# CIawevy/FreeFine

Hardware: AMD Instinct MI355X
Metric: edited images/sec/GPU @512px 50-step DDIM (higher is better)
Workload: dtype bf16x3

## Files before the change

freefine_amd/_lib.py:

```python
import ctypes as C
import os

_HERE = os.path.dirname(os.path.abspath(__file__))
LIB_PATH = os.environ.get("FREEFINE_HIP_LIB") or os.path.join(_HERE, "libfreefine_hip.so")

FFN_F32, FFN_BF16, FFN_BF16X3, FFN_FP8 = 0, 1, 2, 3
IG_OUT_SILU, IG_OUT_F32, IG_GEGLU, IG_OUT_TRANSPOSED, IG_OUT_PAIR, IG_OUT_GELU, IG_OUT_RELU, IG_OUT_KV64 = 1, 2, 4, 8, 16, 32, 64, 128
IG_OUT_QGELU = 256
ELT_RELU, ELT_ADD, ELT_GELU = 0, 1, 2
ATT_MAXP, ATT_MAXB = 4, 16
ATT_HEAD_RULE, ATT_UNIFORM_SEL1, ATT_UNIFORM_SEL0, ATT_CAUSAL = 1, 2, 4, 8
NORM_SILU, NORM_OUT_PAIR = 1, 2
IMGPREP_MAX_SIDE = 4096
IMGPREP_MAX_TAPS = 2 * 3 * IMGPREP_MAX_SIDE + 1
BOX_NMS_MAX = 16384
KEEP_NONE, KEEP_SUM_LT128, KEEP_GT128 = 0, 1, 2


class IgemmDesc(C.Structure):
    _fields_ = [
        ("A", C.c_void_p), ("W", C.c_void_p), ("out", C.c_void_p),
        ("bias", C.c_void_p), ("rowbias", C.c_void_p), ("residual", C.c_void_p),
        ("M", C.c_int), ("N", C.c_int), ("K", C.c_int), ("Kpad", C.c_int),
        ("lda", C.c_int), ("ldo", C.c_int), ("ldr", C.c_int), ("ldrb", C.c_int),
        ("rows_per_batch", C.c_int),
        ("Hin", C.c_int), ("Win", C.c_int), ("Cin", C.c_int), ("Hout", C.c_int), ("Wout", C.c_int),
        ("stride", C.c_int), ("pad", C.c_int), ("upsample", C.c_int),
        ("flags", C.c_int), ("alpha", C.c_float), ("conv", C.c_int),
        ("splitk", C.c_int), ("ws", C.c_void_p), ("ws_bytes", C.c_long),
        ("a_lo", C.c_int), ("x3", C.c_int), ("f8", C.c_int), ("kv64_from", C.c_int),
    ]


class AttnEntry(C.Structure):
    _fields_ = [
        ("q_row", C.c_int), ("kv_row", C.c_int),
        ("w_const", C.c_float), ("w_slope", C.c_float),
        ("wq", C.c_void_p), ("kmask", C.c_void_p), ("qsel", C.c_void_p),
        ("flags", C.c_int), ("hr_row", C.c_int),
    ]


class AttnDesc(C.Structure):
    _fields_ = [
        ("q", C.c_void_p), ("k", C.c_void_p), ("vt", C.c_void_p), ("out", C.c_void_p), ("w_dev", C.c_void_p),
        ("Bo", C.c_int), ("S", C.c_int), ("Sk", C.c_int), ("heads", C.c_int), ("D", C.c_int),
        ("ldq", C.c_int), ("ldk", C.c_int), ("ldvt", C.c_int), ("ldo", C.c_int),
        ("scale", C.c_float), ("npass", C.c_int), ("out_pair", C.c_int), ("kv_pair", C.c_int),
        ("e", AttnEntry * (ATT_MAXP * ATT_MAXB)),
    ]


class CtrlStepDesc(C.Structure):
    _fields_ = [
        ("eps", C.c_void_p), ("x", C.c_void_p), ("noise", C.c_void_p), ("m", C.c_void_p), ("om", C.c_void_p),
        ("x_prev", C.c_void_p), ("pred_x0", C.c_void_p),
        ("c_bt", C.c_float), ("c_at", C.c_float), ("c_ap", C.c_float), ("c_dir", C.c_float),
        ("c_dirm", C.c_float * 8), ("stdv", C.c_float * 8), ("row_masked", C.c_int * 8),
        ("rows", C.c_int), ("CHW", C.c_int), ("HW", C.c_int),
    ]


class SplatXform(C.Structure):
    _fields_ = [("center", C.c_float * 3), ("translate", C.c_float * 3), ("rotate", C.c_float * 9), ("scale", C.c_float * 3),
                ("tan_half_fov", C.c_float)]


class PackDesc(C.Structure):
    _fields_ = [
        ("src", C.c_void_p), ("dst", C.c_void_p), ("src_row", C.c_int * 16),
        ("B", C.c_int), ("Cl", C.c_int), ("CP", C.c_int), ("HW", C.c_int),
    ]


class DiftDesc(C.Structure):
    _fields_ = [
        ("src", C.c_void_p), ("tgt", C.c_void_p), ("kps", C.c_void_p), ("ws", C.c_void_p), ("out_rc", C.c_void_p), ("out_cos", C.c_void_p),
        ("ws_bytes", C.c_long), ("es", C.c_long),
        ("dtype", C.c_int), ("E", C.c_int), ("C", C.c_int), ("ld", C.c_int), ("h", C.c_int), ("w", C.c_int), ("H", C.c_int), ("W", C.c_int), ("K", C.c_int),
    ]


class ResizePilDesc(C.Structure):
    _fields_ = [
        ("src", C.c_void_p), ("dst", C.c_void_p), ("scratch", C.c_void_p), ("m1", C.c_void_p), ("m2", C.c_void_p),
        ("hbounds", C.c_void_p), ("hcoef", C.c_void_p), ("vbounds", C.c_void_p), ("vcoef", C.c_void_p),
        ("B", C.c_int), ("H", C.c_int), ("W", C.c_int), ("C", C.c_int), ("oh", C.c_int), ("ow", C.c_int), ("hksize", C.c_int), ("vksize", C.c_int),
        ("y0", C.c_int), ("x0", C.c_int), ("ch", C.c_int), ("cw", C.c_int), ("rule", C.c_int),
    ]


class CoarseEditDesc(C.Structure):
    _fields_ = [
        ("src_img", C.c_void_p), ("src_mask", C.c_void_p), ("bg", C.c_void_p), ("hole_img", C.c_void_p), ("hole_mask", C.c_void_p), ("inv", C.c_void_p),
        ("final_img", C.c_void_p), ("tmask", C.c_void_p), ("trans_hole", C.c_void_p),
        ("B", C.c_int), ("H", C.c_int), ("W", C.c_int), ("mask_c", C.c_int), ("hole_mask_c", C.c_int),
    ]


_vp, _i, _f, _l = C.c_void_p, C.c_int, C.c_float, C.c_long
SYMBOLS = {
    "ffn_version": (_i, []),
    "ffn_last_error": (C.c_char_p, []),
    "ffn_device_info": (_i, [_i, C.c_char_p, _i]),
    "ffn_graph_launch": (_i, [_vp, _vp]),
    "ffn_igemm": (_i, [_vp, _i, C.POINTER(IgemmDesc)]),
    "ffn_conv3x3_n4": (_i, [_vp, _i, _vp, _vp, _vp, _vp, _i, _i, _i, _i]),
    "ffn_split_pair": (_i, [_vp, _vp, _vp, _l, _i, _i]),
    "ffn_groupnorm_f8": (_i, [_vp, _vp, _vp, _vp, _vp, _i, _i, _i, _i, _i, _f, _i, _f, _vp, _vp, _vp]),
    "ffn_attn": (_i, [_vp, _i, C.POINTER(AttnDesc)]),
    "ffn_attn_kernel_name": (_i, [_i, C.POINTER(AttnDesc), C.c_char_p, _i]),
    "ffn_igemm_tune": (_i, [_vp, _i, C.POINTER(IgemmDesc)]),
    "ffn_igemm_tune_entry_ints": (_i, []),
    "ffn_igemm_tune_export": (_i, [C.POINTER(C.c_int), _i]),
    "ffn_igemm_tune_import": (_i, [C.POINTER(C.c_int), _i]),
    "ffn_igemm_tune_stamp": (_i, []),
    "ffn_igemm_tune_clear": (_i, []),
    "ffn_igemm_tune_enable": (_i, [_i]),
    "ffn_igemm_num_configs": (_i, []),
    "ffn_igemm_force_config": (_i, [_i]),
    "ffn_igemm_kernel_name": (_i, [_i, C.POINTER(IgemmDesc), C.c_char_p, _i]),
    "ffn_attn_presplit": (_i, [_vp, _vp, _vp, _vp, _vp, _i, _i, _i, _i, _i]),
    "ffn_attn_variant": (_i, [_i, _i, C.POINTER(C.c_int), C.POINTER(C.c_int)]),
    "ffn_gn_nchunk": (_i, [_i]),
    "ffn_gn_fused": (_i, [_i, _i, _i, _i]),
    "ffn_gn_stats": (_i, [_vp, _i, _vp, _vp, _vp, _i, _i, _i, _i, _f, _vp, _vp, _vp]),
    "ffn_gn_apply": (_i, [_vp, _i, _vp, _vp, _vp, _vp, _i, _i, _i, _i]),
    "ffn_groupnorm": (_i, [_vp, _i, _vp, _vp, _vp, _vp, _i, _i, _i, _i, _f, _i, _vp, _vp, _vp]),
    "ffn_groupnorm_pair_raw": (_i, [_vp, _vp, _vp, _vp, _vp, _vp, _i, _i, _i, _i, _f, _i, _vp, _vp, _vp]),
    "ffn_layernorm": (_i, [_vp, _i, _vp, _vp, _vp, _vp, _i, _i, _f]),
    "ffn_layernorm_pair": (_i, [_vp, _vp, _vp, _vp, _vp, _i, _i, _f]),
    "ffn_softmax_rows": (_i, [_vp, _i, _vp, _vp, _l, _i, _f]),
    "ffn_pool_layernorm": (_i, [_vp, _i, _vp, _vp, _vp, _vp, _vp, _i, _i, _i, _f, _i]),
    "ffn_cosine_rows": (_i, [_vp, _vp, _vp, _vp, _i, _i, _i]),
    "ffn_cfg_masked": (_i, [_vp, _vp, _vp, _vp, _f, _vp, _l, _i]),
    "ffn_ddim_inv_step": (_i, [_vp, _vp, _vp, _f, _f, _f, _f, _vp, _vp, _l]),
    "ffn_ddim_ctrl_step": (_i, [_vp, C.POINTER(CtrlStepDesc)]),
    "ffn_pack_nchw": (_i, [_vp, _i, C.POINTER(PackDesc)]),
    "ffn_nhwc_to_nchw_f32": (_i, [_vp, _vp, _vp, _i, _i, _i, _i]),
    "ffn_concat": (_i, [_vp, _i, _vp, _vp, _vp, _l, _i, _i]),
    "ffn_timestep_embed": (_i, [_vp, _i, _vp, _vp, _vp, _i, _i, _i]),
    "ffn_transpose": (_i, [_vp, _i, _vp, _vp, _i, _i, _i, _i, _i]),
    "ffn_cast": (_i, [_vp, _i, _i, _vp, _vp, _l]),
    "ffn_eltwise": (_i, [_vp, _i, _i, _vp, _vp, _vp, _l]),
    "ffn_resize_bilinear": (_i, [_vp, _i, _vp, _vp, _i, _i, _i, _i, _i, _i, _i]),
    "ffn_splat_lift": (_i, [_vp, _vp, _vp, _vp, _i, _i, _i, _f, _f]),
    "ffn_splat_project": (_i, [_vp, _vp, _vp, _i, C.POINTER(SplatXform)]),
    "ffn_splat_bin": (_i, [_vp, _i, _vp, _i, _f, _i, _i, _vp, _vp, _vp]),
    "ffn_splat_render": (_i, [_vp, _vp, _vp, _vp, _vp, _f, _i, _i, _i, _vp, _vp, _vp]),
    "ffn_splat_ids": (_i, [_vp, _vp, _vp, _vp, _f, _i, _i, _i, _vp]),
    "ffn_splat_correspond": (_i, [_vp, _vp, _vp, _i, _i, _i, _vp, _i, _vp, _vp]),
    "ffn_geo_project": (_i, [_vp, _vp, C.POINTER(C.c_float), _f, _i, _i, _vp, _vp]),
    "ffn_splat_composite": (_i, [_vp, _vp, _vp, _vp, _vp, _f, _f, _i, _i, _i, _i, _i, _vp]),
    "ffn_mesh_cover": (_i, [_vp, _vp, _vp, _i, _i, _vp]),
    "ffn_embed_tokens": (_i, [_vp, _i, _vp, _vp, _vp, _vp, _l, _i, _i, _i]),
    "ffn_dift_match": (_i, [_vp, C.POINTER(DiftDesc)]),
    "ffn_dift_workspace_bytes": (_l, [_i, _i, _i, _i]),
    "ffn_sift_base": (_i, [_vp, _vp, _vp, _i, _i, _i]),
    "ffn_gauss_blur_f32": (_i, [_vp, _vp, _vp, _vp, _i, _i, _vp, _i]),
    "ffn_decimate2_f32": (_i, [_vp, _vp, _vp, _i, _i]),
    "ffn_sift_extrema": (_i, [_vp, _vp, _vp, _i, _i, _vp, _i, _vp, C.POINTER(C.c_int)]),
    "ffn_sift_refine_orient": (_i, [_vp, _vp, _vp, _i, _i, _i, _vp, _i, _vp]),
    "ffn_sift_describe": (_i, [_vp, _vp, _i, _i, _i, _vp, _i, _vp, _vp]),
    "ffn_knn2_u8": (_i, [_vp, _vp, _i, _vp, _i, _vp, _vp]),
    "ffn_resize_pil_bilinear_u8": (_i, [_vp, _vp, _vp, _vp, _i, _i, _i, _i, _i, _vp, _vp, _i, _vp, _vp, _i]),
    "ffn_resize_pil_u8": (_i, [_vp, C.POINTER(ResizePilDesc)]),
    "ffn_resize_taps8_u8": (_i, [_vp, _vp, _vp, _i, _i, _i, _i, _i, _i, _vp, _vp, _vp, _vp]),
    "ffn_resize_gather_u8": (_i, [_vp, _vp, _vp, _i, _i, _i, _i, _i, _i, _vp, _vp, _i]),
    "ffn_dilate_u8": (_i, [_vp, _vp, _vp, _vp, _i, _i, _i, _i, _i]),
    "ffn_mask_bbox_u8": (_i, [_vp, _vp, _vp, _i, _i, _i, _i]),
    "ffn_coarse_edit_2d": (_i, [_vp, C.POINTER(CoarseEditDesc)]),
    "ffn_vit_patch_rows": (_i, [_vp, _i, _vp, _vp, _vp, _i, _i, _i, _i, _i]),
    "ffn_vit_patch_rows_pair": (_i, [_vp, _vp, _vp, _vp, _i, _i, _i, _i, _i]),
    "ffn_sam_patch_rows": (_i, [_vp, _i, _vp, _vp, _i, _i, _i, _i, _i, _i, C.POINTER(C.c_float), C.POINTER(C.c_float)]),
    "ffn_sam_patch_rows_pair": (_i, [_vp, _vp, _vp, _i, _i, _i, _i, _i, _i, C.POINTER(C.c_float), C.POINTER(C.c_float)]),
    "ffn_hyper_masks": (_i, [_vp, _vp, _vp, _vp, _i, _i, _i, _i]),
    "ffn_upsample_bicubic": (_i, [_vp, _vp, _vp, _vp, _i, _i, _i, _i, _i]),
    "ffn_upsample_bicubic_stats": (_i, [_vp, _vp, _vp, _vp, _i, _i, _i, _i, _i, _f]),
    "ffn_box_nms": (_i, [_vp, _vp, _vp, _i, _f]),
    "ffn_image_to_nhwc": (_i, [_vp, _i, _vp, _vp, _l, _i]),
    "ffn_nhwc_to_image": (_i, [_vp, _i, _vp, _vp, _i, _i, _i]),
}

# ... 29 lines not shown
```

freefine_amd/csrc/capi.hip:

```cpp
#include <stdlib.h>
#include <string.h>

#include "capi_common.h"
#include "conv_small.h"
#include "elementwise.h"
#include "norms.h"

__thread char g_err[512] = "";

extern "C" int ffn_version(void) { return 14; }
extern "C" const char* ffn_last_error(void) { return g_err; }
extern "C" int ffn_device_info(int device, char* name, int name_len) {
    hipDeviceProp_t prop;
    hipError_t e = hipGetDeviceProperties(&prop, device);
    if (e != hipSuccess) return fail(FFN_EHIP, "hipGetDeviceProperties: %s", hipGetErrorString(e));
    if (name && name_len > 0) {
        strncpy(name, prop.gcnArchName, name_len - 1);
        name[name_len - 1] = 0;
    }
    return prop.multiProcessorCount;
}

extern "C" int ffn_graph_launch(void* stream, void* graph_exec) {
    REQUIRE(graph_exec, "graph_launch: null graph");
    hipError_t e = hipGraphLaunch(reinterpret_cast<hipGraphExec_t>(graph_exec), reinterpret_cast<hipStream_t>(stream));
    if (e != hipSuccess) return fail(FFN_EHIP, "hipGraphLaunch: %s", hipGetErrorString(e));
    return FFN_OK;
}

extern "C" int ffn_split_pair(void* stream, const float* src, void* dst, long rows, int C, int ld_src) {
    REQUIRE(src && dst && rows > 0 && C > 0 && C % 4 == 0 && ld_src >= C && ld_src % 4 == 0, "split_pair: bad arguments (C=%d, ld_src=%d)", C, ld_src);
    REQUIRE(aligned16(src) && aligned16(dst), "split_pair: pointers must be 16-byte aligned");
    static const int wide = [] { const char* e = getenv("FFN_PAIR8"); return e ? atoi(e) : 1; }();
    if (wide && C % 8 == 0 && ld_src % 4 == 0) LAUNCH(split_pair8_kernel, dim3(grid_for(rows * (C / 8))), dim3(256), 0, reinterpret_cast<hipStream_t>(stream), src, (bf16*)dst, rows, C, ld_src);
    else LAUNCH(split_pair_kernel, dim3(grid_for(rows * (C / 4))), dim3(256), 0, reinterpret_cast<hipStream_t>(stream), src, (bf16*)dst, rows, C, ld_src);
    return check_launch("split_pair");
}
extern "C" int ffn_conv3x3_n4(void* stream, int dtype, const void* x, const float* w, const float* bias, float* out, int B, int H, int W, int Cin) {
    REQUIRE(dtype == FFN_F32 || dtype == FFN_BF16, "conv3x3_n4: fp32 or bf16 activations");
    REQUIRE(x && w && out && aligned16(x) && aligned16(w) && aligned16(out) && (!bias || aligned16(bias)), "conv3x3_n4: null / unaligned pointer");
    REQUIRE(B > 0 && H > 0 && W > 0 && Cin > 0 && Cin % 16 == 0 && Cin <= 448, "conv3x3_n4: B=%d H=%d W=%d Cin=%d (Cin %% 16 == 0, <= 448)", B, H, W, Cin);
    hipStream_t s = reinterpret_cast<hipStream_t>(stream);
    const long npix = (long)B * H * W;
    const int lds = 36 * Cin * 4;
    dim3 grid((unsigned)((npix + 63) / 64));
    int rc;
    if (dtype == FFN_F32) {
        if ((rc = set_lds(conv3x3_n4_kernel<float>, lds))) return rc;
        LAUNCH(conv3x3_n4_kernel<float>, grid, dim3(256), lds, s, (const float*)x, w, bias, out, B, H, W, Cin);
    } else {
        if ((rc = set_lds(conv3x3_n4_kernel<bf16>, lds))) return rc;
        LAUNCH(conv3x3_n4_kernel<bf16>, grid, dim3(256), lds, s, (const bf16*)x, w, bias, out, B, H, W, Cin);
    }
    return check_launch("conv3x3_n4");
}

extern "C" int ffn_eltwise(void* stream, int dtype, int op, const void* a, const void* b, void* y, long n) {
    REQUIRE(dtype == FFN_F32 || dtype == FFN_BF16, "eltwise: bad dtype %d", dtype);
    REQUIRE(op == FFN_ELT_RELU || op == FFN_ELT_ADD || op == FFN_ELT_GELU, "eltwise: bad op %d", op);
    REQUIRE(a && y && (op != FFN_ELT_ADD || b), "eltwise: null operand");
    REQUIRE(n > 0 && n % 4 == 0, "eltwise: n=%ld must be a positive multiple of 4", n);
    hipStream_t s = reinterpret_cast<hipStream_t>(stream);
    const long n4 = n / 4;
    const int grid = grid_for(n4);
    if (dtype == FFN_F32) {
        if (op == FFN_ELT_RELU) LAUNCH((eltwise_kernel<float, FFN_ELT_RELU>), dim3(grid), dim3(256), 0, s, (const float*)a, (const float*)b, (float*)y, n4);
        else if (op == FFN_ELT_GELU) LAUNCH((eltwise_kernel<float, FFN_ELT_GELU>), dim3(grid), dim3(256), 0, s, (const float*)a, (const float*)b, (float*)y, n4);
        else LAUNCH((eltwise_kernel<float, FFN_ELT_ADD>), dim3(grid), dim3(256), 0, s, (const float*)a, (const float*)b, (float*)y, n4);
    } else {
        if (op == FFN_ELT_RELU) LAUNCH((eltwise_kernel<bf16, FFN_ELT_RELU>), dim3(grid), dim3(256), 0, s, (const bf16*)a, (const bf16*)b, (bf16*)y, n4);
        else if (op == FFN_ELT_GELU) LAUNCH((eltwise_kernel<bf16, FFN_ELT_GELU>), dim3(grid), dim3(256), 0, s, (const bf16*)a, (const bf16*)b, (bf16*)y, n4);
        else LAUNCH((eltwise_kernel<bf16, FFN_ELT_ADD>), dim3(grid), dim3(256), 0, s, (const bf16*)a, (const bf16*)b, (bf16*)y, n4);
    }
    return check_launch("eltwise");
}
extern "C" int ffn_resize_bilinear(void* stream, int dtype, const void* x, void* y, int B, int Hin, int Win, int Hout, int Wout, int C, int relu) {
    REQUIRE(dtype == FFN_F32 || dtype == FFN_BF16, "resize_bilinear: bad dtype %d", dtype);
    REQUIRE(x && y, "resize_bilinear: null operand");
    REQUIRE(B > 0 && Hin > 0 && Win > 0 && Hout > 0 && Wout > 0 && C > 0 && C % 4 == 0, "resize_bilinear: bad shape (C=%d must be a multiple of 4)", C);
    REQUIRE((long)B * Hout * Wout * C < (1l << 40) && (long)Hin * Win < (1l << 31), "resize_bilinear: problem too large");
    hipStream_t s = reinterpret_cast<hipStream_t>(stream);
    const long n4 = (long)B * Hout * Wout * (C / 4);
    const int grid = grid_for(n4);
    if (dtype == FFN_F32) {
        if (relu) LAUNCH((resize_bilinear_kernel<float, true>), dim3(grid), dim3(256), 0, s, (const float*)x, (float*)y, n4, Hin, Win, Hout, Wout, C);
        else LAUNCH((resize_bilinear_kernel<float, false>), dim3(grid), dim3(256), 0, s, (const float*)x, (float*)y, n4, Hin, Win, Hout, Wout, C);
    } else {
        if (relu) LAUNCH((resize_bilinear_kernel<bf16, true>), dim3(grid), dim3(256), 0, s, (const bf16*)x, (bf16*)y, n4, Hin, Win, Hout, Wout, C);
        else LAUNCH((resize_bilinear_kernel<bf16, false>), dim3(grid), dim3(256), 0, s, (const bf16*)x, (bf16*)y, n4, Hin, Win, Hout, Wout, C);
    }
    return check_launch("resize_bilinear");
}

extern "C" int ffn_gn_nchunk(int HW) {
    int n = HW / 128;
    if (n < 1) n = 1;
    if (n > 256) n = 256;
    return n;
}
extern "C" int ffn_gn_fused(int B, int HW, int C, int G) {
    const long slice = (long)HW * (C / (G > 0 ? G : 1));
    if (slice > 131072) return 0;
    if (HW <= 64) return 1;
    if (HW <= 256) return B <= 32 ? 1 : 0;
    return (HW <= 1024 && (long)B * HW * C <= 3000000l) ? 1 : 0;
}
extern "C" int ffn_groupnorm(void* stream, int dtype, const void* x, void* y, const float* gamma, const float* beta, int B, int HW, int C,
                             int G, float eps, int silu, float* partial_ws, float* scale, float* shift) {
    REQUIRE(dtype == FFN_F32 || dtype == FFN_BF16, "groupnorm: bad dtype");
    REQUIRE(x && y && gamma && beta && C % G == 0 && (C / G) % 2 == 0, "groupnorm: bad arguments (C=%d, G=%d)", C, G);
    hipStream_t s = reinterpret_cast<hipStream_t>(stream);
    const long slice = (long)HW * (C / G);
    (void)slice;
    const bool fused = ffn_gn_fused(B, HW, C, G) != 0;
    const bool pair = silu & FFN_NORM_OUT_PAIR;
    REQUIRE(!pair || (dtype == FFN_F32 && C % 4 == 0), "groupnorm: pair output needs fp32 input and C %% 4 == 0");
    silu &= FFN_NORM_SILU;
    if (fused && pair) {
        dim3 grid(G, B);
        if (silu) LAUNCH((gn_fused_kernel<float, true, true>), grid, dim3(1024), 0, s, (const float*)x, (float*)y, gamma, beta, HW, C, G, eps);
        else LAUNCH((gn_fused_kernel<float, false, true>), grid, dim3(1024), 0, s, (const float*)x, (float*)y, gamma, beta, HW, C, G, eps);
        return check_launch("gn_fused(pair)");
    }
    if (fused) {
        dim3 grid(G, B);
        if (dtype == FFN_F32) {
            if (silu) LAUNCH((gn_fused_kernel<float, true>), grid, dim3(1024), 0, s, (const float*)x, (float*)y, gamma, beta, HW, C, G, eps);
            else LAUNCH((gn_fused_kernel<float, false>), grid, dim3(1024), 0, s, (const float*)x, (float*)y, gamma, beta, HW, C, G, eps);
        } else {
            if (silu) LAUNCH((gn_fused_kernel<bf16, true>), grid, dim3(1024), 0, s, (const bf16*)x, (bf16*)y, gamma, beta, HW, C, G, eps);
            else LAUNCH((gn_fused_kernel<bf16, false>), grid, dim3(1024), 0, s, (const bf16*)x, (bf16*)y, gamma, beta, HW, C, G, eps);
        }
        return check_launch("gn_fused");
    }
    REQUIRE(partial_ws && scale && shift, "groupnorm: workspace required beyond 32x32 positions");
    int rc = ffn_gn_stats(stream, dtype, x, gamma, beta, B, HW, C, G, eps, partial_ws, scale, shift);
    if (rc) return rc;
    return ffn_gn_apply(stream, dtype, x, y, scale, shift, B, HW, C, silu | (pair ? FFN_NORM_OUT_PAIR : 0));
}
extern "C" int ffn_groupnorm_pair_raw(void* stream, const void* x, void* y, void* yraw, const float* gamma, const float* beta, int B, int HW, int C, int G,
                                      float eps, int silu, float* partial_ws, float* scale, float* shift) {
    REQUIRE(x && y && yraw && gamma && beta && partial_ws && scale && shift, "groupnorm_pair_raw: null pointer (the workspace is always needed)");
    REQUIRE(C % 8 == 0 && C % G == 0 && (C / G) % 2 == 0 && aligned16(x) && aligned16(y) && aligned16(yraw), "groupnorm_pair_raw: bad arguments (C=%d, G=%d)", C, G);
    REQUIRE(y != yraw && yraw != x && y != x, "groupnorm_pair_raw: x, y and yraw must be distinct buffers");
    int rc = ffn_gn_stats(stream, FFN_F32, x, gamma, beta, B, HW, C, G, eps, partial_ws, scale, shift);
    if (rc) return rc;
    hipStream_t s = reinterpret_cast<hipStream_t>(stream);
    const long n8 = (long)B * HW * (C / 8);
    if (silu & FFN_NORM_SILU) LAUNCH((gn_apply_pair8_kernel<true, true>), dim3(grid_for(n8)), dim3(256), 0, s, (const float*)x, (bf16*)y, scale, shift, n8, HW, C, (bf16*)yraw);
    else LAUNCH((gn_apply_pair8_kernel<false, true>), dim3(grid_for(n8)), dim3(256), 0, s, (const float*)x, (bf16*)y, scale, shift, n8, HW, C, (bf16*)yraw);
    return check_launch("gn_apply(pair + raw pair)");
}
extern "C" int ffn_groupnorm_f8(void* stream, const void* x, void* y, const float* gamma, const float* beta, int B, int HW, int C, int Cp, int G,
                                float eps, int silu, float qscale, float* partial_ws, float* scale, float* shift) {
    REQUIRE(x && y && gamma && beta && partial_ws && scale && shift, "groupnorm_f8: null pointer (the workspace is always needed)");
    REQUIRE(C % 16 == 0 && C % G == 0 && Cp >= C && Cp % 16 == 0 && aligned16(x) && aligned16(y) && qscale > 0.f, "groupnorm_f8: bad arguments (C=%d, Cp=%d)", C, Cp);
    int rc = ffn_gn_stats(stream, FFN_BF16, x, gamma, beta, B, HW, C, G, eps, partial_ws, scale, shift);
    if (rc) return rc;
    hipStream_t s = reinterpret_cast<hipStream_t>(stream);
    const long nch = (long)B * HW * (Cp / 16);
    if (silu & FFN_NORM_SILU) LAUNCH(gn_apply_f8_kernel<true>, dim3(grid_for(nch)), dim3(256), 0, s, (const bf16*)x, (uint8_t*)y, scale, shift, nch, HW, C, Cp, qscale);
    else LAUNCH(gn_apply_f8_kernel<false>, dim3(grid_for(nch)), dim3(256), 0, s, (const bf16*)x, (uint8_t*)y, scale, shift, nch, HW, C, Cp, qscale);
    return check_launch("gn_apply_f8");
// ... 179 lines not shown
```

freefine_amd/csrc/capi_igemm.hip:

```cpp
#include <math.h>
#include <stdlib.h>
#include <string.h>
#include <initializer_list>

#include "capi_common.h"
#include "igemm.h"
#include "igemm_p8.h"

static bool can_split(const ffn_igemm_desc& d) {
    return d.ws && d.splitk != 1 && !(d.flags & (FFN_IG_GEGLU | FFN_IG_OUT_TRANSPOSED | FFN_IG_OUT_KV64));
}
static void igemm_rule_for(int dtype, const ffn_igemm_desc& d, int* bm, int* bn, int* splitk) {
    const long t128 = (long)((d.M + 127) / 128) * ((d.N + 127) / 128);
    const long t12864 = (long)((d.M + 127) / 128) * ((d.N + 63) / 64);
    *splitk = 1;
    if (!d.conv && !(d.flags & FFN_IG_GEGLU) && d.M >= 128 && (!can_split(d) || t12864 >= 128)) {
        *bm = 128; *bn = 64;
    } else if (d.N > 64 && (t128 >= 256 || (can_split(d) && d.M > 512 && d.N >= 128))) {
        *bm = 128; *bn = 128;
    } else if (t12864 >= 256 || d.M >= 4096 || (can_split(d) && d.M >= 96 && d.N >= 64)) {
        *bm = 128; *bn = 64;
    } else { *bm = 64; *bn = 64; }
    if (can_split(d)) {
        const int kstage = dtype == FFN_F32 ? 32 : 64;
        const int nk = (d.K + kstage - 1) / kstage;
        const long tiles = (long)((d.M + *bm - 1) / *bm) * ((d.N + *bn - 1) / *bn);
        int s = d.splitk > 1 ? d.splitk : (tiles >= 224 ? 1 : (int)((448 + tiles - 1) / tiles));
        if (d.splitk <= 1 && s > nk / 6) s = nk / 6;
        const long per = (long)d.M * d.N * 4;
        if ((long)s * per > d.ws_bytes) s = (int)(d.ws_bytes / per);
        if (s > nk) s = nk;
        if (s < 1) s = 1;
        *splitk = s;
    }
}

enum { CFG_64x64, CFG_128x64, CFG_128x128_8, CFG_128x128_16, CFG_256x128, CFG_256x256, CFG_128x320, CFG_128x160, CFG_192x320, CFG_H_128x320, CFG_H_256x128, CFG_H_256x256, CFG_H_128x128, CFG_PP_256x320, CFG_PP_256x256, CFG_PP_192x320, CFG_PP_192x256, CFG_PP_256x128, CFG_COUNT };
struct IgCfgInfo { int bm, bn, nwm, nwn; };
static const IgCfgInfo kCfg[CFG_COUNT] = {{64, 64, 2, 2}, {128, 64, 4, 2}, {128, 128, 2, 4}, {128, 128, 4, 4},
                                          {256, 128, 4, 4}, {256, 256, 4, 4}, {128, 320, 4, 4}, {128, 160, 4, 2}, {192, 320, 3, 4},
                                          {128, 320, 4, 4}, {256, 128, 4, 4}, {256, 256, 4, 4}, {128, 128, 4, 4},
                                          {256, 320, 2, 4}, {256, 256, 2, 4}, {192, 320, 2, 4}, {192, 256, 2, 4},
                                          {256, 128, 2, 4}};
struct IgChoice { int cfg, splitk; };
struct TunedEntry { IgChoice ch; bool validated; };

static bool is_halo_cfg(int cfg) { return cfg == CFG_H_128x320 || cfg == CFG_H_256x128 || cfg == CFG_H_256x256 || cfg == CFG_H_128x128; }
static bool is_pp_cfg(int cfg) { return cfg >= CFG_PP_256x320 && cfg <= CFG_PP_256x128; }
static bool pp_ok(const ffn_igemm_desc& d, int bm, int bn, int splitk = 1) {
    const long lim = (1l << 31) - 4096;
    const int nkt = d.x3 ? d.K / 96 : d.K / 64;
    if (bn == 128 && (bm != 256 || !d.x3 || d.conv != 1 || splitk > 1 || d.N % 256 == 0 || d.N % 320 == 0 || (d.flags & (FFN_IG_GEGLU | FFN_IG_OUT_PAIR | FFN_IG_OUT_KV64 | FFN_IG_OUT_TRANSPOSED)))) return false;
    if (d.x3) {
        if (d.x3 != 2 || d.K % 96 != 0 || d.a_lo != 32) return false;
    } else if (d.K % 64 != 0) return false;
    if (nkt < 2 || d.N % bn != 0 || d.M < bm) return false;
    const int osz = d.x3 ? 4 : 2;
    if (splitk > 1) {
        if (!can_split(d) || nkt % splitk != 0 || nkt / splitk < 2 || (long)splitk * d.M * d.N * 4 > d.ws_bytes || (long)splitk * d.M * d.N * 4 >= lim) return false;
    } else {
        const int act_ok = (!d.residual && !d.x3 && !d.f8 && !(d.flags & FFN_IG_GEGLU)) ? (FFN_IG_OUT_GELU | FFN_IG_OUT_RELU) : 0;
        if ((d.alpha != 1.0f && !d.f8) || (d.flags & ~(FFN_IG_GEGLU | act_ok | (d.x3 ? (FFN_IG_OUT_F32 | FFN_IG_OUT_PAIR | FFN_IG_OUT_KV64) : 0)))) return false;
        if (d.f8 && (!d.conv || (d.flags & FFN_IG_GEGLU))) return false;
        if (d.x3 && (d.flags & FFN_IG_GEGLU) && !(d.flags & FFN_IG_OUT_PAIR)) return false;
        if ((d.flags & FFN_IG_OUT_PAIR) && !(d.flags & FFN_IG_GEGLU) && (d.N % 32 != 0 || (d.ldo / 2) % 32 != 0 || (d.flags & FFN_IG_OUT_TRANSPOSED))) return false;
        if ((d.flags & FFN_IG_GEGLU) && bn != 256) return false;
        if (d.rowbias && d.rows_per_batch < 128) return false;
    }
    long a_bytes;
    if (d.conv) {
        const int pix = d.x3 ? d.lda : d.Cin;
        const int cpt = d.x3 ? d.Cin / 32 : d.Cin / 64;
        if (d.Cin % (d.x3 ? 32 : 64) != 0 || d.K != (d.conv == 2 ? 4 : 9) * (d.x3 ? 3 : 1) * d.Cin) return false;
        if (d.x3 && d.lda != 2 * d.Cin) return false;
        if (d.conv == 2 && (d.f8 || d.stride != 1 || d.upsample)) return false;
        if ((long)cpt * 9 * cpt >= 65536) return false;
        a_bytes = (long)(d.M / (d.Hout * d.Wout)) * d.Hin * d.Win * pix * 2;
        if (2 * d.Hin + 2 >= 32768 || 2 * d.Win + 2 >= 32768) return false;
        if (a_bytes + 256l * pix * 2 >= lim) return false;
    } else {
        a_bytes = (long)d.M * d.lda * 2;
        if (a_bytes + 256l * d.lda * 2 >= lim) return false;
    }
    if ((long)d.N * d.Kpad * 2 >= lim || (long)(d.M + 256) * d.ldo * ((d.flags & FFN_IG_OUT_PAIR) ? 2 : osz) >= lim) return false;
    if (d.residual && (long)(d.M + 256) * d.ldr * osz >= lim) return false;
    return true;
}
static int halo_bytes_for(const ffn_igemm_desc& d, int bm) {
    if (!d.conv || d.stride != 1 || d.upsample || d.pad != 1 || d.Hin != d.Hout || d.Win != d.Wout) return 0;
    if (d.Cin % 64 != 0 || d.Cin > 30000 || d.K != 9 * d.Cin || d.M % bm != 0) return 0;
    const int H = d.Hin, W = d.Win;
    int tw, tr;
    if (W <= bm) {
        if (bm % W != 0 || (H * W) % bm != 0) return 0;
        tw = W; tr = bm / W;
    } else {
        if (W % bm != 0) return 0;
        tw = bm; tr = 1;
    }
    const int nq = ((tr + 2) * (tw + 2) + 7) / 8;
    if (nq > 4 * 16) return 0;
    return nq * 8 * 128;
}
static bool x3_cfg(int cfg) { return cfg == CFG_64x64 || cfg == CFG_128x64 || cfg == CFG_128x128_8 || is_pp_cfg(cfg); }
static ffn_igemm_desc x3_view(const ffn_igemm_desc& d) {
    ffn_igemm_desc v = d;
    v.x3 = d.x3 == 2 ? 2 : 1;
    v.f8 = 0;
    v.K = 3 * d.K;
    v.flags |= FFN_IG_OUT_F32;
    return v;
}
static ffn_igemm_desc f8_view(const ffn_igemm_desc& d) {
    ffn_igemm_desc v = d;
    v.f8 = 1;
    v.x3 = 0;
    v.K = d.K / 2;
    v.Cin = d.Cin / 2;
    v.Kpad = d.Kpad / 2;
    v.lda = d.lda / 2;
    return v;
}
static ffn_igemm_desc igemm_view(int dtype, const ffn_igemm_desc& d) {
    if (dtype == FFN_BF16X3) return x3_view(d);
    if (dtype == FFN_FP8) return f8_view(d);
    ffn_igemm_desc v = d;
    v.x3 = v.f8 = 0;
    return v;
}
static int pp_tile_height(const ffn_igemm_desc& d, int bn, std::initializer_list<int> heights, int min_fill4, bool trans = false) {
    long best = -1;
    int bh = 0;
    for (int h : heights) {
        if (trans ? d.M < h : !pp_ok(d, h, bn)) continue;
        const long tiles = (long)((d.M + h - 1) / h) * (d.N / bn);
        if (tiles * 4 < (long)device_cus() * min_fill4) continue;
        const long cost = ((tiles + device_cus() - 1) / device_cus()) * h;
        if (best < 0 || cost < best) { best = cost; bh = h; }
    }
    return bh;
}
static int pp_cfg(int bm, int bn) {
    for (int cfg = CFG_PP_256x320; cfg <= CFG_PP_256x128; ++cfg)
        if (kCfg[cfg].bm == bm && kCfg[cfg].bn == bn) return cfg;
    return -1;
}
static bool conv2_tile(const ffn_igemm_desc& d, int* bm, int* bn) {
    for (int n : {320, 256})
        for (int h : {256, 192})
            if (pp_tile_height(d, n, {h}, 0)) { *bm = h; *bn = n; return true; }
    return false;
}
static bool pp_trans_tile(const ffn_igemm_desc& d, int* bm, int* bn) {
    const long lim = (1l << 31) - 4096;
    *bn = d.N % 320 == 0 ? 320 : (d.N % 256 == 0 ? 256 : 0);
    if (!*bn || d.alpha != 1.0f || d.rows_per_batch % 16 != 0 || d.M % 4 != 0) return false;
    if (d.x3) {
        if (d.x3 != 2 || d.K % 96 != 0 || d.K < 192 || d.a_lo != 32) return false;
    } else if (d.K % 64 != 0 || d.K < 128) return false;
    if ((long)(d.M + 256) * d.lda * 2 >= lim || (long)d.N * d.Kpad * 2 >= lim) return false;
    if ((long)((d.M + d.rows_per_batch - 1) / d.rows_per_batch) * d.N * d.ldo * (d.x3 ? 4 : 2) >= lim) return false;
    return (*bm = pp_tile_height(d, *bn, {256, 192}, 0, true)) != 0;
}
static IgChoice rule_choice(int dtype, const ffn_igemm_desc& d) {
    int bm, bn, sk;
    igemm_rule_for(dtype, d, &bm, &bn, &sk);
    const int kstage = dtype == FFN_F32 ? 32 : 64;
    const int nk = ((d.K + kstage - 1) / kstage + sk - 1) / sk;
    int cfg = CFG_64x64;
    if (bm == 128 && bn == 64) cfg = CFG_128x64;
    if (bm == 128 && bn == 128) cfg = (!d.conv && nk <= 24 && !d.x3 && !d.f8) ? CFG_128x128_16 : CFG_128x128_8;
    return IgChoice{cfg, sk};
}
static IgChoice heuristic_choice(const ffn_igemm_desc& d) {
    int bm, bn;
    if (d.conv == 2 && conv2_tile(d, &bm, &bn)) return IgChoice{pp_cfg(bm, bn), 1};
    if (d.splitk <= 1) {
        for (int n : {320, 256})
            if ((bm = pp_tile_height(d, n, {256, 192}, 3))) return IgChoice{pp_cfg(bm, n), 1};
        if (pp_tile_height(d, 128, {256}, 3)) return IgChoice{CFG_PP_256x128, 1};
    }
    return rule_choice(FFN_BF16, d);
}

struct TuneKey {
    int M, N, K, conv, Cin, Hin, Win, stride, upsample, flags, lda, splitk, ptrs, wslabs, rpb, alpha1, ldo, pad, Hout, Wout, Kpad, ldr, dtype;
    bool operator==(const TuneKey& o) const { return memcmp(this, &o, sizeof(TuneKey)) == 0; }
};
struct TuneKeyHash {
    size_t operator()(const TuneKey& k) const {
        const int* p = reinterpret_cast<const int*>(&k);
        size_t h = 1469598103934665603ull;
        for (size_t i = 0; i < sizeof(TuneKey) / sizeof(int); ++i) h = (h ^ (size_t)(unsigned)p[i]) * 1099511628211ull;
        return h;
    }
};
static TuneKey tune_key(const ffn_igemm_desc& d) {
    TuneKey k;
    memset(&k, 0, sizeof(k));
    k.M = d.M; k.N = d.N; k.K = d.K; k.conv = d.conv; k.flags = d.flags; k.lda = d.lda; k.splitk = d.splitk;
    if (d.conv) { k.Cin = d.Cin; k.Hin = d.Hin; k.Win = d.Win; k.stride = d.stride; k.upsample = d.upsample; k.pad = d.pad; k.Hout = d.Hout; k.Wout = d.Wout; }
    k.Kpad = d.Kpad;
    k.ldr = d.residual ? d.ldr : 0;
    k.dtype = d.x3 ? (FFN_BF16X3 | (d.x3 << 8)) : (d.f8 ? FFN_FP8 : FFN_BF16);
    k.ptrs = (d.bias ? 1 : 0) | (d.rowbias ? 2 : 0) | (d.residual ? 4 : 0) | (d.ws && d.ws_bytes > 0 ? 8 : 0);
    const long per = (long)d.M * d.N * 4;
    k.wslabs = d.ws ? (int)(d.ws_bytes / per > 1024 ? 1024 : d.ws_bytes / per) : 0;
    k.rpb = d.rows_per_batch;
    k.alpha1 = d.alpha == 1.0f;
    k.ldo = d.ldo;
    return k;
}
static std::mutex g_tune_mu;
static std::unordered_map<TuneKey, TunedEntry, TuneKeyHash> g_tuned;
static int g_tune_runtime = 1;
static bool tune_enabled() {
    static const bool on = [] { const char* e = getenv("FFN_IGEMM_TUNE"); return !(e && atoi(e) == 0); }();
    return on && g_tune_runtime;
}
static constexpr int kPpSplitBelow = 160;
static int candidates_for(const ffn_igemm_desc& d, IgChoice* out, int cap) {
    int n = 0;
    const IgChoice h = heuristic_choice(d);
    out[n++] = h;
    const int nk = (d.K + 63) / 64;
    const long per = (long)d.M * d.N * 4;
    for (int cfg = 0; cfg < CFG_COUNT; ++cfg) {
        const IgCfgInfo& c = kCfg[cfg];
        if ((d.x3 || d.f8) && !x3_cfg(cfg)) continue;
        if (d.conv == 2 && !is_pp_cfg(cfg)) continue;
        if ((cfg == CFG_128x320 || cfg == CFG_128x160 || cfg == CFG_192x320) && (d.flags & FFN_IG_GEGLU)) continue;
        if (is_halo_cfg(cfg)) {
            const int hb = halo_bytes_for(d, c.bm);
            if (hb <= 0 || d.splitk > 1 || 2 * hb + 2 * c.bn * 128 > 160 * 1024) continue;
            if ((cfg == CFG_H_128x320) && (d.flags & FFN_IG_GEGLU)) continue;
        }
        const bool halo = is_halo_cfg(cfg) || is_pp_cfg(cfg);
        if (is_pp_cfg(cfg)) {
            const long pt = (long)((d.M + c.bm - 1) / c.bm) * (d.N / (c.bn > 0 ? c.bn : 1));
            if (d.splitk <= 1 && pp_ok(d, c.bm, c.bn) && n < cap) out[n++] = IgChoice{cfg, 1};
            if (cfg != CFG_PP_256x128 && d.splitk != 1 && pt > 0 && pt < kPpSplitBelow && d.N % c.bn == 0) {
                const int nkt = d.x3 ? d.K / 96 : d.K / 64;
                int added = 0;
                for (int sgo = (int)((384 + pt - 1) / pt); sgo >= 2 && added < 2; --sgo) {
                    if (d.splitk > 1 && sgo != d.splitk) continue;
                    if (nkt % sgo != 0 || nkt / sgo < 2 || !pp_ok(d, c.bm, c.bn, sgo)) continue;
                    if (n < cap) out[n++] = IgChoice{cfg, sgo};
                    ++added;
                }
            }
            continue;
        }
        if (c.bm > 64 && c.bm >= 2 * d.M) continue;
        if (c.bn > 64 && c.bn >= 2 * d.N) continue;
        if (cfg == CFG_64x64 && (long)d.M * d.N > (1l << 22)) continue;
        const long tiles = (long)((d.M + c.bm - 1) / c.bm) * ((d.N + c.bn - 1) / c.bn);
        int splits[3] = {1, 0, 0};
        if (d.splitk > 1) {
            int sf = (can_split(d) && !halo) ? d.splitk : 1;
            if ((long)sf * per > d.ws_bytes) sf = (int)(d.ws_bytes / per);
            if (sf > nk) sf = nk;
            splits[0] = sf >= 2 ? sf : 1;
        } else if (can_split(d) && !halo) {
            for (int t = 0; t < 2; ++t) {
                int sgo = (int)(((t ? 512 : 256) + tiles / 2) / tiles);
                if (sgo > nk / 4) sgo = nk / 4;
                if ((long)sgo * per > d.ws_bytes) sgo = (int)(d.ws_bytes / per);
                if (sgo >= 2) splits[1 + t] = sgo;
            }
            if (splits[2] == splits[1]) splits[2] = 0;
        }
        for (int t = 0; t < 3 && n < cap; ++t) {
            if (!splits[t]) continue;
            bool dup = false;
            for (int j = 0; j < n; ++j) dup |= out[j].cfg == cfg && out[j].splitk == splits[t];
            if (!dup) out[n++] = IgChoice{cfg, splits[t]};
        }
    }
    return n;
}
static int g_force_cfg = -1;
extern "C" int ffn_igemm_num_configs(void) { return CFG_COUNT; }
extern "C" int ffn_igemm_force_config(int cfg) {
    const int prev = g_force_cfg;
    g_force_cfg = (cfg >= 0 && cfg < CFG_COUNT) ? cfg : -1;
    return prev;
}
static bool known_choice(const ffn_igemm_desc& d, IgChoice* ch) {
    IgChoice cand[40];
    if (g_force_cfg >= 0) {
        *ch = heuristic_choice(d);
        for (int i = candidates_for(d, cand, 40) - 1; i >= 0; --i)
            if (cand[i].cfg == g_force_cfg) *ch = cand[i];
        return true;
    }
    std::lock_guard<std::mutex> lk(g_tune_mu);
    auto it = g_tuned.find(tune_key(d));
    if (it == g_tuned.end()) return false;
    if (!it->second.validated) {
        const int nc = candidates_for(d, cand, 40);
        bool ok = false;
        for (int i = 0; i < nc; ++i) ok |= cand[i].cfg == it->second.ch.cfg && cand[i].splitk == it->second.ch.splitk;
        if (!ok) return g_tuned.erase(it), false;
        it->second.validated = true;
    }
    *ch = it->second.ch;
    return true;
}

enum IgKind { IG_RING, IG_HALO, IG_PP, IG_PP_TRANS };
struct IgemmPlan {
    IgKind kind;
    bool f32;
    int bm, bn, amode, nwm, nwn;
    bool swap, fastk, x3, f8;
    bool res, geglu, split;
    int splitk, halo_bytes, lds;
    bool reduce_f32;
    dim3 grid, block;
};
static int igemm_plan(int dtype, const ffn_igemm_desc& d, const IgChoice* ch, IgemmPlan* p) {
    *p = IgemmPlan{};
    p->f32 = dtype == FFN_F32;
    p->x3 = d.x3 != 0;
    p->f8 = d.f8 != 0;
    p->amode = d.conv ? AMODE_CONV3 : AMODE_DENSE;
    p->swap = !(d.flags & FFN_IG_OUT_TRANSPOSED);
    p->reduce_f32 = p->f32 || p->x3;
    p->splitk = 1;
    p->block = dim3(512);
    const bool tuned = ch != nullptr;
    IgChoice rule;
    if (!tuned && !p->f32 && pp_trans_tile(d, &p->bm, &p->bn)) {
        p->kind = IG_PP_TRANS;
    } else {
        if (!tuned) ch = &(rule = rule_choice(p->f32 ? FFN_F32 : FFN_BF16, d));
        REQUIRE(ch->cfg >= 0 && ch->cfg < CFG_COUNT, "igemm: bad configuration %d", ch->cfg);
        REQUIRE(!(p->x3 || p->f8) || x3_cfg(ch->cfg), "igemm: configuration %d is not built for split-bf16 / fp8 problems", ch->cfg);
        const IgCfgInfo& c = kCfg[ch->cfg];
        p->kind = is_halo_cfg(ch->cfg) ? IG_HALO : (is_pp_cfg(ch->cfg) ? IG_PP : IG_RING);
        p->bm = c.bm; p->bn = c.bn; p->nwm = c.nwm; p->nwn = c.nwn;
        p->splitk = ch->splitk;
        p->block = dim3(64 * c.nwm * c.nwn);
        if (!tuned && p->x3) p->nwm = p->nwn = 2, p->block = dim3(256);
    }
    const int ntm = (d.M + p->bm - 1) / p->bm, ntn = (d.N + p->bn - 1) / p->bn;
    switch (p->kind) {
    case IG_RING: {
        p->fastk = tuned && !p->x3 && !p->f8 && (d.conv ? d.Cin % 64 == 0 : d.K % 64 == 0) && (long)d.K * 2 + 256 <= (long)sizeof(g_zero_page);
        p->lds = 2 * (p->bm + p->bn) * 128;
        int gx = ntm * ntn;
        if (tuned || p->x3) {
            int per_cu = (160 * 1024) / p->lds;
            if (per_cu > 2048 / (int)p->block.x) per_cu = 2048 / (int)p->block.x;
            const int cap = (device_cus() * per_cu) / p->splitk;
            if (gx > cap && cap >= 8) gx = cap;
        }
        p->grid = dim3(gx, p->splitk);
        break;
    }
    case IG_HALO:
        p->halo_bytes = halo_bytes_for(d, p->bm);
        REQUIRE(p->halo_bytes > 0 && p->splitk == 1 && !p->x3 && !p->f8, "igemm: halo kernel not applicable");
        p->lds = 2 * p->halo_bytes + 2 * p->bn * 128;
        p->grid = dim3((d.M / p->bm) * ntn);
        break;
    case IG_PP:
        REQUIRE(pp_ok(d, p->bm, p->bn, p->splitk), "igemm: ping-pong kernel not applicable");
        p->split = p->splitk > 1;
        p->res = !p->split && d.residual;
        p->geglu = !p->split && !d.conv && (d.flags & FFN_IG_GEGLU);
        [[fallthrough]];
    case IG_PP_TRANS: {
        p->lds = 2 * (p->bm + p->bn) * 128 + 12288;
        const int nt = ntm * (d.N / p->bn) * p->splitk;
        p->grid = dim3(nt < device_cus() ? nt : device_cus());
        break;
    }
    }
    return FFN_OK;
}
template <typename K, typename... A>
static int igemm_launch(const IgemmPlan& p, K kern, hipStream_t s, A... args) {
    static const char* const what[] = {"igemm", "igemm(halo)", "igemm(ping-pong)", "igemm(ping-pong, transposed)"};
    if (int rc = set_lds(kern, p.lds)) return rc;
    LAUNCH(kern, p.grid, p.block, p.lds, s, args...);
    return check_launch(what[p.kind]);
}
template <typename T, int AMODE, bool SWAP, bool FASTK = false, bool X3 = false, bool F8 = false>
static int launch_ring(const IgemmPlan& p, hipStream_t s, const ffn_igemm_desc& d) {
#define FFN_RING(BM_, BN_, WM_, WN_) \
    if (p.bm == BM_ && p.bn == BN_ && p.nwm == WM_ && p.nwn == WN_) return igemm_launch(p, igemm_glds_kernel<T, BM_, BN_, AMODE, SWAP, 2, WM_, WN_, FASTK, X3, F8>, s, d)
    if constexpr (X3 && !SWAP) {
        FFN_RING(64, 64, 2, 2);
        FFN_RING(128, 64, 2, 2);
        FFN_RING(128, 128, 2, 2);
    } else {
        FFN_RING(64, 64, 2, 2);
        FFN_RING(128, 64, 4, 2);
        FFN_RING(128, 128, 2, 4);
        if constexpr (!X3 && !F8) FFN_RING(128, 128, 4, 4);
        if constexpr (sizeof(T) == 2 && SWAP && !X3 && !F8) {
            FFN_RING(256, 128, 4, 4);
            FFN_RING(256, 256, 4, 4);
            FFN_RING(128, 320, 4, 4);
            FFN_RING(128, 160, 4, 2);
            FFN_RING(192, 320, 3, 4);
        }
    }
#undef FFN_RING
    return fail(FFN_EINVAL, "igemm: no %d x %d tile on %d x %d waves for this problem", p.bm, p.bn, p.nwm, p.nwn);
}
template <int AMODE, bool X3 = false, bool F8 = false>
static int launch_pp(const IgemmPlan& p, hipStream_t s, const ffn_igemm_desc& d) {
    const bool trans = p.kind == IG_PP_TRANS;
#define FFN_PP(BM_, BN_, RES_, GEGLU_, SPLIT_, TRANS_)                                                                       \
    if (p.bm == BM_ && p.bn == BN_ && p.res == RES_ && p.geglu == GEGLU_ && p.split == SPLIT_ && trans == TRANS_) \
        return igemm_launch(p, igemm_pp_kernel<BM_, BN_, AMODE, RES_, GEGLU_, SPLIT_, TRANS_, X3, F8>, s, d, p.splitk)
#define FFN_PP_TILE(BM_, BN_)                                                                   \
    FFN_PP(BM_, BN_, false, false, false, false);                                               \
    FFN_PP(BM_, BN_, true, false, false, false);                                                \
    FFN_PP(BM_, BN_, false, false, true, false);                                                \
    if constexpr (AMODE == AMODE_DENSE && !F8) {                                                \
        FFN_PP(BM_, BN_, false, false, false, true);                                            \
        if constexpr (BN_ == 256) FFN_PP(BM_, BN_, false, true, false, false);                  \
    }
    FFN_PP_TILE(256, 320)
    FFN_PP_TILE(256, 256)
    FFN_PP_TILE(192, 320)
    FFN_PP_TILE(192, 256)
    if constexpr (X3 && AMODE == AMODE_CONV3) {
        FFN_PP(256, 128, false, false, false, false);
        FFN_PP(256, 128, true, false, false, false);
    }
#undef FFN_PP_TILE
#undef FFN_PP
    return fail(FFN_EINVAL, "igemm: no %d x %d ping-pong tile of this form", p.bm, p.bn);
}
static int igemm_run(hipStream_t s, int dtype, const ffn_igemm_desc& d, const IgChoice* ch) {
    IgemmPlan p;
    int rc = igemm_plan(dtype, d, ch, &p);
    if (rc) return rc;
    const bool conv = p.amode == AMODE_CONV3;
    switch (p.kind) {
    case IG_RING:
        if (p.f32) rc = conv ? launch_ring<float, AMODE_CONV3, true>(p, s, d) : (p.swap ? launch_ring<float, AMODE_DENSE, true>(p, s, d) : launch_ring<float, AMODE_DENSE, false>(p, s, d));
        else if (!p.swap) rc = p.x3 ? launch_ring<bf16, AMODE_DENSE, false, false, true>(p, s, d) : launch_ring<bf16, AMODE_DENSE, false>(p, s, d);
        else if (p.x3) rc = conv ? launch_ring<bf16, AMODE_CONV3, true, false, true>(p, s, d) : launch_ring<bf16, AMODE_DENSE, true, false, true>(p, s, d);
        else if (p.f8) rc = launch_ring<bf16, AMODE_CONV3, true, false, false, true>(p, s, d);
        else if (p.fastk) rc = conv ? launch_ring<bf16, AMODE_CONV3, true, true>(p, s, d) : launch_ring<bf16, AMODE_DENSE, true, true>(p, s, d);
        else rc = conv ? launch_ring<bf16, AMODE_CONV3, true>(p, s, d) : launch_ring<bf16, AMODE_DENSE, true>(p, s, d);
        break;
    case IG_HALO:
#define FFN_HALO(BM_, BN_) \
    if (p.bm == BM_ && p.bn == BN_) rc = igemm_launch(p, igemm_halo_kernel<bf16, BM_, BN_, 4, 4>, s, d, p.halo_bytes)
        FFN_HALO(128, 320);
        FFN_HALO(256, 128);
        FFN_HALO(256, 256);
        FFN_HALO(128, 128);
#undef FFN_HALO
        break;
    case IG_PP:
    case IG_PP_TRANS:
        if (p.x3) rc = conv ? launch_pp<AMODE_CONV3, true>(p, s, d) : launch_pp<AMODE_DENSE, true>(p, s, d);
        else if (p.f8) rc = launch_pp<AMODE_CONV3, false, true>(p, s, d);
        else rc = conv ? launch_pp<AMODE_CONV3>(p, s, d) : launch_pp<AMODE_DENSE>(p, s, d);
        break;
    }
    if (rc || p.splitk == 1) return rc;
    const dim3 grid(grid_for((long)d.M * (d.N / 4)));
    if (p.reduce_f32) LAUNCH(igemm_splitk_reduce_kernel<float>, grid, dim3(256), 0, s, d, p.splitk);
    else LAUNCH(igemm_splitk_reduce_kernel<bf16>, grid, dim3(256), 0, s, d, p.splitk);
    return check_launch("igemm_splitk_reduce");
}
static int igemm_tune_now(hipStream_t s, int dtype, const ffn_igemm_desc& d) {
    std::lock_guard<std::mutex> lk(g_tune_mu);
    IgChoice cand[40];
    const int nc = candidates_for(d, cand, 40);
    hipEvent_t e0, e1;
    if (hipEventCreate(&e0) != hipSuccess || hipEventCreate(&e1) != hipSuccess) return igemm_run(s, dtype, d, &cand[0]);
    IgChoice best = cand[0];
    float best_ms = 1e30f;
    const int reps = 3;
    for (int i = 0; i < nc; ++i) {
        int rc = igemm_run(s, dtype, d, &cand[i]);
        if (rc) continue;
        float ms = 1e30f;
        for (int round = 0; round < 2 && !rc; ++round) {
            (void)hipEventRecord(e0, s);
            for (int r = 0; r < reps && !rc; ++r) rc = igemm_run(s, dtype, d, &cand[i]);
            (void)hipEventRecord(e1, s);
            if (rc || hipEventSynchronize(e1) != hipSuccess) { rc = rc ? rc : FFN_EHIP; break; }
            float t = 0.f;
            (void)hipEventElapsedTime(&t, e0, e1);
            if (t < ms) ms = t;
        }
        if (rc) continue;
        if (ms < best_ms) { best_ms = ms; best = cand[i]; }
    }
    (void)hipEventDestroy(e0);
    (void)hipEventDestroy(e1);
    g_tuned[tune_key(d)] = TunedEntry{best, true};
    static const bool verbose = getenv("FFN_IGEMM_TUNE_VERBOSE") != nullptr;
    if (verbose)
        fprintf(stderr, "[ffn tune] %s M=%d N=%d K=%d flags=%d -> %dx%d split %d (%.1f us, %d candidates)\n", d.conv ? "conv" : "dense", d.M, d.N,
                d.K, d.flags, kCfg[best.cfg].bm, kCfg[best.cfg].bn, best.splitk, best_ms * 1e3f / reps, nc);
    return igemm_run(s, dtype, d, &best);
}
static constexpr int kTuneEntryInts = (int)(sizeof(TuneKey) / sizeof(int)) + 3;
static constexpr int kTuneStamp = 0x67780000 ^ (950 << 4) ^ ((int)sizeof(TuneKey) << 8) ^ CFG_COUNT ^ (4 << 24);
extern "C" int ffn_igemm_tune_entry_ints(void) { return kTuneEntryInts; }
extern "C" int ffn_igemm_tune_stamp(void) { return kTuneStamp; }
extern "C" int ffn_igemm_tune_clear(void) {
    std::lock_guard<std::mutex> lk(g_tune_mu);
    const int n = (int)g_tuned.size();
    g_tuned.clear();
    return n;
}
extern "C" int ffn_igemm_tune_enable(int on) {
    std::lock_guard<std::mutex> lk(g_tune_mu);
    const int prev = g_tune_runtime;
    g_tune_runtime = on ? 1 : 0;
    return prev;
}
extern "C" int ffn_igemm_tune_export(int* buf, int max_entries) {
    std::lock_guard<std::mutex> lk(g_tune_mu);
    int n = 0;
    for (const auto& kv : g_tuned) {
        if (buf && n < max_entries) {
            int* e = buf + (long)n * kTuneEntryInts;
            e[0] = kTuneStamp;
            memcpy(e + 1, &kv.first, sizeof(TuneKey));
            e[kTuneEntryInts - 2] = kv.second.ch.cfg;
            e[kTuneEntryInts - 1] = kv.second.ch.splitk;
        }
        ++n;
    }
    return n;
}
extern "C" int ffn_igemm_tune_import(const int* buf, int n_entries) {
    REQUIRE(buf || n_entries == 0, "igemm_tune_import: null buffer");
    std::lock_guard<std::mutex> lk(g_tune_mu);
    int n = 0;
    for (int i = 0; i < n_entries; ++i) {
        const int* e = buf + (long)i * kTuneEntryInts;
        if (e[0] != kTuneStamp) continue;
        TuneKey k;
        memcpy(&k, e + 1, sizeof(TuneKey));
        const IgChoice ch{e[kTuneEntryInts - 2], e[kTuneEntryInts - 1]};
        if (ch.cfg < 0 || ch.cfg >= CFG_COUNT || ch.splitk < 1) continue;
        g_tuned[k] = TunedEntry{ch, false};
        ++n;
    }
    return n;
}
static int igemm_validate(int dtype, const ffn_igemm_desc& d) {
    REQUIRE(dtype == FFN_F32 || dtype == FFN_BF16 || dtype == FFN_BF16X3 || dtype == FFN_FP8, "igemm: bad dtype %d", dtype);
    if (dtype == FFN_FP8) {
        REQUIRE(d.conv && d.Cin > 0 && d.Cin % 16 == 0 && d.K == 9 * d.Cin && d.Kpad >= d.K && d.Kpad % 16 == 0 && d.lda == d.Cin,
                "igemm(fp8): 3x3 convolutions with Cin %% 16 == 0 only (Cin=%d, K=%d, Kpad=%d, lda=%d)", d.Cin, d.K, d.Kpad, d.lda);
        REQUIRE(d.M > 0 && d.N > 0 && d.N % 4 == 0 && d.ldo % 4 == 0 && d.rows_per_batch > 0 && d.M % (d.Hout * d.Wout) == 0, "igemm(fp8): bad shape");
        REQUIRE(!(d.flags & (FFN_IG_GEGLU | FFN_IG_OUT_TRANSPOSED | FFN_IG_OUT_PAIR | FFN_IG_OUT_F32)), "igemm(fp8): plain / SiLU / residual epilogues only");
        REQUIRE(d.stride == 1 || d.stride == 2, "igemm(fp8): stride %d", d.stride);
        int ex = 0;
        REQUIRE(d.alpha > 0.f && frexpf(d.alpha, &ex) == 0.5f, "igemm(fp8): alpha must be a power of two (the un-scaling of two power-of-two operand scales)");
        if (d.residual) REQUIRE(d.ldr % 4 == 0 && d.ldr >= d.N, "igemm(fp8): ldr=%d must be a multiple of 4 and >= N=%d", d.ldr, d.N);
        REQUIRE(d.ldo >= d.N, "igemm(fp8): ldo=%d must be >= N=%d", d.ldo, d.N);
        return FFN_OK;
    }
    const int epc = dtype == FFN_F32 ? 4 : 8;
    const int kmul = dtype == FFN_BF16X3 ? (d.x3 == 2 ? 2 : 3) : 1;
    REQUIRE(d.M > 0 && d.N > 0 && d.K > 0, "igemm: empty problem M=%d N=%d K=%d", d.M, d.N, d.K);
    REQUIRE(d.Kpad >= kmul * d.K && d.Kpad % epc == 0, "igemm: Kpad=%d (row stride of W) must be >= %d x K=%d and a multiple of %d", d.Kpad, kmul, d.K, epc);
    if (dtype == FFN_BF16X3) {
        const int plane = d.conv ? d.Cin : d.K;
        if (d.x3 == 2) {
            REQUIRE(plane % 32 == 0 && d.a_lo == 32 && d.lda >= 2 * plane, "igemm: blocked split-bf16 operands need K (conv: Cin) %% 32 == 0, a_lo = 32, lda >= 2 x that (%d, a_lo=%d, lda=%d)", plane, d.a_lo, d.lda);
        } else {
            REQUIRE(d.a_lo % 8 == 0 && d.a_lo >= plane && d.a_lo + plane <= d.lda, "igemm: split-bf16 A needs planes of %d elements: a_lo=%d, lda=%d", plane, d.a_lo, d.lda);
        }
        REQUIRE(d.lda % 8 == 0, "igemm: lda=%d must be a multiple of 8", d.lda);
        REQUIRE(d.alpha == 1.0f, "igemm: split-bf16 problems take alpha = 1");
    }
    REQUIRE(d.K % epc == 0, "igemm: K=%d must be a multiple of %d", d.K, epc);
    REQUIRE(d.rows_per_batch > 0, "igemm: rows_per_batch must be > 0");
    if (d.conv) {
        REQUIRE(d.Cin % epc == 0, "igemm: Cin=%d must be a multiple of %d", d.Cin, epc);
        if (d.conv == 2) {
            REQUIRE((dtype == FFN_BF16 || dtype == FFN_BF16X3) && d.K == 4 * d.Cin && d.stride == 1 && d.upsample == 0 && d.pad >= 0 && d.pad <= 3 && d.splitk <= 1,
                    "igemm: 2x2 convolution needs FFN_BF16 / FFN_BF16X3, K = 4*Cin, stride 1, no upsample, pad in 0..3, no forced split");
            int bm, bn;
            REQUIRE(conv2_tile(igemm_view(dtype, d), &bm, &bn), "igemm: 2x2 convolution M=%d N=%d Cin=%d fits no ping-pong tile (Cin %% 64 (split-bf16: 32), N %% 256 / 320, M >= 192)", d.M, d.N, d.Cin);
        } else {
            REQUIRE(d.conv == 1, "igemm: conv=%d", d.conv);
            REQUIRE(d.K == 9 * d.Cin, "igemm: conv K=%d != 9*Cin=%d", d.K, 9 * d.Cin);
        }
        REQUIRE(d.stride == 1 || d.stride == 2, "igemm: stride %d", d.stride);
        REQUIRE(d.upsample == 0 || d.upsample == 1, "igemm: upsample %d", d.upsample);
        REQUIRE(d.M % (d.Hout * d.Wout) == 0, "igemm: M=%d not a multiple of Hout*Wout", d.M);
    } else {
        REQUIRE(d.lda % epc == 0, "igemm: lda=%d must be a multiple of %d", d.lda, epc);
    }
    if (d.flags & FFN_IG_OUT_KV64) {
        REQUIRE(dtype == FFN_BF16X3 && !d.conv && !d.residual && !d.rowbias && d.splitk <= 1 &&
                    !(d.flags & (FFN_IG_GEGLU | FFN_IG_OUT_PAIR | FFN_IG_OUT_SILU | FFN_IG_OUT_GELU | FFN_IG_OUT_RELU | FFN_IG_OUT_QGELU)),
                "igemm: FFN_IG_OUT_KV64 needs FFN_BF16X3, dense A, the plain epilogue and no forced split-K");
        if (d.flags & FFN_IG_OUT_TRANSPOSED) REQUIRE(d.rows_per_batch % 64 == 0 && d.M % d.rows_per_batch == 0 && d.ldo >= d.rows_per_batch && d.ldo % 64 == 0,
                                                     "igemm: KV64 transposed output needs rows_per_batch %% 64 == 0, whole batches, ldo %% 64 == 0 (rows_per_batch=%d, ldo=%d)", d.rows_per_batch, d.ldo);
        else REQUIRE(d.kv64_from >= 0 && d.kv64_from < d.N && d.kv64_from % 64 == 0 && d.N % 64 == 0 && d.ldo % 4 == 0,
                     "igemm: KV64 output needs kv64_from and N %% 64 == 0 (kv64_from=%d, N=%d)", d.kv64_from, d.N);
    }
    if (d.flags & FFN_IG_OUT_TRANSPOSED) {
        REQUIRE(!d.conv, "igemm: transposed output is only supported for dense A");
        REQUIRE(d.ldo % 4 == 0, "igemm: transposed ldo=%d must be a multiple of 4", d.ldo);
        REQUIRE(!(d.flags & (FFN_IG_GEGLU | FFN_IG_OUT_F32 | FFN_IG_OUT_SILU | FFN_IG_OUT_GELU | FFN_IG_OUT_RELU | FFN_IG_OUT_QGELU)) && !d.residual && !d.rowbias,
                "igemm: transposed output supports bias only");
    } else {
        REQUIRE(d.N % 4 == 0 && d.ldo % 4 == 0, "igemm: N=%d and ldo=%d must be multiples of 4", d.N, d.ldo);
        if (d.residual) REQUIRE(d.ldr % 4 == 0, "igemm: ldr=%d must be a multiple of 4", d.ldr);
        if (d.flags & FFN_IG_OUT_PAIR) {
            const int nout = (d.flags & FFN_IG_GEGLU) ? d.N / 2 : d.N;
            REQUIRE(dtype == FFN_BF16X3 && d.ldo % 16 == 0 && d.ldo / 2 >= nout, "igemm: pair output needs FFN_BF16X3, ldo %% 16 == 0, ldo/2 >= columns");
            REQUIRE(d.residual != d.out, "igemm: pair output cannot overwrite its fp32 residual");
            REQUIRE((d.ldo / 2) % 32 != 0 || nout % 32 == 0 || nout == d.ldo / 2, "igemm: blocked pair output (ldo/2 %% 32 == 0) needs whole 32-column blocks");
            REQUIRE(nout == d.ldo / 2 || (d.ldo / 2) % 32 == 0, "igemm: pair output into a wider row needs ldo/2 %% 32 == 0 (ldo=%d, columns=%d)", d.ldo, nout);
        }
        if (d.flags & FFN_IG_GEGLU) {
            REQUIRE(d.N % 64 == 0, "igemm: GEGLU needs N %% 64 == 0 (N=%d)", d.N);
            REQUIRE(!d.residual && !d.rowbias && !(d.flags & (FFN_IG_OUT_F32 | FFN_IG_OUT_SILU | FFN_IG_OUT_GELU | FFN_IG_OUT_RELU | FFN_IG_OUT_QGELU)), "igemm: GEGLU epilogue is exclusive");
        }
    }
    const int act = d.flags & (FFN_IG_OUT_SILU | FFN_IG_OUT_GELU | FFN_IG_OUT_RELU | FFN_IG_OUT_QGELU);
    REQUIRE((act & (act - 1)) == 0, "igemm: SILU / GELU / QGELU / RELU are mutually exclusive");
    REQUIRE(d.splitk >= 0, "igemm: splitk must be >= 0");
    if (!d.conv && dtype != FFN_BF16X3) REQUIRE(d.lda >= d.K, "igemm: lda=%d must be >= K=%d", d.lda, d.K);
    if (d.flags & FFN_IG_OUT_TRANSPOSED) {
        const int cols = d.rows_per_batch < d.M ? d.rows_per_batch : d.M;
        REQUIRE(d.ldo >= cols, "igemm: transposed ldo=%d must be >= the %d rows of a batch", d.ldo, cols);
    } else if (!(d.flags & FFN_IG_OUT_PAIR)) {
        const int nout = (d.flags & FFN_IG_GEGLU) ? d.N / 2 : d.N;
        REQUIRE(d.ldo >= nout, "igemm: ldo=%d must be >= the %d output columns", d.ldo, nout);
    }
    if (d.residual) REQUIRE(d.ldr >= d.N, "igemm: ldr=%d must be >= N=%d", d.ldr, d.N);
    return FFN_OK;
}
static bool tuned_family(int dtype, const ffn_igemm_desc& d) { return dtype != FFN_F32 && !(d.flags & FFN_IG_OUT_TRANSPOSED); }
extern "C" int ffn_igemm_kernel_name(int dtype, const ffn_igemm_desc* d0, char* buf, int len) {
    REQUIRE(d0 && buf && len > 0, "igemm_kernel_name: null argument");
    if (int rc = igemm_validate(dtype, *d0)) return rc;
    const ffn_igemm_desc d = igemm_view(dtype, *d0);
    const bool tuned = tuned_family(dtype, d);
    IgChoice ch;
    if (tuned && !known_choice(d, &ch)) ch = heuristic_choice(d);
    IgemmPlan p;
    if (int rc = igemm_plan(dtype, d, tuned ? &ch : nullptr, &p)) return rc;
    auto b = [](bool v) { return v ? "true" : "false"; };
    switch (p.kind) {
    case IG_RING:
        snprintf(buf, len, "void igemm_glds_kernel<%s, %d, %d, %d, %s, 2, %d, %d, %s, %s, %s>(ffn_igemm_desc)", p.f32 ? "float" : "bf16", p.bm, p.bn, p.amode,
                 b(p.swap), p.nwm, p.nwn, b(p.fastk), b(p.x3), b(p.f8));
        break;
    case IG_HALO: snprintf(buf, len, "void igemm_halo_kernel<bf16, %d, %d, %d, %d>(ffn_igemm_desc, int)", p.bm, p.bn, p.nwm, p.nwn); break;
    case IG_PP:
    case IG_PP_TRANS:
        snprintf(buf, len, "void igemm_pp_kernel<%d, %d, %d, %s, %s, %s, %s, %s, %s>(ffn_igemm_desc, int)", p.bm, p.bn, p.amode, b(p.res), b(p.geglu), b(p.split),
                 b(p.kind == IG_PP_TRANS), b(p.x3), b(p.f8));
        break;
    }
    return FFN_OK;
}
extern "C" int ffn_igemm(void* stream, int dtype, const ffn_igemm_desc* d0) {
    REQUIRE(d0, "igemm: null descriptor");
    if (int rc = igemm_validate(dtype, *d0)) return rc;
    if (dtype == FFN_FP8) {
        REQUIRE(d0->A && d0->W && d0->out && aligned16(d0->A) && aligned16(d0->W) && aligned16(d0->out), "igemm(fp8): A/W/out must be non-null and 16-byte aligned");
    } else {
        REQUIRE(d0->A && d0->W && d0->out, "igemm: null A/W/out");
        REQUIRE(aligned16(d0->A) && aligned16(d0->W) && aligned16(d0->out), "igemm: A/W/out must be 16-byte aligned");
    }
    if ((dtype == FFN_BF16X3 || dtype == FFN_F32) && d0->residual) REQUIRE(aligned16(d0->residual), "igemm: fp32 residual must be 16-byte aligned");
    if ((dtype == FFN_BF16 || dtype == FFN_FP8) && d0->residual)
        REQUIRE((reinterpret_cast<uintptr_t>(d0->residual) & 7) == 0, "igemm%s: bf16 residual must be 8-byte aligned", dtype == FFN_FP8 ? "(fp8)" : "");
    if (d0->ws) REQUIRE(aligned16(d0->ws) && d0->ws_bytes >= 0, "igemm%s: workspace must be 16-byte aligned", dtype == FFN_FP8 ? "(fp8)" : "");
    hipStream_t s = reinterpret_cast<hipStream_t>(stream);
    const ffn_igemm_desc d = igemm_view(dtype, *d0);
    if (!tuned_family(dtype, d)) return igemm_run(s, dtype, d, nullptr);
    IgChoice ch;
    if (!known_choice(d, &ch)) {
        hipStreamCaptureStatus cap = hipStreamCaptureStatusNone;
        (void)hipStreamIsCapturing(s, &cap);
        if (tune_enabled() && cap == hipStreamCaptureStatusNone && d.residual != d.out) return igemm_tune_now(s, dtype, d);
        ch = heuristic_choice(d);
    }
    return igemm_run(s, dtype, d, &ch);
}

extern "C" int ffn_igemm_tune(void* stream, int dtype, const ffn_igemm_desc* d) { return ffn_igemm(stream, dtype, d); }
```

freefine_amd/csrc/igemm.h:

```cpp
#pragma once
#include <type_traits>
#include "common.h"
#include "../../include/freefine_hip.h"

enum { AMODE_DENSE = 0, AMODE_CONV3 = 1 };
enum { IG_OUT_SILU = FFN_IG_OUT_SILU, IG_OUT_F32 = FFN_IG_OUT_F32, IG_GEGLU = FFN_IG_GEGLU, IG_OUT_TRANSPOSED = FFN_IG_OUT_TRANSPOSED, IG_OUT_PAIR = FFN_IG_OUT_PAIR,
       IG_OUT_GELU = FFN_IG_OUT_GELU, IG_OUT_RELU = FFN_IG_OUT_RELU, IG_OUT_KV64 = FFN_IG_OUT_KV64, IG_OUT_QGELU = FFN_IG_OUT_QGELU };
__device__ __forceinline__ float ig_activation(float x, int flags) {
    if (flags & IG_OUT_SILU) return silu_exact(x);
    if (flags & IG_OUT_GELU) return gelu_erf(x);
    if (flags & IG_OUT_RELU) return fmaxf(x, 0.f);
    if (flags & IG_OUT_QGELU) return x / (1.0f + expf(-1.702f * x));
    return x;
}
__device__ __forceinline__ void store_pair_row4(bf16* row, int c, int C, const float* v) {
    bf16* p = row + pair_pos(c, C);
    const int lo_off = pair_lo(C);
    u32x2 hi, lo;
    hi[0] = pack_bf16x2(v[0], v[1]);
    hi[1] = pack_bf16x2(v[2], v[3]);
    lo[0] = pack_bf16x2(v[0] - __uint_as_float(hi[0] << 16), v[1] - __uint_as_float(hi[0] & 0xffff0000u));
    lo[1] = pack_bf16x2(v[2] - __uint_as_float(hi[1] << 16), v[3] - __uint_as_float(hi[1] & 0xffff0000u));
    *reinterpret_cast<u32x2*>(p) = hi;
    *reinterpret_cast<u32x2*>(p + lo_off) = lo;
}
__device__ __forceinline__ void store_kv64_4(float* blk, int d, const float* v) {
    bf16* p = reinterpret_cast<bf16*>(blk) + d;
    u32x2 hi, lo;
    hi[0] = pack_bf16x2(v[0], v[1]);
    hi[1] = pack_bf16x2(v[2], v[3]);
    lo[0] = pack_bf16x2(v[0] - __uint_as_float(hi[0] << 16), v[1] - __uint_as_float(hi[0] & 0xffff0000u));
    lo[1] = pack_bf16x2(v[2] - __uint_as_float(hi[1] << 16), v[3] - __uint_as_float(hi[1] & 0xffff0000u));
    *reinterpret_cast<u32x2*>(p) = hi;
    *reinterpret_cast<u32x2*>(p + 64) = lo;
}
typedef ffn_igemm_desc IgemmParams;

template <typename T, int FM, int FN, bool SWAP>
__device__ __forceinline__ void igemm_epilogue(const IgemmParams& p, f32x4 (&acc)[FM][FN], int mbase, int nbase, int l15, int g) {
    T* __restrict__ outT = reinterpret_cast<T*>(p.out);
    float* __restrict__ outF = reinterpret_cast<float*>(p.out);
    const T* __restrict__ res = reinterpret_cast<const T*>(p.residual);
    const bool out_f32 = p.flags & IG_OUT_F32;
    const bool out_act = p.flags & (IG_OUT_SILU | IG_OUT_GELU | IG_OUT_RELU | IG_OUT_QGELU);

    if (SWAP && gridDim.y > 1) {
        float* __restrict__ slab = reinterpret_cast<float*>(p.ws) + (long)blockIdx.y * p.M * p.N;
#pragma unroll
        for (int i = 0; i < FM; ++i) {
            const int m = mbase + i * 16 + l15;
#pragma unroll
            for (int j = 0; j < FN; ++j) {
                const int n = nbase + j * 16 + 4 * g;
                if (m < p.M && n < p.N) {
                    float v[4] = {acc[i][j][0], acc[i][j][1], acc[i][j][2], acc[i][j][3]};
                    store4(slab + (long)m * p.N + n, v);
                }
            }
        }
        return;
    }
    if (SWAP) {
        if ((FN % 2 == 0) && (p.flags & IG_GEGLU)) {
#pragma unroll
            for (int i = 0; i < FM; ++i) {
                const int m = mbase + i * 16 + l15;
#pragma unroll
                for (int j = 0; j + 1 < FN; j += 2) {
                    const int nh = nbase + j * 16 + 4 * g;
                    if (m < p.M && nh < p.N) {
                        float v[4];
#pragma unroll
                        for (int r = 0; r < 4; ++r) {
                            float h = acc[i][j][r] * p.alpha, gt = acc[i][j + 1][r] * p.alpha;
                            if (p.bias) {
                                h += p.bias[nh + r];
                                gt += p.bias[nh + 16 + r];
                            }
                            v[r] = h * gelu_for<T>(gt);
                        }
                        const int no = (nbase) / 2 + (j / 2) * 16 + 4 * g;
                        if (p.flags & IG_OUT_PAIR) store_pair_row4(reinterpret_cast<bf16*>(p.out) + (long)m * p.ldo, no, p.ldo / 2, v);
                        else store4(outT + (long)m * p.ldo + no, v);
                    }
                }
            }
        } else {
#pragma unroll
            for (int i = 0; i < FM; ++i) {
                const int m = mbase + i * 16 + l15;
                const int bb = m / p.rows_per_batch;
#pragma unroll
                for (int j = 0; j < FN; ++j) {
                    const int n = nbase + j * 16 + 4 * g;
                    if (m < p.M && n < p.N) {
                        float v[4];
#pragma unroll
                        for (int r = 0; r < 4; ++r) {
                            float x = acc[i][j][r] * p.alpha;
                            if (p.bias) x += p.bias[n + r];
                            if (p.rowbias) x += p.rowbias[(long)bb * p.ldrb + n + r];
                            if (out_act) x = ig_activation(x, p.flags);
                            v[r] = x;
                        }
                        if (res) {
                            float rr[4];
                            load4(res + (long)m * p.ldr + n, rr);
#pragma unroll
                            for (int r = 0; r < 4; ++r) v[r] += rr[r];
                        }
                        if (p.flags & IG_OUT_PAIR)
                            store_pair_row4(reinterpret_cast<bf16*>(p.out) + (long)m * p.ldo, n, p.ldo / 2, v);
                        else if ((p.flags & IG_OUT_KV64) && n >= p.kv64_from)
                            store_kv64_4(outF + (long)m * p.ldo + p.kv64_from + ((n - p.kv64_from) & ~63), (n - p.kv64_from) & 63, v);
                        else if (out_f32)
                            store4(outF + (long)m * p.ldo + n, v);
                        else
                            store4(outT + (long)m * p.ldo + n, v);
                    }
                }
            }
        }
    } else {
#pragma unroll
        for (int i = 0; i < FM; ++i) {
            const int mb = mbase + i * 16 + 4 * g;
#pragma unroll
            for (int j = 0; j < FN; ++j) {
                const int n = nbase + j * 16 + l15;
                if (n >= p.N) continue;
                float v[4];
#pragma unroll
                for (int r = 0; r < 4; ++r) {
                    float x = acc[i][j][r] * p.alpha;
                    if (p.bias) x += p.bias[n];
                    v[r] = x;
                }
                if (p.flags & IG_OUT_TRANSPOSED) {
                    const int bb = mb / p.rows_per_batch, s = mb - bb * p.rows_per_batch;
                    if ((p.flags & IG_OUT_KV64) && mb < p.M) {
                        store_kv64_4(outF + ((long)bb * p.N + n) * p.ldo + (s & ~63), s & 63, v);
                    } else if ((p.rows_per_batch & 3) == 0 && mb + 3 < p.M) {
                        store4(outT + ((long)bb * p.N + n) * p.ldo + s, v);
                    } else {
#pragma unroll
                        for (int r = 0; r < 4; ++r) {
                            const int m = mb + r;
                            if (m < p.M) {
                                const int b2 = m / p.rows_per_batch, s2 = m - b2 * p.rows_per_batch;
                                DT<T>::st(outT + ((long)b2 * p.N + n) * p.ldo + s2, v[r]);
                            }
                        }
                    }
                } else {
#pragma unroll
                    for (int r = 0; r < 4; ++r) {
                        const int m = mb + r;
                        if (m < p.M) DT<T>::st(outT + (long)m * p.ldo + n, v[r]);
// ... 462 lines not shown
```

freefine_amd/csrc/igemm_p8.h:

```cpp
#pragma once
#include <type_traits>
#include "igemm.h"

#ifndef PP_PRIO
#define PP_PRIO 1
#endif
#ifndef PP_ABL
#define PP_ABL 0
#endif
#ifndef PP_TAPINNER
#define PP_TAPINNER 1
#endif
#ifdef PP_STAMP
__device__ unsigned long long pp_stamp_out[8 * 64];
#define PP_STAMP_AT(k_) do { if (blockIdx.x == 7 && s >= 24 && s < 28) { const unsigned long long t_ = __builtin_amdgcn_s_memtime(); \
    if (lane == 0) *reinterpret_cast<unsigned long long*>(smem + CV + 12288 + (wave * 64 + (s - 24) * 16 + (k_)) * 8) = t_; } } while (0)
#else
#define PP_STAMP_AT(k_) do {} while (0)
#endif
#ifdef PP_NBE
#define X3_NBE(FN_, NA_) (PP_NBE)
#else
#define X3_NBE(FN_, NA_) ((FN_) + 2 - ((FN_) + (NA_) + 1) / 2)
#endif
template <int N>
__device__ __forceinline__ void pp_wait_vmcnt() {
    if (PP_ABL != 2) asm volatile("s_waitcnt vmcnt(%0)" ::"n"(N) : "memory");
}
__device__ __forceinline__ void pp_barrier() {
    asm volatile("" ::: "memory");
    __builtin_amdgcn_s_barrier();
    asm volatile("" ::: "memory");
}

#ifdef PP_TRACE
__device__ unsigned long long pp_trace[256 * 64];
#endif
template <int BM, int BN, int AMODE, bool RES, bool GEGLU, bool SPLIT = false, bool TRANS = false, bool X3 = false, bool F8 = false>
__global__ __launch_bounds__(512) void igemm_pp_kernel(const IgemmParams p, int splitk = 1) {
    typedef bf16 T;
    constexpr int HM = BM / 2;
    constexpr int FM = HM / 16;
    constexpr int FH = FM / 2;
    constexpr int NA = BM / 64;
    constexpr int FN = BN / 64;
    constexpr int WN = BN / 4;
    constexpr int ABYTES = BM * 128, BBYTES = BN * 128, BUF = ABYTES + BBYTES;
    constexpr int CV = 2 * BUF;
    constexpr int NB1 = (FN + 1) / 2;
    constexpr int NST = (SPLIT || TRANS || X3) ? FH * FN : (GEGLU ? FH * FN / 2 : FH * ((FN + 1) / 2));
    constexpr int OSZ = (X3 && !GEGLU) ? 4 : 2;
    constexpr int OOB = (int)0x80000000;
    static_assert((BM == 256 || BM == 192) && (BN == 256 || BN == 320 || (BN == 128 && BM == 256 && X3 && AMODE == AMODE_CONV3 && !GEGLU && !SPLIT && !TRANS)), "tiles built for this kernel");
    static_assert(!GEGLU || FN % 2 == 0, "GEGLU pairs hidden / gate column blocks inside a wave");

    extern __shared__ __attribute__((aligned(16))) char smem[];

    const int tid = threadIdx.x;
    const int lane = tid & 63, wave = __builtin_amdgcn_readfirstlane(tid >> 6);
    const int wr = wave >> 2, wc = wave & 3;
    const int l15 = lane & 15, g = lane >> 4;
    const int lrow = lane >> 3, csrc = (lane & 7) ^ lrow;

    static_assert(!SPLIT || (!RES && !GEGLU), "split-K slabs carry raw accumulators: the epilogue runs in the reduce kernel");
    static_assert(!TRANS || (!RES && !GEGLU && !SPLIT && AMODE == AMODE_DENSE), "transposed output: dense A, bias only");
    static_assert(!F8 || (!X3 && !TRANS && !GEGLU), "fp8 operands: plain / residual / split-K epilogues");
    const int ntn = p.N / BN;
    const int ntm = (p.M + BM - 1) / BM;
    const int nsl = SPLIT ? splitk : 1;
    const int ntiles = ntm * ntn * nsl;
    const int G = gridDim.x;
    const int nk = (X3 ? p.K / 96 : p.K / 64) / nsl;
    const int first = __builtin_amdgcn_readfirstlane(xcd_remap(blockIdx.x, G));
    const int my_tiles = (ntiles - first + G - 1) / G;
    const int S = my_tiles * nk;

    const int PIX = X3 ? p.lda * 2 : p.Cin * 2;
    const long a_bytes = AMODE == AMODE_DENSE ? (long)p.M * p.lda * 2 : (long)(p.M / (p.Hout * p.Wout)) * p.Hin * p.Win * PIX;
    const __amdgpu_buffer_rsrc_t rsrcA = __builtin_amdgcn_make_buffer_rsrc(const_cast<void*>(p.A), 0, (int)a_bytes, 0x00020000);
    const __amdgpu_buffer_rsrc_t rsrcB = __builtin_amdgcn_make_buffer_rsrc(const_cast<void*>(p.W), 0, (int)((long)p.N * p.Kpad * 2), 0x00020000);
    const __amdgpu_buffer_rsrc_t rsrcBias = __builtin_amdgcn_make_buffer_rsrc(const_cast<float*>(p.bias), 0, p.bias ? p.N * 4 : 0, 0x00020000);
    const int nbatch = (p.M + p.rows_per_batch - 1) / p.rows_per_batch;
    const __amdgpu_buffer_rsrc_t rsrcRb =
        __builtin_amdgcn_make_buffer_rsrc(const_cast<float*>(p.rowbias), 0, p.rowbias ? ((nbatch - 1) * p.ldrb + p.N) * 4 : 0, 0x00020000);
    const long o_bytes = TRANS ? (long)((p.M + p.rows_per_batch - 1) / p.rows_per_batch) * p.N * p.ldo * OSZ : (long)p.M * p.ldo * OSZ;
    const __amdgpu_buffer_rsrc_t rsrcO = __builtin_amdgcn_make_buffer_rsrc(p.out, 0, (int)o_bytes, 0x00020000);
    const __amdgpu_buffer_rsrc_t rsrcR = __builtin_amdgcn_make_buffer_rsrc(const_cast<void*>(p.residual), 0, RES ? (int)((long)p.M * p.ldr * OSZ) : 0, 0x00020000);

    int l_tile = first, l_kt = 0;
    int l_k0 = 0;
    int a_off[NA];
    int a_yx[NA];
    int b_voff;
    const int b_step = 64 * p.Kpad * 2;
    int apiece[NA];
    if constexpr (BM == 256) {
        apiece[0] = wave; apiece[1] = 16 + wave; apiece[2] = 8 + wave; apiece[3] = 24 + wave;
    } else {
        apiece[0] = wave < 6 ? wave : wave + 6;
        apiece[1] = wave < 4 ? 14 + wave : 2 + wave;
        apiece[2] = wave < 2 ? 10 + wave : 16 + wave;
    }
    const int cpt = AMODE == AMODE_DENSE ? 1 : (X3 ? p.Cin / 32 : p.Cin / 64);
    const int cpt_rcp = (65536 + cpt - 1) / cpt;
    constexpr bool TAPIN = X3 && AMODE != AMODE_DENSE && PP_TAPINNER;
    const int ntap = p.conv == 2 ? 4 : 9;
    auto kt_split = [&](int kt, int& tap, int& c) {
        if (TAPIN) {
            c = p.conv == 2 ? (kt >> 2) : ((kt * 7282) >> 16);
            tap = kt - c * ntap;
        } else {
            tap = (kt * cpt_rcp) >> 16;
            c = kt - tap * cpt;
        }
    };
    int ka = 0, tap_ky = 0, tap_kx = 0, tap_off = 0;
    auto k_position = [&]() {
        const int kt = l_k0 + l_kt;
        if (AMODE == AMODE_DENSE) {
            ka = kt * 128;
        } else {
            int tap, c;
            kt_split(kt, tap, c);
            ka = c * 128;
            tap_ky = p.conv == 2 ? (tap >> 1) : ((tap * 21846) >> 16);
            tap_kx = tap - (p.conv == 2 ? 2 : 3) * tap_ky;
            tap_off = (tap_ky * p.Win + tap_kx) * PIX;
        }
    };
    auto w_position = [&]() {
        const int kt = l_k0 + l_kt;
        if (!TAPIN) return kt * 128;
        int tap, c;
        kt_split(kt, tap, c);
        return (tap * cpt + c) * 128;
    };
    auto prep = [&](int wtile) {
        const int tile = wtile / nsl;
        l_k0 = (wtile - tile * nsl) * nk;
        const int mt = (tile / ntn) * BM, nt = (tile % ntn) * BN;
#pragma unroll
        for (int i = 0; i < NA; ++i) {
            const int m = mt + 8 * apiece[i] + lrow;
            if (AMODE == AMODE_DENSE) {
                a_off[i] = m < p.M ? (PP_ABL == 10 ? m & 255 : m) * (p.lda * 2) + csrc * 16 : OOB;
            } else {
                const int hw = p.Hout * p.Wout;
                const int ma = PP_ABL == 10 ? (m & 255) : m;
                const int b = ma / hw, rem = ma - b * hw;
                const int yo = rem / p.Wout, xo = rem - yo * p.Wout;
                const int y0 = yo * p.stride - (p.conv == 2 ? (p.pad >> 1) : p.pad), x0 = xo * p.stride - (p.conv == 2 ? (p.pad & 1) : p.pad);
                a_off[i] = ((b * p.Hin + (y0 >> p.upsample)) * p.Win + (x0 >> p.upsample)) * PIX + csrc * 16;
                a_yx[i] = m < p.M ? ((y0 << 16) | (x0 & 0xffff)) : (int)0x80008000;
            }
        }
        b_voff = (nt + 8 * wave + lrow) * (p.Kpad * 2) + csrc * 16;
    };
    auto issue_a = [&](int i, int buf) {
        int voff = a_off[i];
        if (AMODE != AMODE_DENSE) {
            const int y0 = a_yx[i] >> 16, x0 = (int)(short)(a_yx[i] & 0xffff);
            const int yy = y0 + tap_ky, xx = x0 + tap_kx;
            const bool inb = (unsigned)yy < (unsigned)(p.Hin << p.upsample) && (unsigned)xx < (unsigned)(p.Win << p.upsample);
            int toff = tap_off;
            if (p.upsample) {
                const int dy = (tap_ky + (y0 & 1)) >> 1, dx = (tap_kx + (x0 & 1)) >> 1;
                toff = (dy * p.Win + dx) * PIX;
            }
            voff = inb ? voff + toff : OOB;
        }
        if (PP_ABL != 1) __builtin_amdgcn_raw_ptr_buffer_load_lds(rsrcA, (lptr_t)(smem + buf * BUF + apiece[i] * 1024), 16, voff, ka, 0, 0);
    };
    auto issue_b = [&](int i, int buf) {
        const int so = w_position() + i * b_step;
        if (PP_ABL != 1) __builtin_amdgcn_raw_ptr_buffer_load_lds(rsrcB, (lptr_t)(smem + buf * BUF + ABYTES + (wave + 8 * i) * 1024), 16, b_voff, so, 0, 0);
    };
    auto issue_colvec = [&](int tile) {
        if (SPLIT) return;
        const int mt = (tile / ntn) * BM + wr * HM, nt = (tile % ntn) * BN + wc * WN;
        const int bb = mt / p.rows_per_batch;
        char* slot = smem + CV + wave * 1536;
#pragma unroll
        for (int h = 0; h < 2; ++h) {
            const int c = h * 64 + lane;
            const int vb = c < WN ? (nt + c) * 4 : OOB;
            __builtin_amdgcn_raw_ptr_buffer_load_lds(rsrcBias, (lptr_t)(slot + h * 256), 4, vb, 0, 0, 0);
            __builtin_amdgcn_raw_ptr_buffer_load_lds(rsrcRb, (lptr_t)(slot + 512 + h * 256), 4, vb, bb * p.ldrb * 4, 0, 0);
            __builtin_amdgcn_raw_ptr_buffer_load_lds(rsrcRb, (lptr_t)(slot + 1024 + h * 256), 4, vb, (bb + 1) * p.ldrb * 4, 0, 0);
        }
    };
    int switched = 0;
    auto advance = [&]() {
        ++l_kt;
        switched = 0;
        if (l_kt == nk) {
            l_kt = 0;
            l_tile += G;
            if (l_tile < ntiles) {
                prep(l_tile);
                issue_colvec(l_tile);
                switched = 1;
            }
        }
    };

    const int swz = l15 & 7;
    const int a_rd0 = (wr * HM + l15) * 128 + ((g ^ swz) << 4);
    const int a_rd1 = (wr * HM + l15) * 128 + (((4 + g) ^ swz) << 4);
    const int b_rd0 = ABYTES + (wc * WN + l15) * 128 + ((g ^ swz) << 4);
    const int b_rd1 = ABYTES + (wc * WN + l15) * 128 + (((4 + g) ^ swz) << 4);

    f32x4 acc[FM][FN];
    u32x4 fa[FH], fb[FN];

    auto read_a = [&](int buf, int rd, int i0) {
#pragma unroll
        for (int i = 0; i < FH; ++i) fa[i] = *reinterpret_cast<const u32x4*>(smem + buf * BUF + rd + (i0 + i) * 2048);
    };
    auto read_b = [&](int buf, int rd) {
#pragma unroll
        for (int j = 0; j < FN; ++j) fb[j] = *reinterpret_cast<const u32x4*>(smem + buf * BUF + rd + j * 2048);
    };
    auto mfma_rows = [&](auto I0) {
        constexpr int i0 = decltype(I0)::value;
        if (PP_PRIO == 1) __builtin_amdgcn_s_setprio(1);
        if (PP_PRIO == 2) __builtin_amdgcn_s_setprio(0);
#pragma unroll
        for (int i = 0; i < FH; ++i)
#pragma unroll
            for (int j = 0; j < FN; ++j) {
                if constexpr (F8) mma_fp8(fb[j], fa[i], acc[i0 + i][j]);
                else if constexpr (TRANS) DT<T>::mma(fa[i], fb[j], acc[i0 + i][j]);
                else DT<T>::mma(fb[j], fa[i], acc[i0 + i][j]);
            }
        if (PP_PRIO == 1) __builtin_amdgcn_s_setprio(0);
        if (PP_PRIO == 2) __builtin_amdgcn_s_setprio(1);
    };
    typedef std::integral_constant<int, 0> I0_t;
    typedef std::integral_constant<int, FH> I4_t;

    const float f8_inv = F8 ? 1.0f / p.alpha : 1.0f;
    auto init_rows = [&](int tile, auto I0) {
        constexpr int i0 = decltype(I0)::value;
        if constexpr (SPLIT) {
#pragma unroll
            for (int i = i0; i < i0 + FH; ++i)
#pragma unroll
                for (int j = 0; j < FN; ++j) acc[i][j] = f32x4{0.f, 0.f, 0.f, 0.f};
            return;
        }
        const char* slot = smem + CV + wave * 1536;
        if constexpr (TRANS) {
#pragma unroll
            for (int j = 0; j < FN; ++j) {
                const float bv = *reinterpret_cast<const float*>(slot + (j * 16 + l15) * 4);
#pragma unroll
                for (int i = i0; i < i0 + FH; ++i) acc[i][j] = f32x4{bv, bv, bv, bv};
            }
            return;
        }
        const int m0 = (tile / ntn) * BM + wr * HM, n0 = (tile % ntn) * BN + wc * WN;
        const int E = (m0 / p.rows_per_batch + 1) * p.rows_per_batch - m0;
        if constexpr (RES && X3) {
            const int voff = (l15 * p.ldr + 4 * g) * 4;
#pragma unroll
            for (int i = i0; i < i0 + FH; ++i)
#pragma unroll
                for (int j = 0; j < FN; ++j)
                    acc[i][j] = __builtin_bit_cast(f32x4, __builtin_amdgcn_raw_buffer_load_b128(rsrcR, voff, ((m0 + i * 16) * p.ldr + n0 + j * 16) * 4, 0));
#pragma unroll
            for (int j = 0; j < FN; ++j) {
                const f32x4 bv = *reinterpret_cast<const f32x4*>(slot + (j * 16 + 4 * g) * 4);
                const f32x4 c0 = bv + *reinterpret_cast<const f32x4*>(slot + 512 + (j * 16 + 4 * g) * 4);
                const f32x4 c1 = bv + *reinterpret_cast<const f32x4*>(slot + 1024 + (j * 16 + 4 * g) * 4);
#pragma unroll
                for (int i = i0; i < i0 + FH; ++i) acc[i][j] += (i * 16 + l15 >= E) ? c1 : c0;
                __builtin_amdgcn_sched_barrier(0);
            }
            return;
        }
        constexpr int RB = X3 ? 1 : ((BM == 256 && BN == 320) ? 2 : FH);
#pragma unroll
        for (int ib = i0; ib < i0 + FH; ib += RB) {
            u32x2 w[(RES && !X3) ? RB : 1][(RES && !X3) ? FN : 1];
            u32x4 w4[(RES && X3) ? RB : 1][(RES && X3) ? FN : 1];
            if constexpr (RES && X3) {
                const int voff = (l15 * p.ldr + 4 * g) * 4;
#pragma unroll
                for (int i = 0; i < RB; ++i)
#pragma unroll
                    for (int j = 0; j < FN; ++j)
                        w4[i][j] = __builtin_bit_cast(u32x4, __builtin_amdgcn_raw_buffer_load_b128(rsrcR, voff, ((m0 + (ib + i) * 16) * p.ldr + n0 + j * 16) * 4, 0));
            } else if constexpr (RES) {
                const int voff = (l15 * p.ldr + 4 * g) * 2;
#pragma unroll
                for (int i = 0; i < RB; ++i)
#pragma unroll
                    for (int j = 0; j < FN; ++j)
                        w[i][j] = __builtin_bit_cast(u32x2, __builtin_amdgcn_raw_buffer_load_b64(rsrcR, voff, ((m0 + (ib + i) * 16) * p.ldr + n0 + j * 16) * 2, 0));
            }
#pragma unroll
            for (int i = ib; i < ib + RB && i < i0 + FH; ++i) {
                const int rb_off = (i * 16 + l15 >= E) ? 1024 : 512;
#pragma unroll
                for (int j = 0; j < FN; ++j) {
                    f32x4 c = *reinterpret_cast<const f32x4*>(slot + (j * 16 + 4 * g) * 4) + *reinterpret_cast<const f32x4*>(slot + rb_off + (j * 16 + 4 * g) * 4);
                    if constexpr (F8) c *= f8_inv;
                    if constexpr (RES && X3) {
                        acc[i][j] = c + __builtin_bit_cast(f32x4, w4[i - ib][j]);
                    } else if constexpr (RES) {
                        const unsigned w0 = w[i - ib][j][0], w1 = w[i - ib][j][1];
                        if constexpr (F8) {
                            acc[i][j][0] = fmaf(__uint_as_float(w0 << 16), f8_inv, c[0]);
                            acc[i][j][1] = fmaf(__uint_as_float(w0 & 0xffff0000u), f8_inv, c[1]);
                            acc[i][j][2] = fmaf(__uint_as_float(w1 << 16), f8_inv, c[2]);
                            acc[i][j][3] = fmaf(__uint_as_float(w1 & 0xffff0000u), f8_inv, c[3]);
                        } else {
                        acc[i][j][0] = c[0] + __uint_as_float(w0 << 16);
                        acc[i][j][1] = c[1] + __uint_as_float(w0 & 0xffff0000u);
                        acc[i][j][2] = c[2] + __uint_as_float(w1 << 16);
                        acc[i][j][3] = c[3] + __uint_as_float(w1 & 0xffff0000u);
                        }
// ... 477 lines not shown
```

freefine_amd/ops.py:

```python
import ctypes as CT
import math

import os
import threading

import torch

from . import _lib as L


def _dt(t):
    if t.dtype == torch.float32:
        return L.FFN_F32
    if t.dtype == torch.bfloat16:
        return L.FFN_BF16
    raise TypeError(f"unsupported dtype {t.dtype}")


def epc(dtype):
    return 4 if dtype == torch.float32 else 8


def kstage(dtype):
    return 8 * epc(dtype)


def _stream():
    return torch.cuda.current_stream().cuda_stream


def _p(t):
    return 0 if t is None else t.data_ptr()


_PROF = None


def profile_begin():
    global _PROF
    _PROF = []


def profile_end():
    global _PROF
    rec, _PROF = _PROF, None
    torch.cuda.synchronize()
    out = {}
    for name, flops, nbytes, s, e in rec:
        d = out.setdefault(name, dict(calls=0, total_ms=0.0, flops=0.0, bytes=0.0))
        d["calls"] += 1
        d["total_ms"] += s.elapsed_time(e)
        d["flops"] += flops
        d["bytes"] += nbytes
    return out


def _timed(name, flops, nbytes, fn):
    if _PROF is None:
        return fn()
    s, e = torch.cuda.Event(enable_timing=True), torch.cuda.Event(enable_timing=True)
    s.record()
    rc = fn()
    e.record()
    _PROF.append((name, flops, nbytes, s, e))
    return rc


def _tname(t):
    return "float" if t.dtype == torch.float32 else "bf16"


def _igemm_name(lib, dcode, d):
    buf = CT.create_string_buffer(160)
    lib.ffn_igemm_kernel_name(dcode, CT.byref(d), buf, 160)
    return buf.value.decode()


_GN_CHUNK_MB = float(os.environ.get("FFN_GN_CHUNK_MB", "0"))
_GN_RAW = os.environ.get("FFN_GN_RAW", "1") != "0"
_KV64 = os.environ.get("FFN_KV64", "1") != "0"
_ATTN_PRESPLIT = os.environ.get("FFN_ATTN_PRESPLIT", "1") != "0"


def _mark_x3(t, order=1):
    t._ffn_x3 = order
    return t


def is_x3(w):
    return bool(getattr(w, "_ffn_x3", 0))


def split_hi_lo(w):
    w = w.float()
    hi = w.to(torch.bfloat16)
    return hi, (w - hi.float()).to(torch.bfloat16)


def pack_linear(w, dtype, x3=False):
    n, k = w.shape
    if x3:
        assert k % 8 == 0, f"split-bf16 weights need K % 8 == 0 (K={k})"
        hi, lo = split_hi_lo(w)
        if k % 32 == 0:
            return _mark_x3(torch.stack([hi.reshape(n, k // 32, 32), lo.reshape(n, k // 32, 32)], dim=2).reshape(n, 2 * k).contiguous(), 2)
        return _mark_x3(torch.cat([hi, lo, hi], dim=1).contiguous(), 1)
    ks = kstage(dtype)
    kpad = (k + ks - 1) // ks * ks
    out = torch.zeros(n, kpad, dtype=dtype, device=w.device)
    out[:, :k] = w.to(dtype)
    return out


def pack_conv3x3(w, dtype, cin_pad=None, x3=False):
    cout, cin = w.shape[:2]
    cp = cin_pad or cin
    w2 = torch.zeros(cout, 3, 3, cp, dtype=torch.float32, device=w.device)
    w2[..., :cin] = w.permute(0, 2, 3, 1).float()
    if x3:
        assert cp % 8 == 0, f"split-bf16 conv weights need Cin % 8 == 0 (Cin={cp})"
        hi, lo = split_hi_lo(w2.reshape(cout, 9, cp))
        if cp % 32 == 0:
            return _mark_x3(torch.stack([hi.reshape(cout, 9, cp // 32, 32), lo.reshape(cout, 9, cp // 32, 32)], dim=3).reshape(cout, 18 * cp).contiguous(), 2)
        return _mark_x3(torch.cat([hi, lo, hi], dim=2).reshape(cout, 27 * cp).contiguous(), 1)
    return pack_linear(w2.reshape(cout, 9 * cp), dtype)


def pack_conv3x3_n4(w):
    assert w.shape[0] == 4 and w.shape[2:] == (3, 3)
    return w.float().permute(0, 2, 3, 1).reshape(4, -1).contiguous()


def conv3x3_n4_eligible(cout, cin):
    return cout == 4 and cin % 16 == 0 and cin <= 448 and os.environ.get("FFN_CONV_N4", "1") != "0"


def conv3x3_n4(x, w4, bias, B, H, W, Cin):
    lib = L.load()
    assert x.is_contiguous() and x.shape[-1] == Cin and x.dtype in (torch.float32, torch.bfloat16)
    out = torch.empty(B, H * W, 4, dtype=torch.float32, device=x.device)
    L.check(_timed("conv3x3_n4_kernel", 2.0 * B * H * W * 4 * 9 * Cin, x.element_size() * x.numel() + 16.0 * B * H * W,
                   lambda: lib.ffn_conv3x3_n4(_stream(), _dt(x), x.data_ptr(), w4.data_ptr(), _p(bias), out.data_ptr(), B, H, W, Cin)), "ffn_conv3x3_n4")
    return out


def up2x_eligible(cin, cout, rows):
    return cin % 64 == 0 and (cout % 256 == 0 or cout % 320 == 0) and rows >= 192


def pack_conv3x3_up2x(w, dtype, x3=False):
    assert dtype == torch.bfloat16 or x3
    cout, cin = w.shape[:2]
    wf = w.float()
    groups = {0: ((0,), (1, 2)), 1: ((0, 1), (2,))}
    out = torch.empty(4, cout, 2, 2, cin, dtype=torch.float32, device=w.device)
    for a in (0, 1):
        for b in (0, 1):
            for dy in (0, 1):
                for dx in (0, 1):
                    acc = torch.zeros(cout, cin, dtype=torch.float32, device=w.device)
                    for ky in groups[a][dy]:
                        for kx in groups[b][dx]:
                            acc += wf[:, :, ky, kx]
                    out[2 * a + b, :, dy, dx] = acc
    if x3:
        assert cin % 32 == 0
        hi, lo = split_hi_lo(out.reshape(4 * cout, 4, cin))
        return _mark_x3(torch.stack([hi.reshape(4 * cout, 4, cin // 32, 32), lo.reshape(4 * cout, 4, cin // 32, 32)], dim=3).reshape(4 * cout, 8 * cin).contiguous(), 2)
    return pack_linear(out.reshape(4 * cout, 4 * cin), dtype)


def conv3x3_up2x(x, w4, bias, B, Hin, Win, Cin, *, out=None):
    lib = L.load()
    cout = w4.shape[0] // 4
    x3 = is_x3(w4)
    per_img = Hin * Win * max(4 * cout * (4 if x3 else 2), Cin * (4 if x3 else 2))
    nb = max(1, ((1 << 30) - 1) // per_img)
    if B > nb:
        if out is None:
            out = torch.empty(B, 4 * Hin * Win, cout, dtype=torch.float32 if x3 else x.dtype, device=x.device)
        for b0 in range(0, B, nb):
            b1 = min(B, b0 + nb)
            conv3x3_up2x(x[b0:b1], w4, bias, b1 - b0, Hin, Win, Cin, out=out[b0:b1])
        return out
    if x3:
        xa = x if pair_width(x) is not None else split_pair(x, Cin)
        assert pair_width(xa) == Cin
        odt, dcode = torch.float32, L.FFN_BF16X3
    else:
        assert x.dtype == torch.bfloat16 and x.is_contiguous()
        xa, odt, dcode = x, x.dtype, L.FFN_BF16
    assert w4.shape[1] >= (8 if x3 else 4) * Cin
    y = torch.empty(B, Hin * Win, 4 * cout, dtype=odt, device=x.device)
    for c in range(4):
        a, b = c >> 1, c & 1
        d = L.IgemmDesc()
        d.A, d.W = xa.data_ptr(), w4.data_ptr() + c * cout * w4.stride(0) * w4.element_size()
        d.bias, d.rowbias, d.residual = _p(bias), None, None
        d.M, d.N, d.K, d.Kpad = B * Hin * Win, cout, 4 * Cin, w4.stride(0)
        d.lda, d.a_lo, d.x3 = (2 * Cin, 32, 2) if x3 else (Cin, 0, 0)
        d.rows_per_batch, d.ldrb = Hin * Win, 0
        d.out, d.ldo, d.ldr = y.data_ptr() + c * cout * y.element_size(), 4 * cout, 0
        d.Hin, d.Win, d.Cin, d.Hout, d.Wout = Hin, Win, Cin, Hin, Win
        d.stride, d.pad, d.upsample = 1, 2 * (1 - a) + (1 - b), 0
        d.flags, d.alpha, d.conv = 0, 1.0, 2
        d.splitk, d.ws, d.ws_bytes = 0, _workspace(x.device).data_ptr(), WS_BYTES
        if _PROF is None:
            L.check(lib.ffn_igemm(_stream(), dcode, CT.byref(d)), "ffn_igemm(conv 2x2)")
        else:
            L.check(_timed(_igemm_name(lib, dcode, d), 2.0 * d.M * cout * 4 * Cin, y.element_size() * (x.numel() + cout * 4 * Cin + d.M * cout),
                           lambda: lib.ffn_igemm(_stream(), dcode, CT.byref(d))), "ffn_igemm(conv 2x2)")
    if out is None:
        out = torch.empty(B, 4 * Hin * Win, cout, dtype=odt, device=x.device)
    out.view(B, Hin, 2, Win, 2, cout).copy_(y.view(B, Hin, Win, 2, 2, cout).permute(0, 1, 3, 2, 4, 5))
    return out


F8_ACT_SCALE = 16.0


def pack_conv3x3_f8(w, cin_pad=None):
    cout, cin = w.shape[:2]
    cp = cin_pad or (cin + 127) // 128 * 128
    w2 = torch.zeros(cout, 3, 3, cp, dtype=torch.float32, device=w.device)
    w2[..., :cin] = w.permute(0, 2, 3, 1).float()
    amax = float(w2.abs().max())
    k = math.floor(math.log2(448.0 / amax)) if amax > 0 else 0
    ws = 2.0 ** k
    q = (w2 * ws).clamp(-448.0, 448.0).to(torch.float8_e4m3fn).reshape(cout, 9 * cp).contiguous().view(torch.uint8)
    q._ffn_f8 = (cp, 1.0 / (ws * F8_ACT_SCALE))
    return q


def is_f8(w):
    return getattr(w, "_ffn_f8", None) is not None


def groupnorm_f8(x, gamma, beta, G, eps, Cp, silu=False, ws=None):
    lib = L.load()
    B, HW, Cc = x.shape
    assert x.dtype == torch.bfloat16
    out = torch.empty(B, HW, Cp, dtype=torch.uint8, device=x.device)
    out._ffn_f8_act = Cc
    partial, scale, shift = ws if ws is not None else gn_workspace(B, HW, Cc, x.device)
    call = lambda: lib.ffn_groupnorm_f8(_stream(), x.data_ptr(), out.data_ptr(), gamma.data_ptr(), beta.data_ptr(), B, HW, Cc, Cp, G, eps,
                                        L.NORM_SILU if silu else 0, F8_ACT_SCALE, partial.data_ptr(), scale.data_ptr(), shift.data_ptr())
    L.check(_timed("gn_partial+gn_finalize+gn_apply_f8", 0.0, x.numel() * 2.0 + out.numel(), call), "ffn_groupnorm_f8")
    return out


def pack_geglu(w, b, dtype, x3=False):
    f2, k = w.shape
    f = f2 // 2
    assert f % 16 == 0
    idx = torch.arange(f, device=w.device).reshape(f // 16, 16)
    order = torch.stack([idx, idx + f], dim=1).reshape(-1)
    wp = pack_linear(w[order], dtype, x3)
    bp = None if b is None else b[order].float().contiguous()
    return wp, bp


def _mark_pair(t, C):
    t._ffn_pair = C
    return t


def pair_width(x):
    return getattr(x, "_ffn_pair", None)


def split_pair(x, K=None):
    lib = L.load()
    assert x.dtype == torch.float32 and x.stride(-1) == 1
    K = K if K is not None else x.shape[-1]
    rows = x.numel() // x.shape[-1]
    ld = x.stride(-2) if x.ndim > 1 else x.shape[-1]
    out = torch.empty(*x.shape[:-1], 2 * K, dtype=torch.bfloat16, device=x.device)
    L.check(_timed("split_pair_kernel", 0.0, 8.0 * rows * K, lambda: lib.ffn_split_pair(_stream(), x.data_ptr(), out.data_ptr(), rows, K, ld)),
            "ffn_split_pair")
    return _mark_pair(out, K)


_WS = {}
WS_BYTES = 96 << 20


def _workspace(device):
    key = (device, torch.cuda.current_stream().cuda_stream)
    ws = _WS.get(key)
    if ws is None:
        ws = _WS[key] = torch.empty(WS_BYTES // 4, dtype=torch.float32, device=device)
    return ws

_TLS = threading.local()


def _invariant():
    return getattr(_TLS, "batch_invariant", False)


class batch_invariant:

    def __enter__(self):
        self.prev, _TLS.batch_invariant = _invariant(), True

    def __exit__(self, *exc):
        _TLS.batch_invariant = self.prev


def linear(x, w, bias=None, *, K=None, out=None, residual=None, rowbias=None, rows_per_batch=None, silu=False,
           geglu=False, out_f32=False, transposed_ld=None, alpha=1.0, splitk=0, out_pair=False, gelu=False, relu=False, kv64_from=None, qgelu=False):
    lib = L.load()
    K = K if K is not None else x.shape[-1]
    M = x.numel() // x.shape[-1]
    N = w.shape[0]
    d = L.IgemmDesc()
    x3 = is_x3(w)
    if x3 and pair_width(x) is not None:
        K = pair_width(x)
        M = x.numel() // x.shape[-1]
        xa = x
    else:
        xa = split_pair(x, K) if x3 else x
    dcode = L.FFN_BF16X3 if x3 else _dt(x)
    d.A, d.W = xa.data_ptr(), w.data_ptr()
    d.bias, d.rowbias, d.residual = _p(bias), _p(rowbias), _p(residual)
    d.M, d.N, d.K, d.Kpad = M, N, K, w.stride(0)
    d.lda = xa.stride(-2) if xa.ndim > 1 else xa.shape[-1]
    d.x3 = int(w._ffn_x3) if x3 else 0
    d.a_lo = (32 if d.x3 == 2 else K) if x3 else 0
    odt = torch.float32 if x3 else x.dtype
    d.rows_per_batch = rows_per_batch or M
    d.ldrb = rowbias.stride(0) if rowbias is not None else 0
    flags = 0
    n_out = N
    if silu:
        flags |= L.IG_OUT_SILU
    if gelu:
        flags |= L.IG_OUT_GELU
    if relu:
        flags |= L.IG_OUT_RELU
    if qgelu:
        flags |= L.IG_OUT_QGELU
    if geglu:
        flags |= L.IG_GEGLU
        n_out = N // 2
    if out_f32:
        flags |= L.IG_OUT_F32
    if transposed_ld is not None:
        flags |= L.IG_OUT_TRANSPOSED
        nb = M // d.rows_per_batch
        if out is None:
            alloc = torch.zeros if transposed_ld > d.rows_per_batch else torch.empty
            out = alloc(nb, N, transposed_ld, dtype=odt, device=x.device)
        d.ldo = transposed_ld
    elif out_pair:
        assert x3 and out is None
        flags |= L.IG_OUT_PAIR
        out = _mark_pair(torch.empty(*x.shape[:-1], 2 * n_out, dtype=torch.bfloat16, device=x.device), n_out)
        d.ldo = 2 * n_out
    else:
        if out is None:
            out = torch.empty(*x.shape[:-1], n_out, dtype=torch.float32 if out_f32 else odt, device=x.device)
        d.ldo = out.stride(-2) if out.ndim > 1 else n_out
    assert xa.stride(-1) == 1 and out.stride(-1) == 1 and (residual is None or residual.stride(-1) == 1), "linear: x, out and residual need contiguous columns"
    d.ldr = (residual.stride(-2) if residual.ndim > 1 else residual.shape[-1]) if residual is not None else 0
    d.out = out.data_ptr()
    if kv64_from is not None:
        assert x3 and residual is None and rowbias is None and not (silu or gelu or relu or qgelu or geglu or out_pair)
        flags |= L.IG_OUT_KV64
        d.kv64_from = int(kv64_from)
        splitk = 1
    d.flags, d.alpha, d.conv = flags, alpha, 0
    if splitk == 0 and _invariant():
        splitk = 1
    d.splitk, d.ws, d.ws_bytes = splitk, _workspace(x.device).data_ptr(), WS_BYTES
    if _PROF is None:
        L.check(lib.ffn_igemm(_stream(), dcode, CT.byref(d)), "ffn_igemm")
    else:
        esz = x.element_size()
        L.check(_timed(_igemm_name(lib, dcode, d), 2.0 * M * N * K, esz * (M * K + N * K + M * n_out),
                       lambda: lib.ffn_igemm(_stream(), dcode, CT.byref(d))), "ffn_igemm")
    return out


def conv3x3(x, w, bias, B, Hin, Win, Cin, *, stride=1, pad=1, upsample=False, out=None, residual=None, rowbias=None,
            rowbias_ld=None, out_f32=False, Hout=None, Wout=None, splitk=0, relu=False):
    lib = L.load()
    He, We = (Hin * 2, Win * 2) if upsample else (Hin, Win)
    if Hout is None:
        Hout = (He + 2 * pad - 3) // stride + 1
        Wout = (We + 2 * pad - 3) // stride + 1
    N = w.shape[0]
    d = L.IgemmDesc()
    x3 = is_x3(w)
    f8 = is_f8(w)
    if f8:
        assert x.dtype == torch.uint8 and x.shape[-1] == w._ffn_f8[0] and out_f32 is False
        Cin = x.shape[-1]
        xa = x
    elif x3 and pair_width(x) is not None:
        assert pair_width(x) == Cin
        xa = x
    else:
        xa = split_pair(x, Cin) if x3 else x
    dcode = L.FFN_FP8 if f8 else (L.FFN_BF16X3 if x3 else _dt(x))
    odt = torch.float32 if x3 else (torch.bfloat16 if f8 else x.dtype)
    d.A, d.W = xa.data_ptr(), w.data_ptr()
    d.bias, d.rowbias, d.residual = _p(bias), _p(rowbias), _p(residual)
    d.M, d.N, d.K, d.Kpad = B * Hout * Wout, N, 9 * Cin, w.shape[1]
    d.lda = 2 * Cin if x3 else Cin
    d.x3 = int(w._ffn_x3) if x3 else 0
    d.a_lo = (32 if d.x3 == 2 else Cin) if x3 else 0
    d.rows_per_batch = Hout * Wout
    d.ldrb = (rowbias_ld or rowbias.stride(0)) if rowbias is not None else 0
    if out is None:
        out = torch.empty(B, Hout * Wout, N, dtype=torch.float32 if out_f32 else odt, device=x.device)
    assert xa.is_contiguous(), "conv3x3: x must be contiguous (a column view of a wider buffer has no pixel stride the kernels could follow)"
    assert out.stride(-1) == 1 and (residual is None or residual.stride(-1) == 1), "conv3x3: out and residual need contiguous columns"
    d.out, d.ldo = out.data_ptr(), out.stride(-2)
    d.ldr = residual.stride(-2) if residual is not None else 0
    d.Hin, d.Win, d.Cin, d.Hout, d.Wout = Hin, Win, Cin, Hout, Wout
    d.stride, d.pad, d.upsample = stride, pad, 1 if upsample else 0
    d.flags, d.alpha, d.conv = (L.IG_OUT_F32 if out_f32 else 0) | (L.IG_OUT_RELU if relu else 0), (w._ffn_f8[1] if f8 else 1.0), 1
    if splitk == 0 and _invariant():
        splitk = 1
    d.splitk, d.ws, d.ws_bytes = splitk, _workspace(x.device).data_ptr(), WS_BYTES
    if _PROF is None:
        L.check(lib.ffn_igemm(_stream(), dcode, CT.byref(d)), "ffn_igemm(conv)")
    else:
        esz = x.element_size()
        k_real = 9 * getattr(x, "_ffn_f8_act", Cin)
        L.check(_timed(_igemm_name(lib, dcode, d), 2.0 * d.M * N * k_real, esz * (x.numel() + N * d.K + d.M * N),
                       lambda: lib.ffn_igemm(_stream(), dcode, CT.byref(d))), "ffn_igemm(conv)")
    return out


class AttnEntrySpec:
    __slots__ = ("q_row", "kv_row", "w_const", "w_slope", "wq", "kmask", "qsel", "flags", "hr_row")

    def __init__(self, q_row, kv_row, w_const=1.0, w_slope=0.0, wq=None, kmask=None, qsel=None, flags=0, hr_row=None):
        self.q_row, self.kv_row, self.w_const, self.w_slope = q_row, kv_row, w_const, w_slope
        self.wq, self.kmask, self.qsel, self.flags, self.hr_row = wq, kmask, qsel, flags, hr_row

    def remap(self, row_map, logical_row):
        return AttnEntrySpec(row_map[self.q_row], row_map[self.kv_row], self.w_const, self.w_slope, self.wq, self.kmask, self.qsel,
                             self.flags, logical_row if self.hr_row is None else self.hr_row)

    def pinned(self, logical_row):
        return self if self.hr_row is not None else AttnEntrySpec(self.q_row, self.kv_row, self.w_const, self.w_slope, self.wq, self.kmask, self.qsel,
                                                                  self.flags, logical_row)

    def renumber(self, ren, kv_ren=None):
        kv_ren = ren if kv_ren is None else kv_ren
        if self.q_row not in ren or self.kv_row not in kv_ren:
            raise ValueError(f"attention term (q row {self.q_row}, kv row {self.kv_row}) reaches outside the rows of this phase {sorted(ren)} / {sorted(kv_ren)}")
        return AttnEntrySpec(ren[self.q_row], kv_ren[self.kv_row], self.w_const, self.w_slope, self.wq, self.kmask, self.qsel, self.flags, self.hr_row)

    def shifted(self, base, logical_row, kv_base=None):
        return AttnEntrySpec(self.q_row + base, self.kv_row + (base if kv_base is None else kv_base), self.w_const, self.w_slope, self.wq,
                             self.kmask, self.qsel, self.flags, logical_row if self.hr_row is None else self.hr_row)


def _set_entries(d, passes, b0, nb, ptr=_p):
    for p, rows in enumerate(passes):
        for b in range(nb):
            sp = rows[b0 + b]
            e = d.e[p * L.ATT_MAXB + b]
            if sp is None:
                e.w_const = e.w_slope = 0.0
                continue
            e.q_row, e.kv_row, e.w_const, e.w_slope = sp.q_row, sp.kv_row, sp.w_const, sp.w_slope
            e.wq, e.kmask, e.qsel, e.flags = ptr(sp.wq), ptr(sp.kmask), ptr(sp.qsel), sp.flags
            hr = sp.hr_row if sp.hr_row is not None else (b0 + b if b0 else None)
            e.hr_row = 0 if hr is None else hr + 1


def _takes_kv_images(lib, d):
    probe = L.AttnDesc.from_buffer_copy(d)
    probe.kv_pair = 1
    return lib.ffn_attn_kernel_name(L.FFN_BF16X3, CT.byref(probe), CT.create_string_buffer(160), 160) == 0


def kv_images_ok(Dh, S, Sk, passes=None, nbytes=0):
    if not (_ATTN_PRESPLIT and _KV64 and nbytes < 2 ** 31 - 65536):
        return False
    lib = L.load()
    passes = passes or [[AttnEntrySpec(0, 0)]]
    Bo = len(passes[0])
    for b0 in range(0, Bo, L.ATT_MAXB):
        nb = min(L.ATT_MAXB, Bo - b0)
        d = L.AttnDesc()
        d.Bo, d.S, d.Sk, d.heads, d.D, d.npass = nb, S, Sk, 1, Dh, len(passes)
        d.ldq = d.ldk = d.ldo = Dh
        d.ldvt = Sk
        d.w_dev = 1
        _set_entries(d, passes, b0, nb, lambda t: 0 if t is None else 1)
        if not _takes_kv_images(lib, d):
            return False
    return True


_ROWSPLIT = os.environ.get("FFN_ATT_ROWSPLIT", "1") != "0"
_CUS = {}


def attn_row_split(Bo, wg_per_row, maxb, cus):
    best_n, best = min(maxb, Bo), None
    for n in range(min(maxb, Bo), 0, -1):
        full, rest = divmod(Bo, n)
        rounds = full * -(-n * wg_per_row // cus) + (-(-rest * wg_per_row // cus) if rest else 0)
        if best is None or rounds < best:
            best_n, best = n, rounds
    return best_n


def attention(q, k, vt, heads, scale, passes=None, *, Sk=None, out=None, w_dev=None, Bo=None, C=None, x3=False, out_pair=False, kv_images=False, causal=False):
    lib = L.load()
    Bq, S, _ = q.shape
    Cq = C if C is not None else q.shape[2]
    Sk = Sk if Sk is not None else k.shape[1]
    Dh = Cq // heads
    if passes is None:
        passes = [[AttnEntrySpec(b, b) for b in range(Bq)]]
    if causal:
        passes = [[None if sp is None else AttnEntrySpec(sp.q_row, sp.kv_row, sp.w_const, sp.w_slope, sp.wq, sp.kmask, sp.qsel, sp.flags | L.ATT_CAUSAL, sp.hr_row)
                   for sp in rows] for rows in passes]
    Bo = Bo if Bo is not None else len(passes[0])
    out_pair = bool(out_pair and x3 and q.dtype == torch.float32 and Dh <= 64 and out is None and Cq % 8 == 0)
    if out_pair:
        out = _mark_pair(torch.empty(Bo, S, 2 * Cq, dtype=torch.bfloat16, device=q.device), Cq)
    if out is None:
        out = torch.empty(Bo, S, Cq, dtype=q.dtype, device=q.device)
    for rows in passes:
        assert len(rows) == Bo
    esz = q.element_size()
    dcode = L.FFN_BF16X3 if (x3 and q.dtype == torch.float32) else _dt(q)
    descs = []
    chunk = L.ATT_MAXB
    if _ROWSPLIT and Bo > 1 and Dh == 64 and S >= 128 and Sk % 64 == 0 and q.is_cuda:
        di = q.device.index if q.device.index is not None else torch.cuda.current_device()
        if di not in _CUS:
            _CUS[di] = torch.cuda.get_device_properties(di).multi_processor_count
        chunk = attn_row_split(Bo, heads * -(-S // 256), L.ATT_MAXB, _CUS[di])
    for b0 in range(0, Bo, chunk):
        nb = min(chunk, Bo - b0)
        d = L.AttnDesc()
        d.q, d.k, d.vt, d.w_dev = q.data_ptr(), k.data_ptr(), vt.data_ptr(), _p(w_dev)
        d.out = out.data_ptr() + b0 * S * Cq * esz
        d.Bo, d.S, d.Sk, d.heads, d.D = nb, S, Sk, heads, Dh
        d.ldq, d.ldk, d.ldvt, d.ldo = q.stride(1), k.stride(1), vt.stride(1), (2 * Cq if out_pair else Cq)
        d.out_pair = 1 if out_pair else 0
        d.scale, d.npass = scale, len(passes)
        d.kv_pair = 1 if kv_images else 0
        _set_entries(d, passes, b0, nb)
        descs.append((b0, nb, d))
    if kv_images:
        assert dcode == L.FFN_BF16X3 and kv_images_ok(Dh, S, Sk)
    elif dcode == L.FFN_BF16X3 and _ATTN_PRESPLIT and k.stride(2) == 1 and vt.stride(2) == 1 and k.stride(0) == Sk * k.stride(1) \
            and vt.stride(0) == heads * Dh * vt.stride(1) and k.shape[0] * Sk * heads * Dh * 4 < 2 ** 31 - 65536:
        if all(_takes_kv_images(lib, d) for _, _, d in descs):
            Bk = k.shape[0]
            kp = torch.empty(Bk, Sk, 2 * heads * Dh, dtype=torch.bfloat16, device=q.device)
            vp = torch.empty(Bk, heads * Dh, 2 * Sk, dtype=torch.bfloat16, device=q.device)
            L.check(_timed("attn_presplit_kernel", 0.0, 16.0 * Bk * Sk * heads * Dh,
                           lambda: lib.ffn_attn_presplit(_stream(), k.data_ptr(), vt.data_ptr(), kp.data_ptr(), vp.data_ptr(), Bk, Sk, heads, k.stride(1), vt.stride(1))),
                    "ffn_attn_presplit")
            for _, _, d in descs:
                d.k, d.vt, d.kv_pair = kp.data_ptr(), vp.data_ptr(), 1
                d.ldk, d.ldvt = heads * Dh, Sk
    for b0, nb, d in descs:
        if _PROF is None:
            L.check(lib.ffn_attn(_stream(), dcode, CT.byref(d)), "ffn_attn")
        else:
            nterms = sum(1 for rows in passes for sp in rows[b0:b0 + nb] if sp is not None and (sp.w_const != 0.0 or sp.w_slope != 0.0))
            nbuf = CT.create_string_buffer(160)
            lib.ffn_attn_kernel_name(dcode, CT.byref(d), nbuf, 160)
            L.check(_timed(nbuf.value.decode(), 4.0 * nterms * S * Sk * Cq,
                           esz * nterms * (S * Cq + 2 * Sk * Cq) + esz * nb * S * Cq,
                           lambda: lib.ffn_attn(_stream(), dcode, CT.byref(d))), "ffn_attn")
    return out


def gn_workspace(B, HW, C, device):
    lib = L.load()
    nchunk = lib.ffn_gn_nchunk(HW)
# ... 885 lines not shown
```

freefine_amd/unet.py:

```python
import ctypes as CT
import os
import weakref

import torch

from . import _lib as L
from . import ops
from .config import UNetConfig

_GRAPH_RAW = os.environ.get("FFN_GRAPH_RAW", "1") != "0"


class _Res:
    pass


class HipUNet:
    def __init__(self, cfg: UNetConfig, state, dtype=torch.bfloat16, device="cuda:0", x3=False, fp8_conv=False):
        assert not x3 or dtype == torch.float32, "split-bf16 mode keeps fp32 activations"
        assert not fp8_conv or dtype == torch.bfloat16, "fp8 convolutions are an option of the bf16 fast mode"
        self.x3 = bool(x3)
        self.fp8_conv = bool(fp8_conv)
        self.cfg, self.dtype, self.device = cfg, dtype, torch.device(device)
        self.in_channels = cfg.in_channels
        self.hook, self.controller = "edit", None
        self._graphs = {}
        self._capture_stream = None
        self._text_bufs = {}
        self.use_graph = False
        self._row_map = None
        self._plan_cache = {}
        self._row_idx = {}
        self._reuse, self._reuse_idx, self._enc_a, self.last_boundary = None, {}, {}, None
        self._in_phase_a = False
        self._kv_ext = False
        self.last_kv = None
        self._enc_rows = 0
        self.reuse_replays = 0
        self._pack(state)

    def _f32(self, t):
        return t.detach().float().contiguous().to(self.device)

    def _lin(self, st, name, bias=True):
        w = st[name + ".weight"].to(self.device)
        if w.ndim == 4:
            w = w.reshape(w.shape[0], w.shape[1])
        return ops.pack_linear(w.float(), self.dtype, self.x3), (self._f32(st[name + ".bias"]) if bias else None), w.shape[1]

    def _conv(self, st, name, cin_pad=None):
        w = st[name + ".weight"].to(self.device)
        return ops.pack_conv3x3(w.float(), self.dtype, cin_pad, self.x3), self._f32(st[name + ".bias"]), (cin_pad or w.shape[1])

    def _resnet(self, st, p, temb_list):
        r = _Res()
        r.n1 = (self._f32(st[p + ".norm1.weight"]), self._f32(st[p + ".norm1.bias"]))
        r.n2 = (self._f32(st[p + ".norm2.weight"]), self._f32(st[p + ".norm2.bias"]))
        if self.fp8_conv:
            r.c1 = (ops.pack_conv3x3_f8(st[p + ".conv1.weight"].to(self.device).float()), self._f32(st[p + ".conv1.bias"]), st[p + ".conv1.weight"].shape[1])
            r.c2 = (ops.pack_conv3x3_f8(st[p + ".conv2.weight"].to(self.device).float()), self._f32(st[p + ".conv2.bias"]), st[p + ".conv2.weight"].shape[1])
        else:
            r.c1 = self._conv(st, p + ".conv1")
            r.c2 = self._conv(st, p + ".conv2")
        r.cout = st[p + ".conv1.weight"].shape[0]
        r.sc = self._lin(st, p + ".conv_shortcut") if (p + ".conv_shortcut.weight") in st else None
        r.temb_off = sum(w.shape[0] for w, _ in temb_list)
        temb_list.append((st[p + ".time_emb_proj.weight"].float(), st[p + ".time_emb_proj.bias"].float()))
        return r

    def _transformer(self, st, p, heads):
        t = _Res()
        t.heads = heads
        t.norm = (self._f32(st[p + ".norm.weight"]), self._f32(st[p + ".norm.bias"]))
        t.proj_in = self._lin(st, p + ".proj_in")
        t.proj_out = self._lin(st, p + ".proj_out")
        b = p + ".transformer_blocks.0"
        t.ln = [(self._f32(st[f"{b}.norm{i}.weight"]), self._f32(st[f"{b}.norm{i}.bias"])) for i in (1, 2, 3)]
        wq, wk = st[f"{b}.attn1.to_q.weight"].float(), st[f"{b}.attn1.to_k.weight"].float()
        t.C = wq.shape[0]
        t.w_qk1 = ops.pack_linear(torch.cat([wq, wk], 0).to(self.device), self.dtype, self.x3)
        t.w_v1 = ops.pack_linear(st[f"{b}.attn1.to_v.weight"].float().to(self.device), self.dtype, self.x3)
        t.o1 = self._lin(st, f"{b}.attn1.to_out.0")
        t.w_q2 = ops.pack_linear(st[f"{b}.attn2.to_q.weight"].float().to(self.device), self.dtype, self.x3)
        t.w_k2 = ops.pack_linear(st[f"{b}.attn2.to_k.weight"].float().to(self.device), self.dtype, self.x3)
        t.w_v2 = ops.pack_linear(st[f"{b}.attn2.to_v.weight"].float().to(self.device), self.dtype, self.x3)
        t.o2 = self._lin(st, f"{b}.attn2.to_out.0")
        t.ff1 = ops.pack_geglu(st[f"{b}.ff.net.0.proj.weight"].float().to(self.device), st[f"{b}.ff.net.0.proj.bias"].float().to(self.device), self.dtype, self.x3)
        t.ff2 = self._lin(st, f"{b}.ff.net.2")
        return t

    def _pack(self, st):
        cfg = self.cfg
        ch = cfg.block_out_channels
        n = len(ch)
        e = 8 if self.x3 else ops.epc(self.dtype)
        self.cin_pad = (cfg.in_channels + e - 1) // e * e
        self.conv_in = self._conv(st, "conv_in", self.cin_pad)
        self.te1 = self._lin(st, "time_embedding.linear_1")
        self.te2 = self._lin(st, "time_embedding.linear_2")
        self.freq = ops.timestep_freqs(ch[0], self.device, shift=cfg.freq_shift)
        temb_list = []
        self.down, self.up = [], []
        self.attn_calls = 0
        for i in range(n):
            blk = _Res()
            blk.res = [self._resnet(st, f"down_blocks.{i}.resnets.{j}", temb_list) for j in range(cfg.layers_per_block)]
            blk.attn = [self._transformer(st, f"down_blocks.{i}.attentions.{j}", cfg.heads[i]) for j in range(cfg.layers_per_block)] \
                if cfg.down_has_attn[i] else None
            blk.down = self._conv(st, f"down_blocks.{i}.downsamplers.0.conv") if i < n - 1 else None
            self.down.append(blk)
        self.mid = _Res()
        self.mid.res = [self._resnet(st, "mid_block.resnets.0", temb_list)]
        self.mid.attn = [self._transformer(st, "mid_block.attentions.0", cfg.heads[n - 1])]
        self.mid.res.append(self._resnet(st, "mid_block.resnets.1", temb_list))
        rev_attn = list(reversed(cfg.down_has_attn))
        for i in range(n):
            blk = _Res()
            blk.res = [self._resnet(st, f"up_blocks.{i}.resnets.{j}", temb_list) for j in range(cfg.layers_per_block + 1)]
            blk.attn = [self._transformer(st, f"up_blocks.{i}.attentions.{j}", cfg.heads[n - 1 - i]) for j in range(cfg.layers_per_block + 1)] \
                if rev_attn[i] else None
            blk.up = self._conv(st, f"up_blocks.{i}.upsamplers.0.conv") if i < n - 1 else None
            blk.up2 = None
            if blk.up is not None and (self.dtype == torch.bfloat16 or self.x3) and os.environ.get("FFN_UP2X", "1") != "0":
                wu = st[f"up_blocks.{i}.upsamplers.0.conv.weight"].to(self.device)
                if ops.up2x_eligible(wu.shape[1], wu.shape[0], 192):
                    blk.up2 = ops.pack_conv3x3_up2x(wu, self.dtype, x3=self.x3)
            self.up.append(blk)
        self.norm_out = (self._f32(st["conv_norm_out.weight"]), self._f32(st["conv_norm_out.bias"]))
        self.conv_out = self._conv(st, "conv_out")
        wco = st["conv_out.weight"]
        self.conv_out_n4 = ops.pack_conv3x3_n4(wco.to(self.device)) if ops.conv3x3_n4_eligible(wco.shape[0], wco.shape[1]) else None
        wcat = torch.cat([w for w, _ in temb_list], 0).to(self.device)
        self.temb_w = ops.pack_linear(wcat, self.dtype, self.x3)
        self.temb_b = torch.cat([b for _, b in temb_list], 0).float().to(self.device).contiguous()
        self.transformers = [t for blk in self.down if blk.attn for t in blk.attn] + self.mid.attn + \
                            [t for blk in self.up if blk.attn for t in blk.attn]
        self.num_attention_calls = 2 * len(self.transformers)
        self.t_dev = torch.zeros(1, dtype=torch.float32, device=self.device)
        self.cg_dev = torch.zeros(1, dtype=torch.float32, device=self.device)

    _INSTANCE_STATE = ("hook", "controller", "_graphs", "_capture_stream", "_text_bufs", "use_graph", "_row_map", "_plan_cache", "_row_idx", "t_dev", "cg_dev",
                       "_reuse", "_reuse_idx", "_enc_a", "last_boundary", "last_kv")

    def share(self):
        other = object.__new__(HipUNet)
        other.__dict__.update({k: v for k, v in self.__dict__.items() if k not in self._INSTANCE_STATE})
        other.hook, other.controller = "edit", None
        other._graphs, other._text_bufs, other._plan_cache, other._row_idx = {}, {}, {}, {}
        other._capture_stream = None
        other._reuse, other._reuse_idx, other._enc_a, other.last_boundary, other.last_kv = None, {}, {}, None, None
        other.use_graph, other._row_map = self.use_graph, None
        other.t_dev, other.cg_dev = torch.zeros_like(self.t_dev), torch.zeros_like(self.cg_dev)
        return other

    def set_attention_control(self, hook, controller):
        self.hook, self.controller = hook, controller
        self._graphs.clear()
        self._plan_cache.clear()

    def _ctrls(self):
        c = self.controller
        return [] if c is None else (list(c) if isinstance(c, (list, tuple)) else [c])

    def to(self, *a, **k):
        return self

    def __call__(self, sample, timestep, encoder_hidden_states=None, row_map=None, reuse=None, **kw):
        return self.forward(sample, timestep, encoder_hidden_states, row_map, reuse)

    def prepare_text(self, enc):
        key = tuple(enc.shape)
        ent = self._text_bufs.get(key)
        if ent is not None and ent["ref"]() is enc and ent["version"] == enc._version:
            return ent["kv"]
        Bt, Sk, Dm = enc.shape
        x = enc.to(self.device)
        x = ops.cast(x.float().contiguous(), self.dtype) if x.dtype != self.dtype else x.contiguous()
        ld = (Sk + 7) // 8 * 8
        old = ent["kv"] if ent is not None else [(None, None)] * len(self.transformers)
        kv = []
        for t, (ko, vo) in zip(self.transformers, old):
            k = ops.linear(x, t.w_k2, None, K=Dm, out=ko)
            vt = ops.linear(x, t.w_v2, None, K=Dm, rows_per_batch=Sk, transposed_ld=ld, out=vo)
            kv.append((k, vt))
        self._text_bufs[key] = dict(ref=weakref.ref(enc), version=enc._version, kv=kv)
        return kv

    def join_block(self, min_tca_block=None):
        n = len(self.up)
        tb = len([t for blk in self.down if blk.attn for t in blk.attn]) + 1
        first = []
        for blk in self.up:
            first.append(tb)
            tb += len(blk.attn) if blk.attn else 0
        if min_tca_block is None:
            return n - 1, first[n - 1]
        j = max([i for i in range(n) if first[i] <= min_tca_block], default=0)
        return j, first[j]

    def forward(self, sample, timestep, enc, row_map=None, reuse=None):
        sample = sample.to(self.device, torch.float32).contiguous()
        B = sample.shape[0]
        self._row_map = tuple(row_map) if row_map is not None else None
        self._enc_rows = enc.shape[0]
        self._reuse = self._prepare_reuse(reuse, B, enc)
        self.t_dev.fill_(float(timestep))
        ctrls = self._ctrls()
        assert not ctrls or B % len(ctrls) == 0, f"batch {B} is not a multiple of the {len(ctrls)} batched images"
        if ctrls and ctrls[0].context_guidance is not None:
            assert all(c.context_guidance == ctrls[0].context_guidance for c in ctrls), "batched images share one schedule"
            self.cg_dev.fill_(float(ctrls[0].context_guidance))
        text_kv = self.prepare_text(enc)
        ru = self._reuse
        if ru is not None and ru["mode"] in ("replay", "replay_kv"):
            ru["text_kv_a"] = self.prepare_text(ru["enc_a"])
            self.reuse_replays += 1
        if not self.use_graph:
            return self._expand(self._run(sample, text_kv))
# ... 157 lines not shown
        merged = [[] for _ in range(npass)]
        if is_cross and sel is not None and tsel is not None:
            Bt = len(tsel)
        else:
            Bt = (self._enc_rows // K) if (is_cross and sel is None and self._enc_rows % K == 0) else Bp
        for i, plan in enumerate(plans):
            ps = plan["passes"] if plan["passes"] is not None else [[ops.AttnEntrySpec(b, b) for b in range(Bp)]]
            for p in range(npass):
                rows = ps[p] if p < len(ps) else [None] * Bp
                for pr, e in enumerate(rows):
                    if e is not None:
                        ref_j = e.kv_row - self.REF_KV
                        e = e.shifted(i * Bp, rep[pr], i * Bt)
                        if ref_j >= 0:
                            e.kv_row = K * Bp + i * nr + ref_j
                    merged[p].append(e)
        out = dict(kind=plans[0]["kind"], passes=merged, needs_cg=any(p["needs_cg"] for p in plans),
                   branch="+".join(sorted({p.get("branch", "") for p in plans})))
        if any("ref_rows" in p for p in plans):
            out["ref_rows"] = [i * Bp + r for i, p in enumerate(plans) for r in p.get("ref_rows", list(range(Bp)))]
        return out

    def _call_list(self, H, W):
        cfg = self.cfg
        n = len(cfg.block_out_channels)
        out = []
        h, w = H, W
        for i in range(n):
            if cfg.down_has_attn[i]:
                out += [(x, "down", h * w, cfg.heads[i]) for _ in range(cfg.layers_per_block) for x in (False, True)]
            if i < n - 1:
                h, w = (h + 1) // 2, (w + 1) // 2
        out += [(False, "mid", h * w, cfg.heads[n - 1]), (True, "mid", h * w, cfg.heads[n - 1])]
        rev_attn = list(reversed(cfg.down_has_attn))
        for i in range(n):
            if rev_attn[i]:
                out += [(x, "up", h * w, cfg.heads[n - 1 - i]) for _ in range(cfg.layers_per_block + 1) for x in (False, True)]
            if i < n - 1:
                h, w = 2 * h, 2 * w
        return out

    def _ctrl_key(self, B, H, W):
        ru = self._reuse
        key = [self.hook, B, H, W, self._row_map,
               None if ru is None or ru["mode"] == "record" else (ru["mode"], ru.get("join"), ru.get("kv_from"), ru["ref"], ru.get("text_sel"), bool(ru.get("drop_tail")))]
        for c in self._ctrls():
            mv = tuple((m.data_ptr(), m._version) if torch.is_tensor(m) else None
                       for m in (c.fg_retain_mask, c.fg_ref_mask, c.local_edit_region, c.src_masks, c.tgt_masks))
            key.append((id(c), c.use_tca, c.use_style_align, c.local_edit, c.method, tuple(c.layer_idx), tuple(c.tca_scope),
                        tuple(c.style_align_scope), c.cur_att_layer, c.prompt_length, c._mask_epoch, mv))
        return tuple(key)

    def _plan_all(self, B, H, W):
        ctrls = self._ctrls()
        if not ctrls:
            return None
        key = self._ctrl_key(B, H, W)
        hit = self._plan_cache.get(key)
        if hit is not None:
            for c in ctrls:
                c.cur_step += 1 if c.cur_att_layer == 0 else 0
                if c.cur_att_layer != 0:
                    for _ in range(self.num_attention_calls):
                        c._tick()
            return hit
        fp = self._plan_all_slow(B, H, W)
        if len(self._plan_cache) > 64:
            self._plan_cache.clear()
        self._plan_cache[key] = fp
        return fp

    def _plan_all_slow(self, B, H, W):
        fps = []
        ru = self._reuse
        join_tb = self.join_block_tb(ru["join"]) if (ru is not None and ru["mode"] == "replay") else -1
        kv_from = ru["kv_from"] if (ru is not None and ru["mode"] == "replay_kv") else None
        calls = self._call_list(H, W)
        drop = ru is not None and ru["mode"] == "replay" and bool(ru.get("drop_tail"))
        for ci, (is_cross, place, S, heads) in enumerate(calls):
            self._in_phase_a = ci // 2 < join_tb
            self._kv_ext = kv_from is not None and not is_cross and ci // 2 >= kv_from
            if drop and ci == len(calls) - 1:
                self._in_phase_a = True
            plan = self._plan(is_cross, place, B, S, heads)
            if drop and ci == len(calls) - 2:
                plan = self._without_ref_queries(plan, B)
            if plan["passes"] is None:
                fps.append(0)
                continue
            rows = tuple(tuple(None if e is None else (e.q_row, e.kv_row, e.w_const, e.w_slope, e.flags, e.hr_row,
                                                       0 if e.wq is None else e.wq.data_ptr(),
                                                       0 if e.kmask is None else e.kmask.data_ptr(),
                                                       0 if e.qsel is None else e.qsel.data_ptr()) for e in r) for r in plan["passes"])
            fps.append((plan["kind"], plan["needs_cg"], rows))
        self._in_phase_a = self._kv_ext = False
        return (self.hook, tuple(fps))

    def join_block_tb(self, join):
        tb = len([t for blk in self.down if blk.attn for t in blk.attn]) + 1
        for blk in self.up[:join]:
            tb += len(blk.attn) if blk.attn else 0
        return tb

    def _capture(self, sample, text_kv, sig):
        ctrls = self._ctrls()
        state = [(c.cur_att_layer, c.cur_step) for c in ctrls]
        x_static = sample.clone()
        ru = self._reuse
        ref_in = None
        if ru is not None and ru["mode"] == "replay":
            ref_in = [t.clone() for t in ru["state"]]
            ru["state_run"] = ref_in
        if ru is not None and ru["mode"] == "replay_kv":
            ref_in = ru["static"] = []
            ru["static_bufs"] = []
        self._run(x_static, text_kv)
        if ru is not None and ru["mode"] == "replay_kv":
            ru["static_ready"] = True
        for c, st in zip(ctrls, state):
            c.cur_att_layer, c.cur_step = st
        torch.cuda.synchronize()
        graph = torch.cuda.CUDAGraph()
        if self._capture_stream is None:
            self._capture_stream = torch.cuda.Stream(device=x_static.device)
        with torch.cuda.graph(graph, stream=self._capture_stream):
            out = self._run(x_static, text_kv)
        rec = ru is not None and ru["mode"] == "record"
        g = dict(graph=graph, x=x_static, out=out, ref_in=ref_in, ref_bufs=ru.get("static_bufs") if ru is not None else None,
                 boundary=self.last_boundary if rec else None, kv=self.last_kv if rec else None, device=x_static.device.index)
        if ru is not None:
            for k in ("state_run", "static", "static_bufs", "static_ready"):
                ru.pop(k, None)
        self._graphs[sig] = g
        return g

    def _gn(self, x, gb, eps, silu):
        B, HW, C = x.shape
        return ops.groupnorm(x, gb[0], gb[1], self.cfg.norm_num_groups, eps, silu=silu, pair=self.x3)

    def _gn_conv_in(self, x, gb, w):
        if ops.is_f8(w):
            return ops.groupnorm_f8(x, gb[0], gb[1], self.cfg.norm_num_groups, self.cfg.norm_eps, w._ffn_f8[0], silu=True)
        return self._gn(x, gb, self.cfg.norm_eps, True)

    def _resblock(self, r, x, B, H, W, temb_all, out=None):
        cin = x.shape[-1]
        if r.sc is not None and self.x3 and not ops.is_f8(r.c1[0]) and ops.pair_width(x) is None and x.dtype == torch.float32:
            h, x = ops.groupnorm_pair_raw(x, r.n1[0], r.n1[1], self.cfg.norm_num_groups, self.cfg.norm_eps, silu=True)
        else:
            h = self._gn_conv_in(x, r.n1, r.c1[0])
        rb = temb_all[:, r.temb_off:r.temb_off + r.cout]
        h = ops.conv3x3(h, r.c1[0], r.c1[1], B, H, W, cin, rowbias=rb, rowbias_ld=temb_all.shape[1])
        h = self._gn_conv_in(h, r.n2, r.c2[0])
        if r.sc is not None:
            x = ops.linear(x, r.sc[0], r.sc[1], K=cin)
        return ops.conv3x3(h, r.c2[0], r.c2[1], B, H, W, r.cout, residual=x, out=out)

    def _without_ref_queries(self, plan, B):
        keep = self._reuse["idx_a_list"]
        passes = plan["passes"] if plan["passes"] is not None else [[ops.AttnEntrySpec(b, b) for b in range(B)]]
        pin = lambda e, r: e if (e is None or e.hr_row is not None) else ops.AttnEntrySpec(e.q_row, e.kv_row, e.w_const, e.w_slope, e.wq, e.kmask, e.qsel, e.flags, r)
        out = dict(plan)
        out["passes"] = [[pin(rows[r], r) for r in keep] for rows in passes]
        return out

    def _self_plan(self, t, place, B, S, drop_ref_queries=False):
        if self.controller is None:
            return dict(kind="plain", needs_cg=False, passes=[[ops.AttnEntrySpec(r, r, hr_row=r) for r in self._reuse["idx_a_list"]]]) if drop_ref_queries else None
        plan = self._plan(False, place, B, S, t.heads)
        if drop_ref_queries:
            assert plan["kind"] != "shared_kv"
            plan = self._without_ref_queries(plan, B)
        return plan

    def _attention(self, t, is_cross, place, q, k, vt, ldq_view, B, S, Sk, plan=None, kv_images=False):
        D = t.C // t.heads
        scale = D ** -0.5
        if is_cross and self.controller is not None:
            plan = self._plan(is_cross, place, B, S, t.heads)
        if plan is None:
            return ops.attention(q, k, vt, t.heads, scale, None, Sk=Sk, C=t.C, x3=self.x3, out_pair=self.x3, kv_images=kv_images)
        if plan["kind"] == "shared_kv":
            assert not kv_images
            rr = plan["ref_rows"]
            kc = k[..., :t.C] if k.shape[-1] != t.C else k
            k2 = torch.cat([kc, kc[rr]], dim=1).contiguous()
            vt2 = torch.cat([vt[..., :Sk], vt[rr][..., :Sk]], dim=2).contiguous()
            return ops.attention(q, k2, vt2, t.heads, scale, plan["passes"], Sk=2 * Sk, C=t.C, x3=self.x3, out_pair=self.x3)
        return ops.attention(q, k, vt, t.heads, scale, plan["passes"], Sk=Sk, C=t.C, w_dev=self.cg_dev if plan["needs_cg"] else None, x3=self.x3,
                             out_pair=self.x3, kv_images=kv_images)

    def _kv_buffers(self, B, S, C, ldv):
        ru = self._reuse
        i = ru["cursor"]
        ru["cursor"] = i + 1
        if ru.get("static_ready"):
            return ru["static_bufs"][i]
        k_ref, vt_ref = ru["state"][2 * i], ru["state"][2 * i + 1]
        nr = k_ref.shape[0]
        assert tuple(k_ref.shape) == (nr, S, C) and tuple(vt_ref.shape) == (nr, C, ldv), (tuple(k_ref.shape), tuple(vt_ref.shape), (S, C, ldv))
        qk = torch.empty(B + nr, S, 2 * C, dtype=self.dtype, device=self.device)
        vt = torch.empty(B + nr, C, ldv, dtype=self.dtype, device=self.device)
        qk[B:, :, C:].copy_(k_ref)
        vt[B:].copy_(vt_ref)
        if ru.get("static") is not None:
            ru["static_bufs"].append((qk, vt))
            ru["static"] += [qk[B:, :, C:], vt[B:]]
        return qk, vt

    def _transformer_block(self, t, x, B, H, W, place, kv_text, out=None, drop=None, tb=0):
        S, C = H * W, t.C
        res0 = x
        ru = self._reuse
        h = self._gn(x, t.norm, 1e-6, False)
        h = ops.linear(h, t.proj_in[0], t.proj_in[1], K=C)
        y = ops.layernorm(h, *t.ln[0], pair=self.x3)
        ldv = (S + 7) // 8 * 8
        if ru is not None and ru["mode"] == "replay_kv" and tb >= ru["kv_from"]:
            qk, vt = self._kv_buffers(B, S, C, ldv)
            ops.linear(y, t.w_qk1, None, K=C, out=qk[:B])
            ops.linear(y, t.w_v1, None, K=C, rows_per_batch=S, transposed_ld=ldv, out=vt[:B])
            self._kv_ext = True
            a = self._attention(t, False, place, qk[:B], qk[..., C:], vt, 2 * C, B, S, S, plan=self._self_plan(t, place, B, S))
            self._kv_ext = False
        else:
            plan = self._self_plan(t, place, B, S, drop_ref_queries=drop is not None)
            rec = ru is not None and ru["mode"] == "record" and ru.get("kv_from") is not None and tb >= ru["kv_from"]
            img = self.x3 and not rec and (plan is None or plan["kind"] != "shared_kv") and \
                ops.kv_images_ok(C // t.heads, S, S, None if plan is None else plan["passes"], B * max(S * 2 * C, C * ldv) * 4)
            qk = ops.linear(y, t.w_qk1, None, K=C, kv64_from=C if img else None)
            vt = ops.linear(y, t.w_v1, None, K=C, rows_per_batch=S, transposed_ld=ldv, kv64_from=0 if img else None)
            if rec:
                self.last_kv.append((qk[..., C:], vt))
            a = self._attention(t, False, place, qk, qk[..., C:], vt, 2 * C, B, S, S, plan=plan, kv_images=img)
        if drop is not None:
            idx, kv_text = drop
            h, res0, B = h.index_select(0, idx), res0.index_select(0, idx), idx.shape[0]
            self._in_phase_a = True
        h = ops.linear(a, t.o1[0], t.o1[1], K=C, residual=h)
        y = ops.layernorm(h, *t.ln[1], pair=self.x3)
        q = ops.linear(y, t.w_q2, None, K=C)
        k2, vt2 = kv_text
        a = self._attention(t, True, place, q, k2, vt2, C, B, S, k2.shape[1])
        h = ops.linear(a, t.o2[0], t.o2[1], K=C, residual=h)
        y = ops.layernorm(h, *t.ln[2], pair=self.x3)
        y = ops.linear(y, t.ff1[0], t.ff1[1], K=C, geglu=True, out_pair=self.x3)
        h = ops.linear(y, t.ff2[0], t.ff2[1], K=4 * C, residual=h, out_pair=self.x3 and C % 32 == 0)
        return ops.linear(h, t.proj_out[0], t.proj_out[1], K=C, residual=res0, out=out)

    def _run(self, sample, text_kv, stop_up=None):
        cfg = self.cfg
        B, _, H, W = sample.shape
        dt = self.dtype
        ru = self._reuse
        replay = ru is not None and ru["mode"] == "replay"
        record = ru is not None and ru["mode"] == "record"
        replay_kv = ru is not None and ru["mode"] == "replay_kv"
        BB = B
        if replay:
            sample = sample.index_select(0, ru["idx_a"])
            B = sample.shape[0]
            text_kv = list(ru["text_kv_a"][:self.join_block_tb(ru["join"])]) + list(text_kv[self.join_block_tb(ru["join"]):])
        if replay_kv:
            sample = sample.index_select(0, ru["idx_a"])
            B = sample.shape[0]
            text_kv = ru["text_kv_a"]
            ru["cursor"] = 0
        if record and ru.get("kv_from") is not None:
            self.last_kv = []
        self._in_phase_a = replay
        ti = iter(text_kv)
        tb = 0
        te = ops.timestep_embed(self.t_dev, self.freq, BB, dt, flip=cfg.flip_sin_to_cos)
        e1 = ops.linear(te, self.te1[0], self.te1[1], K=self.te1[2], silu=True)
        e2 = ops.linear(e1, self.te2[0], self.te2[1], K=self.te2[2], silu=True)
        temb_all = ops.linear(e2, self.temb_w, self.temb_b, K=self.te2[0].shape[0], out_f32=True)
        temb_full = temb_all
        temb_all = temb_all[:B]
        x = ops.pack_nchw(sample, list(range(B)), self.cin_pad, dt)
        x = ops.conv3x3(x, self.conv_in[0], self.conv_in[1], B, H, W, self.cin_pad)
        skips = [(x, H, W)]
        n = len(self.down)
        for i, blk in enumerate(self.down):
            for j, r in enumerate(blk.res):
                x = self._resblock(r, x, B, H, W, temb_all)
                if blk.attn:
                    x = self._transformer_block(blk.attn[j], x, B, H, W, "down", next(ti), tb=tb)
                    tb += 1
                skips.append((x, H, W))
            if blk.down is not None:
                C = x.shape[-1]
                x = ops.conv3x3(x, blk.down[0], blk.down[1], B, H, W, C, stride=2)
                H, W = (H + 1) // 2, (W + 1) // 2
                skips.append((x, H, W))
        x = self._resblock(self.mid.res[0], x, B, H, W, temb_all)
        x = self._transformer_block(self.mid.attn[0], x, B, H, W, "mid", next(ti), tb=tb)
        tb += 1
        def cat_dst(C1, HW):
            return ops.cat_dst((B, HW), C1, skips[-1][0].shape[-1], dt, x.device) if skips else None
        x = self._resblock(self.mid.res[1], x, B, H, W, temb_all, out=cat_dst(self.mid.res[1].cout, H * W))
        for i, blk in enumerate(self.up):
            if ru is not None and ru.get("join") is not None and i == ru["join"]:
                if record:
                    self.last_boundary = [x] + [s for s, _, _ in reversed(skips)]
                if replay:
                    state = ru.get("state_run") or ru["state"]
# ... 42 lines not shown
```

include/freefine_hip.h:

```cpp
#ifndef FREEFINE_HIP_H
#define FREEFINE_HIP_H
#include <stdint.h>
#ifdef __cplusplus
extern "C" {
#endif

enum { FFN_F32 = 0, FFN_BF16 = 1, FFN_BF16X3 = 2 ,
       FFN_FP8 = 3  };
enum { FFN_OK = 0, FFN_EINVAL = -22, FFN_ENOSYS = -38, FFN_EHIP = -5, FFN_ENOSPC = -28 };

int ffn_version(void);
const char* ffn_last_error(void);
int ffn_device_info(int device, char* name, int name_len);
int ffn_graph_launch(void* stream, void* graph_exec);

enum {
    FFN_IG_OUT_SILU = 1 << 0,
    FFN_IG_OUT_F32 = 1 << 1,
    FFN_IG_GEGLU = 1 << 2,
    FFN_IG_OUT_TRANSPOSED = 1 << 3,
    FFN_IG_OUT_PAIR = 1 << 4,
    FFN_IG_OUT_GELU = 1 << 5,
    FFN_IG_OUT_KV64 = 1 << 7,
    FFN_IG_OUT_RELU = 1 << 6,
    FFN_IG_OUT_QGELU = 1 << 8
};
typedef struct ffn_igemm_desc {
    const void* A;
    const void* W;
    void* out;
    const float* bias;
    const float* rowbias;
    const void* residual;
    int M, N, K, Kpad;
    int lda, ldo, ldr, ldrb;
    int rows_per_batch;
    int Hin, Win, Cin, Hout, Wout, stride, pad, upsample;
    int flags;
    float alpha;
    int conv;
    int splitk;
    void* ws;
    long ws_bytes;
    int a_lo;
    int x3;
    int f8;
    int kv64_from;
} ffn_igemm_desc;
int ffn_igemm(void* stream, int dtype, const ffn_igemm_desc* d);
int ffn_split_pair(void* stream, const float* src, void* dst, long rows, int C, int ld_src);
int ffn_conv3x3_n4(void* stream, int dtype, const void* x, const float* w, const float* bias, float* out, int B, int H, int W, int Cin);
int ffn_groupnorm_f8(void* stream, const void* x_bf16, void* y_e4m3, const float* gamma, const float* beta, int B, int HW, int C, int Cp,
                     int G, float eps, int silu, float qscale, float* partial_ws, float* scale, float* shift);
int ffn_igemm_tune(void* stream, int dtype, const ffn_igemm_desc* d);
int ffn_igemm_tune_entry_ints(void);
int ffn_igemm_tune_export(int* buf, int max_entries);
int ffn_igemm_tune_import(const int* buf, int n_entries);
int ffn_igemm_tune_clear(void);
int ffn_igemm_tune_enable(int on);
int ffn_igemm_tune_stamp(void);
int ffn_igemm_num_configs(void);
int ffn_igemm_force_config(int cfg);
int ffn_igemm_kernel_name(int dtype, const ffn_igemm_desc* d, char* buf, int len);

#define FFN_ATT_MAXP 4
#define FFN_ATT_MAXB 16
enum { FFN_ATT_HEAD_RULE = 1, FFN_ATT_UNIFORM_SEL1 = 2, FFN_ATT_UNIFORM_SEL0 = 4,
       FFN_ATT_CAUSAL = 8  };
typedef struct ffn_attn_entry {
    int q_row, kv_row;
    float w_const, w_slope;
    const float* wq;
    const uint8_t* kmask;
    const uint8_t* qsel;
    int flags;
    int hr_row;
} ffn_attn_entry;
typedef struct ffn_attn_desc {
    const void* q;
    const void* k;
    const void* vt;
    void* out;
    const float* w_dev;
    int Bo, S, Sk, heads, D;
    int ldq, ldk, ldvt, ldo;
    float scale;
    int npass;
    int out_pair;
    int kv_pair;
    ffn_attn_entry e[FFN_ATT_MAXP * FFN_ATT_MAXB];
} ffn_attn_desc;
int ffn_attn(void* stream, int dtype, const ffn_attn_desc* d);
int ffn_attn_presplit(void* stream, const float* k, const float* vt, void* k_pair, void* vt_pair, int rows, int Sk, int heads, int ldk, int ldvt);
int ffn_attn_variant(int dtype, int D, int* dp, int* qf);
int ffn_attn_kernel_name(int dtype, const ffn_attn_desc* d, char* buf, int len);

enum { FFN_ELT_RELU = 0, FFN_ELT_ADD = 1, FFN_ELT_GELU = 2 };
int ffn_eltwise(void* stream, int dtype, int op, const void* a, const void* b, void* y, long n);
int ffn_resize_bilinear(void* stream, int dtype, const void* x, void* y, int B, int Hin, int Win, int Hout, int Wout, int C, int relu);

typedef struct ffn_splat_xform {
    float center[3], translate[3], rotate[9] , scale[3];
    float tan_half_fov;
} ffn_splat_xform;
int ffn_splat_lift(void* stream, const float* depth, const int* idx, float* pts, int n, int W, int H, float fx, float fy);
int ffn_splat_project(void* stream, const float* pts, float* proj, int n, const ffn_splat_xform* x);
int ffn_splat_bin(void* stream, int fill, const float* proj, int n, float radius, int W, int H, int* counts, const int* offs, int* list);
int ffn_splat_render(void* stream, const float* proj, const float* rgb, const int* offs, const int* list, float radius, int K, int W, int H,
                     float* image, int* idx_sum, uint8_t* covered);
int ffn_splat_ids(void* stream, const float* proj, const int* offs, const int* list, float radius, int K, int W, int H, int* ids);
int ffn_splat_correspond(void* stream, const float* proj, const int* idx, int n, int W, int H, const int* ids, int K, float* map, uint8_t* visible);

int ffn_geo_project(void* stream, const float* depth, const float* pose, float focal, int H, int W, float* tcoords, float* proj);
int ffn_splat_composite(void* stream, const float* proj, const float* feat, const int* offs, const int* list, float radius, float tau, int K,
                        int C, int H, int W, int round_half, float* out);
int ffn_mesh_cover(void* stream, const float* tcoords, const uint8_t* mask, int H, int W, uint8_t* cover);

enum { FFN_NORM_SILU = 1, FFN_NORM_OUT_PAIR = 2 };
int ffn_gn_nchunk(int HW);
int ffn_gn_fused(int B, int HW, int C, int G);
int ffn_gn_stats(void* stream, int dtype, const void* x, const float* gamma, const float* beta, int B, int HW, int C, int G,
                 float eps, float* partial_ws, float* scale, float* shift);
int ffn_gn_apply(void* stream, int dtype, const void* x, void* y, const float* scale, const float* shift, int B, int HW,
                 int C, int silu);
int ffn_groupnorm(void* stream, int dtype, const void* x, void* y, const float* gamma, const float* beta, int B, int HW, int C, int G,
                  float eps, int silu, float* partial_ws, float* scale, float* shift);
int ffn_groupnorm_pair_raw(void* stream, const void* x, void* y_pair, void* yraw_pair, const float* gamma, const float* beta, int B, int HW, int C, int G,
                           float eps, int silu, float* partial_ws, float* scale, float* shift);
int ffn_layernorm(void* stream, int dtype, const void* x, void* y, const float* gamma, const float* beta, int M, int C,
                  float eps);
int ffn_layernorm_pair(void* stream, const float* x, void* y, const float* gamma, const float* beta, int M, int C, float eps);
int ffn_softmax_rows(void* stream, int dtype, const void* x, void* y, long M, int N, float scale);
int ffn_pool_layernorm(void* stream, int dtype, const void* x, const int* ids, void* y, const float* gamma, const float* beta, int N, int S, int C, float eps,
                       int pair);
int ffn_cosine_rows(void* stream, const float* a, const float* b, float* out, int B, int P, int b_rows);

int ffn_cfg_masked(void* stream, const float* eps_u, const float* eps_c, const float* mask, float cfg, float* eps, long n,
                   int HW);
int ffn_ddim_inv_step(void* stream, const float* eps, const float* x, float c_bt, float c_at, float c_an, float c_bn,
                      float* x_next, float* pred_x0, long n);
typedef struct ffn_ctrl_step_desc {
    const float* eps;
    const float* x;
    const float* noise;
    const float* m;
    const float* om;
    float* x_prev;
    float* pred_x0;
    float c_bt, c_at, c_ap, c_dir;
    float c_dirm[8], stdv[8];
    int row_masked[8];
    int rows, CHW, HW;
} ffn_ctrl_step_desc;
int ffn_ddim_ctrl_step(void* stream, const ffn_ctrl_step_desc* d);

typedef struct ffn_pack_desc {
    const float* src;
    void* dst;
    int src_row[16];
    int B, Cl, CP, HW;
} ffn_pack_desc;
int ffn_pack_nchw(void* stream, int dtype, const ffn_pack_desc* d);
int ffn_nhwc_to_nchw_f32(void* stream, const float* src, float* dst, int B, int HW, int C, int ld);
int ffn_concat(void* stream, int dtype, const void* a, const void* b, void* out, long rows, int C1, int C2);
int ffn_timestep_embed(void* stream, int dtype, const float* t_dev, const float* freq, void* out, int B, int half, int flip);
int ffn_transpose(void* stream, int dtype, const void* src, void* dst, int B, int R, int C, int ld_src, int ld_dst);
int ffn_cast(void* stream, int src_dtype, int dst_dtype, const void* src, void* dst, long n);
int ffn_embed_tokens(void* stream, int dtype, const int* ids, const float* table, const float* pos, void* out, long M, int S, int C, int V);
int ffn_image_to_nhwc(void* stream, int dtype, const uint8_t* img, void* dst, long npix, int CP);
int ffn_nhwc_to_image(void* stream, int dtype, const void* src, float* dst, int B, int HW, int ld);

typedef struct ffn_dift_desc {
    const void* src;
    const void* tgt;
    const int* kps;
    void* ws;
    int* out_rc;
    float* out_cos;
    long ws_bytes;
    long es;
    int dtype, E, C, ld, h, w, H, W, K;
} ffn_dift_desc;
int ffn_dift_match(void* stream, const ffn_dift_desc* d);
long ffn_dift_workspace_bytes(int C, int h, int w, int K);

#define FFN_SIFT_MAX_SIDE 16384
#define FFN_SIFT_MAX_TAPS 63
int ffn_sift_base(void* stream, const uint8_t* img, float* out, int H, int W, int C);
int ffn_gauss_blur_f32(void* stream, const float* src, float* dst, float* tmp, int H, int W, const float* taps, int T);
int ffn_decimate2_f32(void* stream, const float* src, float* dst, int H, int W);
int ffn_sift_extrema(void* stream, const float* gauss, float* dog, int h, int w, int* cand, int cap, int* counter, int* count);
int ffn_sift_refine_orient(void* stream, const float* dog, const float* gauss, int h, int w, int octave, const int* cand, int n, float* out);
int ffn_sift_describe(void* stream, const float* gauss, int h, int w, int octave, const float* kp, int n, uint8_t* desc, float* raw);
int ffn_knn2_u8(void* stream, const uint8_t* des1, int n1, const uint8_t* des2, int n2, int* idx, int* dist);

#define FFN_IMGPREP_MAX_SIDE 4096
int ffn_resize_pil_bilinear_u8(void* stream, const uint8_t* src, uint8_t* dst, uint8_t* scratch, int B, int H, int W, int oh, int ow, const int* hbounds,
                               const int* hcoef, int hksize, const int* vbounds, const int* vcoef, int vksize);
int ffn_vit_patch_rows(void* stream, int dtype, const uint8_t* src, const float* lut, void* out, int B, int H, int W, int patch, int ldo);
int ffn_vit_patch_rows_pair(void* stream, const uint8_t* src, const float* lut, void* out, int B, int H, int W, int patch, int K);
// ... 52 lines not shown
```

Measured before the change: 2.032.

## Fold resnet 1x1 shortcut GEMM into conv2 implicit GEMM as a dense K tail

Adds a conv-plus-dense-tail mode to the ping-pong implicit GEMM kernel. After the 3x3 conv K-stages it keeps accumulating over a second A operand (the block input) against the concatenated 1x1 shortcut weights. Resnet blocks with a shortcut then run one kernel instead of a separate linear plus a residual read, which removes a launch, the shortcut output round trip and the residual load. In exchange it adds per-load branching on a second buffer resource, restricts tile and split choices, and needs a one-time kernel-name probe to confirm the fused kernel was selected.

Result: no change. 2.033 (median of 3 runs) (+0.0%).

```diff
diff --git a/freefine_amd/_lib.py b/freefine_amd/_lib.py
--- a/freefine_amd/_lib.py
+++ b/freefine_amd/_lib.py
@@ -29,6 +29,7 @@
         ("flags", C.c_int), ("alpha", C.c_float), ("conv", C.c_int),
         ("splitk", C.c_int), ("ws", C.c_void_p), ("ws_bytes", C.c_long),
         ("a_lo", C.c_int), ("x3", C.c_int), ("f8", C.c_int), ("kv64_from", C.c_int),
+        ("A2", C.c_void_p), ("lda2", C.c_int), ("K2", C.c_int),
     ]
 
 
diff --git a/freefine_amd/csrc/capi.hip b/freefine_amd/csrc/capi.hip
--- a/freefine_amd/csrc/capi.hip
+++ b/freefine_amd/csrc/capi.hip
@@ -8,7 +8,7 @@
 
 __thread char g_err[512] = "";
 
-extern "C" int ffn_version(void) { return 14; }
+extern "C" int ffn_version(void) { return 15; }
 extern "C" const char* ffn_last_error(void) { return g_err; }
 extern "C" int ffn_device_info(int device, char* name, int name_len) {
     hipDeviceProp_t prop;
diff --git a/freefine_amd/csrc/capi_igemm.hip b/freefine_amd/csrc/capi_igemm.hip
--- a/freefine_amd/csrc/capi_igemm.hip
+++ b/freefine_amd/csrc/capi_igemm.hip
@@ -55,6 +55,13 @@
         if (d.x3 != 2 || d.K % 96 != 0 || d.a_lo != 32) return false;
     } else if (d.K % 64 != 0) return false;
     if (nkt < 2 || d.N % bn != 0 || d.M < bm) return false;
+    if (d.A2) {
+        if (!((bn == 320 && (bm == 192 || bm == 256)) || (bn == 256 && bm == 256))) return false;
+        if (d.x3 != 2 || d.conv != 1 || d.stride != 1 || d.pad != 1 || d.upsample || d.residual) return false;
+        if (d.flags & (FFN_IG_GEGLU | FFN_IG_OUT_PAIR | FFN_IG_OUT_KV64 | FFN_IG_OUT_TRANSPOSED)) return false;
+        if (d.K2 < 32 || d.K2 % 32 != 0 || d.lda2 < 2 * d.K2 || d.lda2 % 8 != 0) return false;
+        if ((long)(d.M + 256) * d.lda2 * 2 >= lim) return false;
+    }
     const int osz = d.x3 ? 4 : 2;
     if (splitk > 1) {
         if (!can_split(d) || nkt % splitk != 0 || nkt / splitk < 2 || (long)splitk * d.M * d.N * 4 > d.ws_bytes || (long)splitk * d.M * d.N * 4 >= lim) return false;
@@ -71,7 +78,8 @@
     if (d.conv) {
         const int pix = d.x3 ? d.lda : d.Cin;
         const int cpt = d.x3 ? d.Cin / 32 : d.Cin / 64;
-        if (d.Cin % (d.x3 ? 32 : 64) != 0 || d.K != (d.conv == 2 ? 4 : 9) * (d.x3 ? 3 : 1) * d.Cin) return false;
+        if (d.Cin % (d.x3 ? 32 : 64) != 0 || d.K != (d.conv == 2 ? 4 : 9) * (d.x3 ? 3 : 1) * d.Cin + (d.A2 ? 3 * d.K2 : 0)) return false;
+        if (d.A2 && nkt >= 32768) return false;
         if (d.x3 && d.lda != 2 * d.Cin) return false;
         if (d.conv == 2 && (d.f8 || d.stride != 1 || d.upsample)) return false;
         if ((long)cpt * 9 * cpt >= 65536) return false;
@@ -172,8 +180,31 @@
     if (bm == 128 && bn == 128) cfg = (!d.conv && nk <= 24 && !d.x3 && !d.f8) ? CFG_128x128_16 : CFG_128x128_8;
     return IgChoice{cfg, sk};
 }
+static constexpr int kPpSplitBelow = 160;
+static IgChoice tail_choice(const ffn_igemm_desc& d) {
+    int bm;
+    if (d.splitk <= 1)
+        for (int n : {320, 256})
+            if ((bm = pp_tile_height(d, n, {256, 192}, 3))) return IgChoice{pp_cfg(bm, n), 1};
+    if (d.splitk != 1)
+        for (int n : {320, 256})
+            for (int h : {256, 192}) {
+                if (d.N % n != 0) continue;
+                const long pt = (long)((d.M + h - 1) / h) * (d.N / n);
+                if (pt >= kPpSplitBelow) continue;
+                for (int sgo = d.splitk > 1 ? d.splitk : (int)((384 + pt - 1) / pt); sgo >= 2; --sgo) {
+                    if ((d.splitk > 1 || (d.K / 96) / sgo >= 6) && pp_ok(d, h, n, sgo)) return IgChoice{pp_cfg(h, n), sgo};
+                    if (d.splitk > 1) break;
+                }
+            }
+    for (int n : {320, 256})
+        for (int h : {256, 192})
+            if (pp_ok(d, h, n)) return IgChoice{pp_cfg(h, n), 1};
+    return IgChoice{-1, 1};
+}
 static IgChoice heuristic_choice(const ffn_igemm_desc& d) {
     int bm, bn;
+    if (d.A2) return tail_choice(d);
     if (d.conv == 2 && conv2_tile(d, &bm, &bn)) return IgChoice{pp_cfg(bm, bn), 1};
     if (d.splitk <= 1) {
         for (int n : {320, 256})
@@ -184,7 +215,7 @@
 }
 
 struct TuneKey {
-    int M, N, K, conv, Cin, Hin, Win, stride, upsample, flags, lda, splitk, ptrs, wslabs, rpb, alpha1, ldo, pad, Hout, Wout, Kpad, ldr, dtype;
+    int M, N, K, conv, Cin, Hin, Win, stride, upsample, flags, lda, splitk, ptrs, wslabs, rpb, alpha1, ldo, pad, Hout, Wout, Kpad, ldr, dtype, K2, lda2;
     bool operator==(const TuneKey& o) const { return memcmp(this, &o, sizeof(TuneKey)) == 0; }
 };
 struct TuneKeyHash {
@@ -209,6 +240,7 @@
     k.rpb = d.rows_per_batch;
     k.alpha1 = d.alpha == 1.0f;
     k.ldo = d.ldo;
+    if (d.A2) { k.K2 = d.K2; k.lda2 = d.lda2; }
     return k;
 }
 static std::mutex g_tune_mu;
@@ -218,7 +250,6 @@
     static const bool on = [] { const char* e = getenv("FFN_IGEMM_TUNE"); return !(e && atoi(e) == 0); }();
     return on && g_tune_runtime;
 }
-static constexpr int kPpSplitBelow = 160;
 static int candidates_for(const ffn_igemm_desc& d, IgChoice* out, int cap) {
     int n = 0;
     const IgChoice h = heuristic_choice(d);
@@ -228,7 +259,7 @@
     for (int cfg = 0; cfg < CFG_COUNT; ++cfg) {
         const IgCfgInfo& c = kCfg[cfg];
         if ((d.x3 || d.f8) && !x3_cfg(cfg)) continue;
-        if (d.conv == 2 && !is_pp_cfg(cfg)) continue;
+        if ((d.conv == 2 || d.A2) && !is_pp_cfg(cfg)) continue;
         if ((cfg == CFG_128x320 || cfg == CFG_128x160 || cfg == CFG_192x320) && (d.flags & FFN_IG_GEGLU)) continue;
         if (is_halo_cfg(cfg)) {
             const int hb = halo_bytes_for(d, c.bm);
@@ -324,7 +355,7 @@
     p->f32 = dtype == FFN_F32;
     p->x3 = d.x3 != 0;
     p->f8 = d.f8 != 0;
-    p->amode = d.conv ? AMODE_CONV3 : AMODE_DENSE;
+    p->amode = d.conv ? (d.A2 ? AMODE_CONV3_TAIL : AMODE_CONV3) : AMODE_DENSE;
     p->swap = !(d.flags & FFN_IG_OUT_TRANSPOSED);
     p->reduce_f32 = p->f32 || p->x3;
     p->splitk = 1;
@@ -339,6 +370,7 @@
         REQUIRE(!(p->x3 || p->f8) || x3_cfg(ch->cfg), "igemm: configuration %d is not built for split-bf16 / fp8 problems", ch->cfg);
         const IgCfgInfo& c = kCfg[ch->cfg];
         p->kind = is_halo_cfg(ch->cfg) ? IG_HALO : (is_pp_cfg(ch->cfg) ? IG_PP : IG_RING);
+        REQUIRE(!d.A2 || p->kind == IG_PP, "igemm: a dense tail (A2) runs on the ping-pong tiles only, not on configuration %d", ch->cfg);
         p->bm = c.bm; p->bn = c.bn; p->nwm = c.nwm; p->nwn = c.nwn;
         p->splitk = ch->splitk;
         p->block = dim3(64 * c.nwm * c.nwn);
@@ -437,11 +469,22 @@
 #undef FFN_PP
     return fail(FFN_EINVAL, "igemm: no %d x %d ping-pong tile of this form", p.bm, p.bn);
 }
+static int launch_pp_tail(const IgemmPlan& p, hipStream_t s, const ffn_igemm_desc& d) {
+#define FFN_PP_TAIL(BM_, BN_)                                                                                                               \
+    if (p.bm == BM_ && p.bn == BN_ && !p.res && !p.geglu)                                                                                   \
+        return p.split ? igemm_launch(p, igemm_pp_kernel<BM_, BN_, AMODE_CONV3_TAIL, false, false, true, false, true, false>, s, d, p.splitk) \
+                       : igemm_launch(p, igemm_pp_kernel<BM_, BN_, AMODE_CONV3_TAIL, false, false, false, false, true, false>, s, d, p.splitk)
+    FFN_PP_TAIL(192, 320);
+    FFN_PP_TAIL(256, 320);
+    FFN_PP_TAIL(256, 256);
+#undef FFN_PP_TAIL
+    return fail(FFN_EINVAL, "igemm: no %d x %d ping-pong tile for a convolution with a dense tail", p.bm, p.bn);
+}
 static int igemm_run(hipStream_t s, int dtype, const ffn_igemm_desc& d, const IgChoice* ch) {
     IgemmPlan p;
     int rc = igemm_plan(dtype, d, ch, &p);
     if (rc) return rc;
-    const bool conv = p.amode == AMODE_CONV3;
+    const bool conv = p.amode != AMODE_DENSE;
     switch (p.kind) {
     case IG_RING:
         if (p.f32) rc = conv ? launch_ring<float, AMODE_CONV3, true>(p, s, d) : (p.swap ? launch_ring<float, AMODE_DENSE, true>(p, s, d) : launch_ring<float, AMODE_DENSE, false>(p, s, d));
@@ -462,7 +505,8 @@
         break;
     case IG_PP:
     case IG_PP_TRANS:
-        if (p.x3) rc = conv ? launch_pp<AMODE_CONV3, true>(p, s, d) : launch_pp<AMODE_DENSE, true>(p, s, d);
+        if (p.amode == AMODE_CONV3_TAIL) rc = p.x3 ? launch_pp_tail(p, s, d) : fail(FFN_EINVAL, "igemm: a dense tail (A2) needs split-bf16 operands");
+        else if (p.x3) rc = conv ? launch_pp<AMODE_CONV3, true>(p, s, d) : launch_pp<AMODE_DENSE, true>(p, s, d);
         else if (p.f8) rc = launch_pp<AMODE_CONV3, false, true>(p, s, d);
         else rc = conv ? launch_pp<AMODE_CONV3>(p, s, d) : launch_pp<AMODE_DENSE>(p, s, d);
         break;
@@ -508,7 +552,7 @@
     return igemm_run(s, dtype, d, &best);
 }
 static constexpr int kTuneEntryInts = (int)(sizeof(TuneKey) / sizeof(int)) + 3;
-static constexpr int kTuneStamp = 0x67780000 ^ (950 << 4) ^ ((int)sizeof(TuneKey) << 8) ^ CFG_COUNT ^ (4 << 24);
+static constexpr int kTuneStamp = 0x67780000 ^ (950 << 4) ^ ((int)sizeof(TuneKey) << 8) ^ CFG_COUNT ^ (5 << 24);
 extern "C" int ffn_igemm_tune_entry_ints(void) { return kTuneEntryInts; }
 extern "C" int ffn_igemm_tune_stamp(void) { return kTuneStamp; }
 extern "C" int ffn_igemm_tune_clear(void) {
@@ -556,6 +600,16 @@
 }
 static int igemm_validate(int dtype, const ffn_igemm_desc& d) {
     REQUIRE(dtype == FFN_F32 || dtype == FFN_BF16 || dtype == FFN_BF16X3 || dtype == FFN_FP8, "igemm: bad dtype %d", dtype);
+    if (d.A2) {
+        REQUIRE(dtype == FFN_BF16X3 && d.x3 == 2, "igemm: a dense tail (A2) needs FFN_BF16X3 with blocked operands (dtype=%d, x3=%d)", dtype, d.x3);
+        REQUIRE(d.conv == 1 && d.stride == 1 && d.pad == 1 && d.upsample == 0, "igemm: a dense tail (A2) follows a 3x3 / stride 1 / pad 1 convolution without upsample (conv=%d, stride=%d, pad=%d, upsample=%d)",
+                d.conv, d.stride, d.pad, d.upsample);
+        REQUIRE(!d.residual && !(d.flags & (FFN_IG_GEGLU | FFN_IG_OUT_TRANSPOSED | FFN_IG_OUT_PAIR | FFN_IG_OUT_KV64)),
+                "igemm: a dense tail (A2) excludes a residual and the GEGLU / transposed / pair / KV64 outputs (flags=%d)", d.flags);
+        REQUIRE(d.K2 >= 32 && d.K2 % 32 == 0 && d.lda2 >= 2 * d.K2 && d.lda2 % 8 == 0, "igemm: a dense tail needs K2 %% 32 == 0, K2 >= 32, lda2 >= 2 K2, lda2 %% 8 == 0 (K2=%d, lda2=%d)", d.K2, d.lda2);
+        REQUIRE(d.N % 256 == 0 || d.N % 320 == 0, "igemm: a dense tail (A2) needs N %% 256 == 0 or N %% 320 == 0 (N=%d)", d.N);
+        REQUIRE(d.Cin > 0 && d.K == 9 * d.Cin + d.K2, "igemm: conv + dense tail K=%d != 9*Cin + K2 = %d", d.K, 9 * d.Cin + d.K2);
+    }
     if (dtype == FFN_FP8) {
         REQUIRE(d.conv && d.Cin > 0 && d.Cin % 16 == 0 && d.K == 9 * d.Cin && d.Kpad >= d.K && d.Kpad % 16 == 0 && d.lda == d.Cin,
                 "igemm(fp8): 3x3 convolutions with Cin %% 16 == 0 only (Cin=%d, K=%d, Kpad=%d, lda=%d)", d.Cin, d.K, d.Kpad, d.lda);
@@ -593,7 +647,7 @@
             REQUIRE(conv2_tile(igemm_view(dtype, d), &bm, &bn), "igemm: 2x2 convolution M=%d N=%d Cin=%d fits no ping-pong tile (Cin %% 64 (split-bf16: 32), N %% 256 / 320, M >= 192)", d.M, d.N, d.Cin);
         } else {
             REQUIRE(d.conv == 1, "igemm: conv=%d", d.conv);
-            REQUIRE(d.K == 9 * d.Cin, "igemm: conv K=%d != 9*Cin=%d", d.K, 9 * d.Cin);
+            REQUIRE(d.K == 9 * d.Cin + (d.A2 ? d.K2 : 0), "igemm: conv K=%d != 9*Cin=%d", d.K, 9 * d.Cin);
         }
         REQUIRE(d.stride == 1 || d.stride == 2, "igemm: stride %d", d.stride);
         REQUIRE(d.upsample == 0 || d.upsample == 1, "igemm: upsample %d", d.upsample);
@@ -642,6 +696,8 @@
         REQUIRE(d.ldo >= nout, "igemm: ldo=%d must be >= the %d output columns", d.ldo, nout);
     }
     if (d.residual) REQUIRE(d.ldr >= d.N, "igemm: ldr=%d must be >= N=%d", d.ldr, d.N);
+    if (d.A2) REQUIRE(d.M > 0 && d.Hout > 0 && d.Wout > 0 && tail_choice(igemm_view(dtype, d)).cfg >= 0,
+                      "igemm: conv + dense tail M=%d N=%d Cin=%d K2=%d fits no ping-pong tile (M >= 192, every operand below 2 GiB)", d.M, d.N, d.Cin, d.K2);
     return FFN_OK;
 }
 static bool tuned_family(int dtype, const ffn_igemm_desc& d) { return dtype != FFN_F32 && !(d.flags & FFN_IG_OUT_TRANSPOSED); }
@@ -681,6 +737,7 @@
     if ((dtype == FFN_BF16X3 || dtype == FFN_F32) && d0->residual) REQUIRE(aligned16(d0->residual), "igemm: fp32 residual must be 16-byte aligned");
     if ((dtype == FFN_BF16 || dtype == FFN_FP8) && d0->residual)
         REQUIRE((reinterpret_cast<uintptr_t>(d0->residual) & 7) == 0, "igemm%s: bf16 residual must be 8-byte aligned", dtype == FFN_FP8 ? "(fp8)" : "");
+    if (d0->A2) REQUIRE(aligned16(d0->A2), "igemm: A2 must be 16-byte aligned");
     if (d0->ws) REQUIRE(aligned16(d0->ws) && d0->ws_bytes >= 0, "igemm%s: workspace must be 16-byte aligned", dtype == FFN_FP8 ? "(fp8)" : "");
     hipStream_t s = reinterpret_cast<hipStream_t>(stream);
     const ffn_igemm_desc d = igemm_view(dtype, *d0);
diff --git a/freefine_amd/csrc/igemm.h b/freefine_amd/csrc/igemm.h
--- a/freefine_amd/csrc/igemm.h
+++ b/freefine_amd/csrc/igemm.h
@@ -3,7 +3,7 @@
 #include "common.h"
 #include "../../include/freefine_hip.h"
 
-enum { AMODE_DENSE = 0, AMODE_CONV3 = 1 };
+enum { AMODE_DENSE = 0, AMODE_CONV3 = 1, AMODE_CONV3_TAIL = 2  };
 enum { IG_OUT_SILU = FFN_IG_OUT_SILU, IG_OUT_F32 = FFN_IG_OUT_F32, IG_GEGLU = FFN_IG_GEGLU, IG_OUT_TRANSPOSED = FFN_IG_OUT_TRANSPOSED, IG_OUT_PAIR = FFN_IG_OUT_PAIR,
        IG_OUT_GELU = FFN_IG_OUT_GELU, IG_OUT_RELU = FFN_IG_OUT_RELU, IG_OUT_KV64 = FFN_IG_OUT_KV64, IG_OUT_QGELU = FFN_IG_OUT_QGELU };
 __device__ __forceinline__ float ig_activation(float x, int flags) {
diff --git a/freefine_amd/csrc/igemm_p8.h b/freefine_amd/csrc/igemm_p8.h
--- a/freefine_amd/csrc/igemm_p8.h
+++ b/freefine_amd/csrc/igemm_p8.h
@@ -1,6 +1,7 @@
 #pragma once
 #include <type_traits>
 #include "igemm.h"
+#include "igemm_tail_map.h"
 
 #ifndef PP_PRIO
 #define PP_PRIO 1
@@ -52,6 +53,7 @@
     constexpr int OSZ = (X3 && !GEGLU) ? 4 : 2;
     constexpr int OOB = (int)0x80000000;
     static_assert((BM == 256 || BM == 192) && (BN == 256 || BN == 320 || (BN == 128 && BM == 256 && X3 && AMODE == AMODE_CONV3 && !GEGLU && !SPLIT && !TRANS)), "tiles built for this kernel");
+    static_assert(AMODE != AMODE_CONV3_TAIL || (X3 && !RES && !GEGLU && !TRANS && !F8 && PP_TAPINNER), "conv + dense tail: split-bf16, plain or split-K epilogue");
     static_assert(!GEGLU || FN % 2 == 0, "GEGLU pairs hidden / gate column blocks inside a wave");
 
     extern __shared__ __attribute__((aligned(16))) char smem[];
@@ -78,6 +80,8 @@
     const int PIX = X3 ? p.lda * 2 : p.Cin * 2;
     const long a_bytes = AMODE == AMODE_DENSE ? (long)p.M * p.lda * 2 : (long)(p.M / (p.Hout * p.Wout)) * p.Hin * p.Win * PIX;
     const __amdgpu_buffer_rsrc_t rsrcA = __builtin_amdgcn_make_buffer_rsrc(const_cast<void*>(p.A), 0, (int)a_bytes, 0x00020000);
+    constexpr bool TAIL = AMODE == AMODE_CONV3_TAIL;
+    const __amdgpu_buffer_rsrc_t rsrcA2 = __builtin_amdgcn_make_buffer_rsrc(const_cast<void*>(p.A2), 0, TAIL ? (int)((long)p.M * p.lda2 * 2) : 0, 0x00020000);
     const __amdgpu_buffer_rsrc_t rsrcB = __builtin_amdgcn_make_buffer_rsrc(const_cast<void*>(p.W), 0, (int)((long)p.N * p.Kpad * 2), 0x00020000);
     const __amdgpu_buffer_rsrc_t rsrcBias = __builtin_amdgcn_make_buffer_rsrc(const_cast<float*>(p.bias), 0, p.bias ? p.N * 4 : 0, 0x00020000);
     const int nbatch = (p.M + p.rows_per_batch - 1) / p.rows_per_batch;
@@ -91,6 +95,7 @@
     int l_k0 = 0;
     int a_off[NA];
     int a_yx[NA];
+    int a2_base = 0, l_mt = 0;
     int b_voff;
     const int b_step = 64 * p.Kpad * 2;
     int apiece[NA];
@@ -105,8 +110,13 @@
     const int cpt_rcp = (65536 + cpt - 1) / cpt;
     constexpr bool TAPIN = X3 && AMODE != AMODE_DENSE && PP_TAPINNER;
     const int ntap = p.conv == 2 ? 4 : 9;
+    int tail = 0;
     auto kt_split = [&](int kt, int& tap, int& c) {
-        if (TAPIN) {
+        if constexpr (TAIL) {
+            const PpTailStage st = pp_tail_stage(kt, cpt, 0);
+            tap = st.tap;
+            c = st.chunk;
+        } else if (TAPIN) {
             c = p.conv == 2 ? (kt >> 2) : ((kt * 7282) >> 16);
             tap = kt - c * ntap;
         } else {
@@ -123,6 +133,7 @@
             int tap, c;
             kt_split(kt, tap, c);
             ka = c * 128;
+            if constexpr (TAIL) tail = kt >= 9 * cpt;
             tap_ky = p.conv == 2 ? (tap >> 1) : ((tap * 21846) >> 16);
             tap_kx = tap - (p.conv == 2 ? 2 : 3) * tap_ky;
             tap_off = (tap_ky * p.Win + tap_kx) * PIX;
@@ -131,6 +142,7 @@
     auto w_position = [&]() {
         const int kt = l_k0 + l_kt;
         if (!TAPIN) return kt * 128;
+        if constexpr (TAIL) return pp_tail_stage(kt, cpt, 0).wcol * 2;
         int tap, c;
         kt_split(kt, tap, c);
         return (tap * cpt + c) * 128;
@@ -154,6 +166,10 @@
                 a_yx[i] = m < p.M ? ((y0 << 16) | (x0 & 0xffff)) : (int)0x80008000;
             }
         }
+        if constexpr (TAIL) {
+            l_mt = mt;
+            a2_base = (mt + lrow) * (p.lda2 * 2) + csrc * 16;
+        }
         b_voff = (nt + 8 * wave + lrow) * (p.Kpad * 2) + csrc * 16;
     };
     auto issue_a = [&](int i, int buf) {
@@ -168,6 +184,13 @@
                 toff = (dy * p.Win + dx) * PIX;
             }
             voff = inb ? voff + toff : OOB;
+        }
+        if constexpr (TAIL) {
+            const int v2 = l_mt + 8 * apiece[i] + lrow < p.M ? a2_base + apiece[i] * (p.lda2 * 16) : OOB;
+            voff = tail ? v2 : voff;
+            const __amdgpu_buffer_rsrc_t rs = tail ? rsrcA2 : rsrcA;
+            __builtin_amdgcn_raw_ptr_buffer_load_lds(rs, (lptr_t)(smem + buf * BUF + apiece[i] * 1024), 16, voff, ka, 0, 0);
+            return;
         }
         if (PP_ABL != 1) __builtin_amdgcn_raw_ptr_buffer_load_lds(rsrcA, (lptr_t)(smem + buf * BUF + apiece[i] * 1024), 16, voff, ka, 0, 0);
     };
diff --git a/freefine_amd/csrc/igemm_tail_map.h b/freefine_amd/csrc/igemm_tail_map.h
--- /dev/null
+++ b/freefine_amd/csrc/igemm_tail_map.h
@@ -0,0 +1,30 @@
+#pragma once
+#if defined(__HIPCC__)
+#define PP_TAIL_HD __host__ __device__ __forceinline__
+#else
+#define PP_TAIL_HD inline
+#endif
+
+struct PpTailStage {
+    int src;
+    int tap;
+    int chunk;
+    int wcol;
+};
+PP_TAIL_HD PpTailStage pp_tail_stage(int kt, int cpt, int cpt2) {
+    (void)cpt2;
+    PpTailStage s;
+    const int n9 = 9 * cpt;
+    if (kt < n9) {
+        s.src = 0;
+        s.chunk = (kt * 7282) >> 16;
+        s.tap = kt - 9 * s.chunk;
+        s.wcol = (s.tap * cpt + s.chunk) * 64;
+    } else {
+        s.src = 1;
+        s.tap = 0;
+        s.chunk = kt - n9;
+        s.wcol = kt * 64;
+    }
+    return s;
+}
diff --git a/freefine_amd/ops.py b/freefine_amd/ops.py
--- a/freefine_amd/ops.py
+++ b/freefine_amd/ops.py
@@ -124,6 +124,13 @@
             return _mark_x3(torch.stack([hi.reshape(cout, 9, cp // 32, 32), lo.reshape(cout, 9, cp // 32, 32)], dim=3).reshape(cout, 18 * cp).contiguous(), 2)
         return _mark_x3(torch.cat([hi, lo, hi], dim=2).reshape(cout, 27 * cp).contiguous(), 1)
     return pack_linear(w2.reshape(cout, 9 * cp), dtype)
+
+
+def pack_conv3x3_shortcut(w2, w_sc):
+    cout, cin = w_sc.shape[:2]
+    assert w2.shape[0] == cout and w2.shape[1] == cout and cout % 32 == 0 and cin % 32 == 0
+    full = torch.cat([pack_conv3x3(w2, torch.float32, x3=True), pack_linear(w_sc.reshape(cout, cin).float(), torch.float32, x3=True)], dim=1).contiguous()
+    return _mark_x3(full, 2), _mark_x3(full[:, :18 * cout], 2), _mark_x3(full[:, 18 * cout:], 2)
 
 
 def pack_conv3x3_n4(w):
@@ -385,7 +392,7 @@
 
 
 def conv3x3(x, w, bias, B, Hin, Win, Cin, *, stride=1, pad=1, upsample=False, out=None, residual=None, rowbias=None,
-            rowbias_ld=None, out_f32=False, Hout=None, Wout=None, splitk=0, relu=False):
+            rowbias_ld=None, out_f32=False, Hout=None, Wout=None, splitk=0, relu=False, a2=None, k2=0, probe=False):
     lib = L.load()
     He, We = (Hin * 2, Win * 2) if upsample else (Hin, Win)
     if Hout is None:
@@ -408,17 +415,20 @@
     odt = torch.float32 if x3 else (torch.bfloat16 if f8 else x.dtype)
     d.A, d.W = xa.data_ptr(), w.data_ptr()
     d.bias, d.rowbias, d.residual = _p(bias), _p(rowbias), _p(residual)
-    d.M, d.N, d.K, d.Kpad = B * Hout * Wout, N, 9 * Cin, w.shape[1]
+    d.M, d.N, d.K, d.Kpad = B * Hout * Wout, N, 9 * Cin + (k2 if a2 is not None else 0), w.stride(0)
+    if a2 is not None:
+        assert x3 and pair_width(a2) == k2 and a2.stride(-1) == 1
+        d.A2, d.lda2, d.K2 = a2.data_ptr(), a2.stride(-2), k2
     d.lda = 2 * Cin if x3 else Cin
     d.x3 = int(w._ffn_x3) if x3 else 0
     d.a_lo = (32 if d.x3 == 2 else Cin) if x3 else 0
     d.rows_per_batch = Hout * Wout
     d.ldrb = (rowbias_ld or rowbias.stride(0)) if rowbias is not None else 0
-    if out is None:
+    if out is None and not probe:
         out = torch.empty(B, Hout * Wout, N, dtype=torch.float32 if out_f32 else odt, device=x.device)
     assert xa.is_contiguous(), "conv3x3: x must be contiguous (a column view of a wider buffer has no pixel stride the kernels could follow)"
-    assert out.stride(-1) == 1 and (residual is None or residual.stride(-1) == 1), "conv3x3: out and residual need contiguous columns"
-    d.out, d.ldo = out.data_ptr(), out.stride(-2)
+    assert (out is None or out.stride(-1) == 1) and (residual is None or residual.stride(-1) == 1), "conv3x3: out and residual need contiguous columns"
+    d.out, d.ldo = (out.data_ptr(), out.stride(-2)) if out is not None else (0, N)
     d.ldr = residual.stride(-2) if residual is not None else 0
     d.Hin, d.Win, d.Cin, d.Hout, d.Wout = Hin, Win, Cin, Hout, Wout
     d.stride, d.pad, d.upsample = stride, pad, 1 if upsample else 0
@@ -426,12 +436,16 @@
     if splitk == 0 and _invariant():
         splitk = 1
     d.splitk, d.ws, d.ws_bytes = splitk, _workspace(x.device).data_ptr(), WS_BYTES
+    if probe:
+        buf = CT.create_string_buffer(160)
+        return buf.value.decode() if lib.ffn_igemm_kernel_name(dcode, CT.byref(d), buf, 160) == 0 else None
     if _PROF is None:
         L.check(lib.ffn_igemm(_stream(), dcode, CT.byref(d)), "ffn_igemm(conv)")
     else:
         esz = x.element_size()
         k_real = 9 * getattr(x, "_ffn_f8_act", Cin)
-        L.check(_timed(_igemm_name(lib, dcode, d), 2.0 * d.M * N * k_real, esz * (x.numel() + N * d.K + d.M * N),
+        k_real += d.K2
+        L.check(_timed(_igemm_name(lib, dcode, d), 2.0 * d.M * N * k_real, esz * (x.numel() + (a2.numel() if a2 is not None else 0) + N * d.K + d.M * N),
                        lambda: lib.ffn_igemm(_stream(), dcode, CT.byref(d))), "ffn_igemm(conv)")
     return out
 
diff --git a/freefine_amd/unet.py b/freefine_amd/unet.py
--- a/freefine_amd/unet.py
+++ b/freefine_amd/unet.py
@@ -37,6 +37,8 @@
         self.last_kv = None
         self._enc_rows = 0
         self.reuse_replays = 0
+        self.fold_shortcut = True
+        self._fold_ok = {}
         self._pack(state)
 
     def _f32(self, t):
@@ -64,6 +66,12 @@
             r.c2 = self._conv(st, p + ".conv2")
         r.cout = st[p + ".conv1.weight"].shape[0]
         r.sc = self._lin(st, p + ".conv_shortcut") if (p + ".conv_shortcut.weight") in st else None
+        r.c2f = None
+        if r.sc is not None and self.x3 and not self.fp8_conv and r.cout % 32 == 0 and r.sc[2] % 32 == 0:
+            full, w2, wsc = ops.pack_conv3x3_shortcut(st[p + ".conv2.weight"].to(self.device).float(), st[p + ".conv_shortcut.weight"].to(self.device).float())
+            r.c2f = (full, (r.c2[1] + r.sc[1]).contiguous(), r.cout)
+            r.c2 = (w2, r.c2[1], r.c2[2])
+            r.sc = (wsc, r.sc[1], r.sc[2])
         r.temb_off = sum(w.shape[0] for w, _ in temb_list)
         temb_list.append((st[p + ".time_emb_proj.weight"].float(), st[p + ".time_emb_proj.bias"].float()))
         return r
@@ -527,6 +535,18 @@
         rb = temb_all[:, r.temb_off:r.temb_off + r.cout]
         h = ops.conv3x3(h, r.c1[0], r.c1[1], B, H, W, cin, rowbias=rb, rowbias_ld=temb_all.shape[1])
         h = self._gn_conv_in(h, r.n2, r.c2[0])
+        if r.sc is not None and r.c2f is not None and self.fold_shortcut:
+            xa = x if ops.pair_width(x) is not None else ops.split_pair(x, cin)
+            args = dict(out=out, a2=xa, k2=cin, splitk=1 if ops._invariant() else 0)
+            key = (id(r), B, H, W, None if out is None else out.stride(-2), xa.stride(-2), args["splitk"])
+            ok = self._fold_ok.get(key)
+            if ok is None:
+                name = ops.conv3x3(h, r.c2f[0], r.c2f[1], B, H, W, r.cout, probe=True, **args)
+                targs = name[name.find("<") + 1:name.rfind(">")].split(", ") if name is not None and name.startswith("void igemm_pp_kernel<") else None
+                ok = self._fold_ok[key] = targs is not None and targs[2] == "2" and targs[5] == "true"
+            if ok:
+                return ops.conv3x3(h, r.c2f[0], r.c2f[1], B, H, W, r.cout, **args)
+            x = xa
         if r.sc is not None:
             x = ops.linear(x, r.sc[0], r.sc[1], K=cin)
         return ops.conv3x3(h, r.c2[0], r.c2[1], B, H, W, r.cout, residual=x, out=out)
diff --git a/include/freefine_hip.h b/include/freefine_hip.h
--- a/include/freefine_hip.h
+++ b/include/freefine_hip.h
@@ -46,6 +46,9 @@
     int x3;
     int f8;
     int kv64_from;
+    const void* A2;
+    int lda2;
+    int K2;
 } ffn_igemm_desc;
 int ffn_igemm(void* stream, int dtype, const ffn_igemm_desc* d);
 int ffn_split_pair(void* stream, const float* src, void* dst, long rows, int C, int ld_src);
```
